# indrajeetadityaroy9/rabitq-ann-search

Hardware: AMD Instinct MI355X
Metric: qps (search_batch_device, layer-0 hot path end to end) + fastscan_dist_per_s (higher is better)
Workload: dtype u32 popcount / f32; 1 GPU; SIFT1M-class synthetic (int-valued, clustered; SURVEY 8d C2): 1000000x128 f32 (D=128), 4-bit RaBitQ FastScan + exact-L2 rerank, R=32, k=10, 10000 queries per GPU resident in HBM; n_index=1000000, dim=128, bits=4, k=10, nq_per_gpu=10000, index_builder=cphnsw_mi355x (this repo), batch_sets=2, parallelism=query-sharded x1, index replicated

## Files before the change

### include/cphnsw_mi355x.h

```cpp
#ifndef CPHNSW_MI355X_H
#define CPHNSW_MI355X_H

#include <stddef.h>
#include <stdint.h>

#ifdef __cplusplus
extern "C" {
#endif

typedef struct cph_index cph_index;

typedef enum {
    CPH_OK = 0,
    CPH_INVALID_ARGUMENT = 1,
    CPH_RUNTIME_ERROR = 2,
    CPH_OUT_OF_MEMORY = 3,
    CPH_NOT_IMPLEMENTED = 4
} cph_status;

const char* cph_last_error(void);

int cph_version(void);

int cph_create(uint64_t dim, uint64_t bits, int device, cph_index** out);
int cph_destroy(cph_index* h);

int cph_load(cph_index* h, const char* path);
int cph_save(cph_index* h, const char* path);
int cph_save_native(cph_index* h, const char* path);
int cph_load_native(cph_index* h, const char* path);
int cph_size(cph_index* h, uint64_t* n);
int cph_dim(cph_index* h, uint64_t* dim);
int cph_is_finalized(cph_index* h, int* flag);

int cph_build(cph_index* h, const float* vectors, uint64_t n);
int cph_finalize(cph_index* h);
int cph_knn_bruteforce(int device, const float* vectors, uint64_t n, uint64_t dim, const float* queries,
                       uint64_t nq, uint32_t* ids, float* dist);

int cph_encode_edges(int device, uint64_t dim, uint64_t bits, const float* parent, const float* nbrs, uint64_t cnt,
                     uint8_t* values, float* aux, uint32_t* pops);

int cph_select_hook(int device, const float* x, uint64_t n, uint64_t D, uint32_t vertex, const uint32_t* fwd,
                    const uint32_t* rev, uint64_t n_rev, uint32_t R, float alpha, float tau, float alpha_max,
                    const float* err, uint32_t* out_ids, uint32_t* out_cnt);

int cph_calib_hook(cph_index* h, const float* queries, const uint32_t* start, uint64_t ns, float* rec, uint32_t* rec_cnt,
                   float* dqp);

int cph_debug_heap_ops(int device, const uint8_t* ops, uint64_t n_ops, const float* keys, const uint32_t* ids, uint64_t n_push,
                       float* out_keys, uint32_t* out_ids, uint32_t* out_size);

int cph_search_batch(cph_index* h, const float* queries, uint64_t n, uint64_t k,
                     int64_t* ids, float* dist);

int cph_search_batch_device(cph_index* h, const float* d_queries, uint64_t n, uint64_t k,
                            int64_t* d_ids, float* d_dist, void* stream);
int cph_synchronize(cph_index* h);

typedef struct cph_filter cph_filter;
int cph_filter_create(cph_index* h, const uint32_t* words, uint64_t n_bits, cph_filter** out);
int cph_filter_destroy(cph_filter* f);
int cph_search_batch_filtered(cph_index* h, const float* queries, uint64_t n, uint64_t k, const cph_filter* f,
                              int64_t* ids, float* dist);
int cph_search_batch_device_filtered(cph_index* h, const float* d_queries, uint64_t n, uint64_t k,
                                     const cph_filter* f, int64_t* d_ids, float* d_dist, void* stream);

int cph_search(cph_index* h, const float* query, uint64_t k, int64_t* ids, float* dist,
               uint64_t* m);

int cph_get_vectors(cph_index* h, uint64_t first, uint64_t count, float* out);

int cph_set_batch_sets(cph_index* h, uint32_t n_sets);

int cph_set_search_params(cph_index* h, uint32_t slots, uint64_t beam_capacity);

int cph_last_search_stats(cph_index* h, uint64_t out[12]);
int cph_last_query_expansions(cph_index* index, uint32_t* out, uint64_t n);
int cph_order_queries(cph_index* index, const float* keys, uint64_t n, uint32_t* order);

int cph_encode_query(cph_index* h, const float* query, uint8_t* lut, float* coeffs);

int cph_entry_point(cph_index* h, const float* query, uint32_t* entry);

int cph_fastscan_block(cph_index* h, const uint8_t* lut, const float* qparams,
                       uint32_t vertex, float dist_qp_sq, float worst, int nn_full,
                       uint32_t* sums, uint32_t* msb, float* est, float* lower,
                       float* lower_stage1);

int cph_exact_l2(cph_index* h, const float* query, const uint32_t* ids, uint64_t n,
                 float* out);

typedef struct cph_stream cph_stream;
int cph_fastscan_stream_create(int device, uint32_t D, uint32_t bits, uint64_t n_blocks,
                               uint64_t seed, cph_stream** out, uint64_t* block_bytes);
int cph_fastscan_stream_run(cph_stream* s, int reps, double* avg_ms, double* checksum);
int cph_fastscan_stream_export(cph_stream* s, uint64_t first, uint64_t count,
                               uint8_t* ref_blocks, uint8_t* lut, float* qparams,
                               float* dist_qp_sq);
int cph_fastscan_stream_eval(cph_stream* s, uint64_t first, uint64_t count, float* est,
                             float* lower);
int cph_fastscan_stream_destroy(cph_stream* s);

int cph_host_rewrite_index(const char* path_in, const char* path_out);
int cph_host_repack_block(uint32_t D, uint32_t bits, const uint8_t* ref_block, uint8_t* dev_block,
                          uint64_t* dev_bytes, uint8_t* ref_roundtrip);
int cph_host_encode_query(uint64_t dim, const float* query, uint8_t* lut, float* coeffs, uint32_t* masks);

#ifdef __cplusplus
}
#endif
#endif
```

### rabitq-ann-search_amd/cphnsw_mi355x/_lib.py

```python
import ctypes as C
import importlib.util
import os
import sys

from . import build as _build

OK, INVALID_ARGUMENT, RUNTIME_ERROR, OUT_OF_MEMORY, NOT_IMPLEMENTED = range(5)

SYMBOLS = {
    "cph_last_error": (C.c_char_p, []),
    "cph_version": (C.c_int, []),
    "cph_create": (C.c_int, [C.c_uint64, C.c_uint64, C.c_int, C.POINTER(C.c_void_p)]),
    "cph_destroy": (C.c_int, [C.c_void_p]),
    "cph_load": (C.c_int, [C.c_void_p, C.c_char_p]),
    "cph_save": (C.c_int, [C.c_void_p, C.c_char_p]),
    "cph_save_native": (C.c_int, [C.c_void_p, C.c_char_p]),
    "cph_load_native": (C.c_int, [C.c_void_p, C.c_char_p]),
    "cph_size": (C.c_int, [C.c_void_p, C.POINTER(C.c_uint64)]),
    "cph_dim": (C.c_int, [C.c_void_p, C.POINTER(C.c_uint64)]),
    "cph_is_finalized": (C.c_int, [C.c_void_p, C.POINTER(C.c_int)]),
    "cph_build": (C.c_int, [C.c_void_p, C.c_void_p, C.c_uint64]),
    "cph_finalize": (C.c_int, [C.c_void_p]),
    "cph_knn_bruteforce": (C.c_int, [C.c_int, C.c_void_p, C.c_uint64, C.c_uint64, C.c_void_p, C.c_uint64,
                                     C.c_void_p, C.c_void_p]),
    "cph_debug_heap_ops": (C.c_int, [C.c_int, C.c_void_p, C.c_uint64, C.c_void_p, C.c_void_p, C.c_uint64, C.c_void_p, C.c_void_p,
                                     C.c_void_p]),
    "cph_select_hook": (C.c_int, [C.c_int, C.c_void_p, C.c_uint64, C.c_uint64, C.c_uint32, C.c_void_p, C.c_void_p, C.c_uint64,
                                  C.c_uint32, C.c_float, C.c_float, C.c_float, C.c_void_p, C.c_void_p, C.c_void_p]),
    "cph_calib_hook": (C.c_int, [C.c_void_p, C.c_void_p, C.c_void_p, C.c_uint64, C.c_void_p, C.c_void_p, C.c_void_p]),
    "cph_encode_edges": (C.c_int, [C.c_int, C.c_uint64, C.c_uint64, C.c_void_p, C.c_void_p, C.c_uint64, C.c_void_p,
                                   C.c_void_p, C.c_void_p]),
    "cph_search_batch": (C.c_int, [C.c_void_p, C.c_void_p, C.c_uint64, C.c_uint64, C.c_void_p, C.c_void_p]),
    "cph_search_batch_device": (C.c_int, [C.c_void_p, C.c_void_p, C.c_uint64, C.c_uint64, C.c_void_p,
                                          C.c_void_p, C.c_void_p]),
    "cph_filter_create": (C.c_int, [C.c_void_p, C.c_void_p, C.c_uint64, C.POINTER(C.c_void_p)]),
    "cph_filter_destroy": (C.c_int, [C.c_void_p]),
    "cph_search_batch_filtered": (C.c_int, [C.c_void_p, C.c_void_p, C.c_uint64, C.c_uint64, C.c_void_p, C.c_void_p,
                                            C.c_void_p]),
    "cph_search_batch_device_filtered": (C.c_int, [C.c_void_p, C.c_void_p, C.c_uint64, C.c_uint64, C.c_void_p,
                                                   C.c_void_p, C.c_void_p, C.c_void_p]),
    "cph_synchronize": (C.c_int, [C.c_void_p]),
    "cph_set_batch_sets": (C.c_int, [C.c_void_p, C.c_uint32]),
    "cph_search": (C.c_int, [C.c_void_p, C.c_void_p, C.c_uint64, C.c_void_p, C.c_void_p,
                             C.POINTER(C.c_uint64)]),
    "cph_get_vectors": (C.c_int, [C.c_void_p, C.c_uint64, C.c_uint64, C.c_void_p]),
    "cph_set_search_params": (C.c_int, [C.c_void_p, C.c_uint32, C.c_uint64]),
    "cph_last_search_stats": (C.c_int, [C.c_void_p, C.POINTER(C.c_uint64)]),
    "cph_last_query_expansions": (C.c_int, [C.c_void_p, C.c_void_p, C.c_uint64]),
    "cph_order_queries": (C.c_int, [C.c_void_p, C.c_void_p, C.c_uint64, C.c_void_p]),
    "cph_encode_query": (C.c_int, [C.c_void_p, C.c_void_p, C.c_void_p, C.c_void_p]),
    "cph_entry_point": (C.c_int, [C.c_void_p, C.c_void_p, C.POINTER(C.c_uint32)]),
    "cph_fastscan_block": (C.c_int, [C.c_void_p, C.c_void_p, C.c_void_p, C.c_uint32, C.c_float, C.c_float,
                                     C.c_int, C.c_void_p, C.c_void_p, C.c_void_p, C.c_void_p, C.c_void_p]),
    "cph_exact_l2": (C.c_int, [C.c_void_p, C.c_void_p, C.c_void_p, C.c_uint64, C.c_void_p]),
    "cph_host_rewrite_index": (C.c_int, [C.c_char_p, C.c_char_p]),
    "cph_host_repack_block": (C.c_int, [C.c_uint32, C.c_uint32, C.c_void_p, C.c_void_p, C.POINTER(C.c_uint64), C.c_void_p]),
    "cph_host_encode_query": (C.c_int, [C.c_uint64, C.c_void_p, C.c_void_p, C.c_void_p, C.c_void_p]),
    "cph_fastscan_stream_create": (C.c_int, [C.c_int, C.c_uint32, C.c_uint32, C.c_uint64, C.c_uint64,
                                             C.POINTER(C.c_void_p), C.POINTER(C.c_uint64)]),
    "cph_fastscan_stream_run": (C.c_int, [C.c_void_p, C.c_int, C.POINTER(C.c_double), C.POINTER(C.c_double)]),
    "cph_fastscan_stream_export": (C.c_int, [C.c_void_p, C.c_uint64, C.c_uint64, C.c_void_p, C.c_void_p,
                                             C.c_void_p, C.POINTER(C.c_float)]),
    "cph_fastscan_stream_eval": (C.c_int, [C.c_void_p, C.c_uint64, C.c_uint64, C.c_void_p, C.c_void_p]),
    "cph_fastscan_stream_destroy": (C.c_int, [C.c_void_p]),
}

_LIB = None


def _share_hip_runtime_with_torch():
    if "torch" in sys.modules:
        return
    try:
        spec = importlib.util.find_spec("torch")
    except (ImportError, ValueError):
        spec = None
    if spec is None or not spec.origin:
        return
    cand = os.path.join(os.path.dirname(spec.origin), "lib", "libamdhip64.so")
    if os.path.exists(cand):
        try:
            C.CDLL(cand, mode=C.RTLD_GLOBAL)
        except OSError:
            pass


def lib():
    global _LIB
    if _LIB is None:
        path = os.environ.get("CPH_LIB_PATH")
        if not path:
            path = _build.LIB_PATH
            if _build.needs_build():
                path = _build.build_library()
        _share_hip_runtime_with_torch()
        L = C.CDLL(path)
        diagnostic = bool(os.environ.get("CPH_LIB_PATH"))
        for name, (res, args) in SYMBOLS.items():
            try:
                fn = getattr(L, name)
            except AttributeError:
                if diagnostic:
                    continue
                raise
            fn.restype = res
            fn.argtypes = args
        _LIB = L
    return _LIB


def check(rc):
    if rc == OK:
        return
    msg = lib().cph_last_error().decode("utf-8", "replace")
    if rc == INVALID_ARGUMENT:
        raise ValueError(msg)
    if rc == OUT_OF_MEMORY:
        raise MemoryError(msg)
    if rc == NOT_IMPLEMENTED:
        raise NotImplementedError(msg)
    raise RuntimeError(msg)
```

### rabitq-ann-search_amd/cphnsw_mi355x/build.py

```python
import os
import shutil
import subprocess

PKG_DIR = os.path.dirname(os.path.abspath(__file__))
CSRC = os.path.join(os.path.dirname(PKG_DIR), "csrc")
LIB_PATH = os.path.join(PKG_DIR, "libcphnsw_mi355x.so")
SOURCES = ["cphnsw_mi355x.hip"]
HEADERS = ["cph_core.h", "builder.h", "builder_host.h", "host_parallel.h", "search_coalescer.h", "builder_pipeline.h", "device_knn.h", "device_knn_sym.h", "device_build.h", "device_buf.h", "native_file.h", "device_encode.h", "device_fastscan.h", "device_search.h", "device_stream.h", "device_heap_test.h", "host_index.h"]
FLAGS = ["-O3", "-std=c++17", "--offload-arch=gfx950", "-fPIC", "-shared", "-ffp-contract=off",
         "-Wall", "-Wno-unused-function"]


def _hipcc():
    for c in (os.environ.get("HIPCC"), shutil.which("hipcc"), "/opt/rocm/bin/hipcc"):
        if c and os.path.exists(c):
            return c
    raise RuntimeError("hipcc not found (need ROCm to build the gfx950 library)")


def needs_build():
    if not os.path.exists(LIB_PATH):
        return True
    t = os.path.getmtime(LIB_PATH)
    deps = [os.path.join(CSRC, f) for f in SOURCES + HEADERS]
    deps.append(os.path.join(os.path.dirname(os.path.dirname(PKG_DIR)), "include", "cphnsw_mi355x.h"))
    return any(os.path.getmtime(d) > t for d in deps if os.path.exists(d))


def build_library(force=False, verbose=False):
    if not force and not needs_build():
        return LIB_PATH
    cmd = [_hipcc()] + FLAGS + [os.path.join(CSRC, s) for s in SOURCES] + ["-o", LIB_PATH, "-lpthread"]
    if verbose:
        print(" ".join(cmd))
    subprocess.check_call(cmd)
    return LIB_PATH


if __name__ == "__main__":
    print(build_library(force=True, verbose=True))
```

### rabitq-ann-search_amd/csrc/builder_pipeline.h

```cpp
#pragma once
#include <exception>
#include <thread>
#include <type_traits>
#include "builder.h"

namespace cph {
namespace build {

struct BuiltDevice {
    DevBuf<uint8_t> blocks;
    DevBuf<float> raw;
    DevBuf<float> norm;
    std::vector<uint8_t> own_host;
};

inline size_t isqrt_sz(size_t n) { return (size_t)std::floor(std::sqrt((double)n)); }

template <int BW, bool G>
inline void launch_encode(const EncodeArgsB& a, uint32_t grid, size_t lds) {
    if (lds > 48 * 1024)
        HIP_CHECK(hipFuncSetAttribute(reinterpret_cast<const void*>(&encode_edges_kernel<BW, G>),
                                      hipFuncAttributeMaxDynamicSharedMemorySize, (int)lds));
    hipLaunchKernelGGL((encode_edges_kernel<BW, G>), dim3(grid), dim3(64), lds, nullptr, a);
    HIP_CHECK(hipGetLastError());
// ... 95 lines not shown
        if (Dk == D) {
            knn_self_device(d_x.p, d_norm.p, n, D, num_cus, d_knn.p, d_kd.p, verbose);
        } else {
            DevBuf<float> d_xk(n * Dk);
            HIP_CHECK(hipMemset(d_xk.p, 0, n * Dk * 4));
            HIP_CHECK(hipMemcpy2D(d_xk.p, Dk * 4, d_x.p, D * 4, D * 4, n, hipMemcpyDeviceToDevice));
            knn_self_device(d_xk.p, d_norm.p, n, Dk, num_cus, d_knn.p, d_kd.p, verbose);
        }
    }
    tm.lap("exact 32-NN (MFMA)");

    GraphStatsRecord gs{};
    {
        const size_t sample = std::max<size_t>(1, std::min(isqrt_sz(n), n));
        std::mt19937 rng(43);
        std::vector<size_t> pick(n);
        std::iota(pick.begin(), pick.end(), 0);
        std::shuffle(pick.begin(), pick.end(), rng);
        pick.resize(sample);
        auto dist = [&](uint32_t a, uint32_t b) {
            double s = 0;
            for (size_t j = 0; j < dim; ++j) { const double t = (double)vecs[(size_t)a * dim + j] - vecs[(size_t)b * dim + j]; s += t * t; }
            return (float)s;
        };
        const size_t pairs_of = std::clamp((size_t)(2.0 * std::sqrt((double)R)), (size_t)4, (size_t)R);
        std::vector<float> edge_len, first_len, between;
        std::vector<uint32_t> row(kKnnK);
        double deg = 0;
        for (size_t v : pick) {
            HIP_CHECK(hipMemcpy(row.data(), d_knn.p + v * kKnnK, kKnnK * 4, hipMemcpyDeviceToHost));
            size_t c = 0;
            while (c < (size_t)kKnnK && row[c] != kInvalidNode) ++c;
            deg += (double)c;
            for (size_t s = 0; s < c; ++s) edge_len.push_back(dist((uint32_t)v, row[s]));
            if (c) first_len.push_back(edge_len[edge_len.size() - c]);
            const size_t m = std::min(c, pairs_of);
            for (size_t i = 0; i < m; ++i)
                for (size_t j = i + 1; j < m; ++j) between.push_back(dist(row[i], row[j]));
        }
        gs.avg_degree = (float)(deg / (double)pick.size());
        if (edge_len.empty() || between.empty() || first_len.empty()) {
            gs.alpha = 1.0f; gs.tau = 0.0f; gs.alpha_max = 4.0f;
        } else {
            std::sort(edge_len.begin(), edge_len.end());
            std::sort(between.begin(), between.end());
            const float tiny = 1e-8f / (float)D;
            const float med = quantile_sorted(edge_len, 1, 2), q1 = quantile_sorted(edge_len, 1, 4), q3 = quantile_sorted(edge_len, 3, 4);
            double mu = 0, var = 0;
            for (float d : edge_len) mu += d;
            mu /= edge_len.size();
            for (float d : edge_len) var += (d - mu) * (d - mu);
            var /= edge_len.size();
            const float cv = mu > tiny ? (float)(std::sqrt(var) / mu) : 0.2f;
            const float inter = quantile_sorted(between, 1, 4);
            gs.alpha = inter < tiny ? 1.0f + cv : med / inter;
            gs.alpha_max = std::min(q1 > tiny ? q3 / q1 : 2.0f, 5.0f);
            gs.alpha = std::clamp(gs.alpha, 1.0f, gs.alpha_max);
            gs.alpha_max = std::max(gs.alpha_max, 2.0f * gs.alpha);
            gs.tau = mad_sigma(first_len, median_of(first_len));
        }
    }

    DevBuf<uint32_t> d_nbr(n * 32), d_cnt(n);
    {
        DevBuf<float> d_err(n);
        const float err_tol = 1.0f / std::sqrt((float)D);
        hipLaunchKernelGGL(centered_norm_kernel, dim3(grid_for(n, 256)), dim3(256), 0, nullptr, d_x.p, d_centroid.p, (uint64_t)n,
                           (uint32_t)D, (uint32_t)dim, err_tol, d_err.p);
        HIP_CHECK(hipGetLastError());
        LayerParams lp{R, gs.alpha, gs.tau, gs.alpha_max, d_err.p};
        select_layer(d_x.p, D, d_knn.p, n, nullptr, lp, num_cus, d_nbr.p, d_cnt.p);
    }
    d_knn.release();
    tm.lap("reverse edges + selection");

    std::vector<uint32_t> nbr(n * 32), cnt(n);
    HIP_CHECK(hipMemcpy(nbr.data(), d_nbr.p, n * 32 * 4, hipMemcpyDeviceToHost));
    HIP_CHECK(hipMemcpy(cnt.data(), d_cnt.p, n * 4, hipMemcpyDeviceToHost));
    std::vector<uint32_t> old_to_new(n, kInvalidNode), new_to_old(n);
    {
        std::vector<std::pair<double, uint32_t>> near(n);
        parallel_for(n, 4096, [&](size_t lo, size_t hi_) {
            for (size_t i = lo; i < hi_; ++i) {
                double s = 0;
                for (size_t j = 0; j < dim; ++j) { const double t = (double)vecs[i * dim + j] - centroid[j]; s += t * t; }
                near[i] = {s, (uint32_t)i};
            }
        });
        const size_t top = std::min(n, std::max<size_t>(1, isqrt_sz(n)));
        std::partial_sort(near.begin(), near.begin() + top, near.end());
        uint32_t hub = near[0].second;
        for (size_t i = 1; i < top; ++i)
            if (cnt[near[i].second] > cnt[hub]) hub = near[i].second;
        std::vector<uint8_t> seen(n, 0);
        std::vector<uint32_t> queue;
        queue.reserve(n);
        uint32_t next = 0;
        auto walk = [&](uint32_t start) {
            if (seen[start]) return;
            seen[start] = 1;
            queue.push_back(start);
            for (size_t head = queue.size() - 1; head < queue.size(); ++head) {
                const uint32_t v = queue[head];
                old_to_new[v] = next;
                new_to_old[next++] = v;
                for (uint32_t j = 0; j < cnt[v]; ++j) {
                    const uint32_t w = nbr[(size_t)v * 32 + j];
                    if (w < n && !seen[w]) { seen[w] = 1; queue.push_back(w); }
                }
            }
        };
        walk(hub);
        for (size_t i = 0; i < n; ++i) walk((uint32_t)i);
    }
    tm.lap("hub + BFS order");

    DevBuf<uint32_t> d_o2n(n), d_n2o(n);
    HIP_CHECK(hipMemcpy(d_o2n.p, old_to_new.data(), n * 4, hipMemcpyHostToDevice));
    HIP_CHECK(hipMemcpy(d_n2o.p, new_to_old.data(), n * 4, hipMemcpyHostToDevice));
    dev.raw.alloc(n * D);
    dev.norm.alloc(n);
    hipLaunchKernelGGL(gather_rows_kernel, dim3((uint32_t)std::min<uint64_t>(n, (uint64_t)num_cus * 64)), dim3(64), 0, nullptr,
                       d_x.p, d_n2o.p, (uint64_t)n, (uint32_t)D, dev.raw.p);
    HIP_CHECK(hipGetLastError());
    hipLaunchKernelGGL(gather_u32_kernel, dim3(grid_for(n, 256)), dim3(256), 0, nullptr, d_norm.p, d_n2o.p, (uint64_t)n, dev.norm.p);
    HIP_CHECK(hipGetLastError());
    DevBuf<uint32_t> d_nbr_new(n * 32);
    hipLaunchKernelGGL(permute_lists_kernel, dim3(grid_for(n * 32, 256)), dim3(256), 0, nullptr, d_nbr.p, d_n2o.p, d_o2n.p,
                       (uint64_t)n, d_nbr_new.p);
    HIP_CHECK(hipGetLastError());
    HIP_CHECK(hipDeviceSynchronize());
    d_x.release(); d_norm.release(); d_nbr.release(); d_cnt.release();

    DevBuf<float> d_signs(3 * D);
    HIP_CHECK(hipMemcpy(d_signs.p, hi.rot.signs.data(), 3 * D * 4, hipMemcpyHostToDevice));
    const float df = (float)D;
    const float norm_factor = 1.0f / (df * std::sqrt(df)), inv_sqrt_d = 1.0f / std::sqrt(df);
    dev.blocks.alloc(n * L.stride + 64);
    HIP_CHECK(hipMemset(dev.blocks.p, 0, n * L.stride + 64));
    const size_t words = (D + 63) / 64;
    const uint32_t own_meta = (uint32_t)round_up(bw * words * 8, 64);
    const uint32_t own_stride = (uint32_t)hi.RL.nb_off;
    DevBuf<uint8_t> d_own(n * own_stride);
    HIP_CHECK(hipMemset(d_own.p, 0, n * own_stride));
    {
        EncodeArgsB a{};
        a.x = dev.raw.p; a.nbr = d_nbr_new.p; a.centroid = d_centroid.p; a.n = n; a.dim = (uint32_t)dim; a.D = (uint32_t)D;
        a.signs = d_signs.p; a.norm_factor = norm_factor; a.inv_sqrt_d = inv_sqrt_d; a.L = L; a.blocks = dev.blocks.p;
        a.own = d_own.p; a.own_stride = own_stride; a.own_meta = own_meta;
        run_encode(bw, a, n, num_cus);
        a.nbr = nullptr;
        run_encode(bw, a, (n + 31) / 32, num_cus);
    }
    tm.lap("gather + edge / own codes");

    std::vector<int32_t> levels_new(n);
    for (size_t nw = 0; nw < n; ++nw) levels_new[nw] = levels[new_to_old[nw]];
    upper_job.wait();
    std::vector<std::vector<UpperEdge>> upper = ul.export_layers(old_to_new);
    const float upper_tau = ul.tau, upper_alpha = ul.alpha;
    tm.lap("upper layers (host threads, built behind the kNN): wait + export");

    hi.raw.resize(n * D);
    hi.norm_sq.resize(n);
    HIP_CHECK(hipMemcpy(hi.raw.data(), dev.raw.p, n * D * 4, hipMemcpyDeviceToHost));
    HIP_CHECK(hipMemcpy(hi.norm_sq.data(), dev.norm.p, n * 4, hipMemcpyDeviceToHost));
    hi.levels = std::move(levels_new);
    hi.search_data.clear();
    dev.own_host.resize(n * (size_t)own_stride);
    HIP_CHECK(hipMemcpy(dev.own_host.data(), d_own.p, n * (size_t)own_stride, hipMemcpyDeviceToHost));
    hi.upper = std::move(upper);
    hi.max_level = max_level;
    hi.entry = old_to_new[entry_old];
    hi.upper_tau = upper_tau;
    hi.upper_alpha = upper_alpha;
    hi.centroid = centroid;
    ProfileRecord prof;
    prof.n = n; prof.D = D; prof.R = R; prof.bits = bw;
    prof.evt_min_tail = std::max<size_t>(64, isqrt_sz(n));
    prof.min_calib_samples = std::clamp((size_t)(10.0 * std::sqrt((double)n)), (size_t)200, n);
    prof.slack_levels = std::clamp((int)std::ceil(std::log2(std::max(10.0f * std::log2((float)std::max(n, (size_t)64)), 4.0f))), 4, 32);
    prof.graph_stats = gs;
    std::memcpy(hi.profile, &prof, 72);
    std::memset(hi.calib, 0, sizeof(hi.calib));
    tm.lap("vectors, norms, own codes to the host");
}

struct DeviceIndexView {
    const uint8_t* blocks;
    const float* raw;
    const float* signs;
    DevLayout L;
    float norm_factor, inv_sqrt_d;
};

inline void calibrate(HostIndex& hi, const DeviceIndexView& dv, int num_cus, bool verbose) {
    StageTimer tm{verbose};
    const size_t n = hi.n, D = hi.D, dim = hi.dim, bw = hi.bw;
    if (n < 50) throw std::runtime_error("Calibration requires at least 50 nodes.");
    ProfileRecord prof;
    std::memcpy(&prof, hi.profile, 72);
    const size_t n_db = std::min(prof.min_calib_samples, n), n_syn = std::min(prof.min_calib_samples / 2, n);
    const size_t ns = n_db + n_syn;
    std::mt19937 rng(42 + 99999);
    std::vector<uint32_t> order(n);
    std::iota(order.begin(), order.end(), 0u);
    std::shuffle(order.begin(), order.end(), rng);
    std::vector<float> sigma(dim, 0.0f);
    {
        const size_t vs = std::max<size_t>(2, std::min(n, prof.min_calib_samples / 4));
        std::vector<double> s1(dim, 0.0), s2(dim, 0.0);
        for (size_t i = 0; i < vs; ++i) {
            const float* v = hi.vec(order[i]);
            for (size_t d = 0; d < dim; ++d) { s1[d] += v[d]; s2[d] += (double)v[d] * v[d]; }
        }
        for (size_t d = 0; d < dim; ++d) {
            const double mu = s1[d] / vs;
            sigma[d] = (float)std::sqrt(std::max(s2[d] / vs - mu * mu, (double)kEpsSmall));
        }
    }
    std::vector<float> q(ns * dim);
    std::vector<uint32_t> start(ns);
    for (size_t i = 0; i < n_db; ++i) {
        std::memcpy(&q[i * dim], hi.vec(order[i]), dim * 4);
        start[i] = order[i];
    }
    std::normal_distribution<float> gauss(0.0f, 1.0f);
    for (size_t i = 0; i < n_syn; ++i) {
        const float* base = hi.vec(order[i % n]);
        for (size_t d = 0; d < dim; ++d) q[(n_db + i) * dim + d] = base[d] + gauss(rng) * sigma[d];
        start[n_db + i] = order[(n_db + i) % n];
    }
    const uint32_t PW = dv.L.PW;
    DevBuf<float> d_q(ns * dim), d_qp(ns * D), d_rec(ns * 32 * 6), d_dqp(ns), d_ed(ns);
    DevBuf<uint4> d_masks(ns * PW);
    DevBuf<QueryHeader> d_hdr(ns);
    DevBuf<uint32_t> d_start(ns), d_rc(ns);
    HIP_CHECK(hipMemcpy(d_q.p, q.data(), ns * dim * 4, hipMemcpyHostToDevice));
    HIP_CHECK(hipMemcpy(d_start.p, start.data(), ns * 4, hipMemcpyHostToDevice));
    {
        EncodeArgs e{};
        e.queries_raw = d_q.p; e.nq = (uint32_t)ns; e.dim = (uint32_t)dim; e.D = (uint32_t)D; e.PW = PW;
        e.signs = dv.signs; e.norm_factor = dv.norm_factor; e.inv_sqrt_d = dv.inv_sqrt_d;
        e.raw = dv.raw; e.n = n; e.entry = 0; e.max_level = 0;
        e.queries_padded = d_qp.p; e.qmasks = d_masks.p; e.qhdr = d_hdr.p; e.entry_dist = d_ed.p;
        hipLaunchKernelGGL(encode_kernel, dim3((uint32_t)std::min<uint64_t>(ns, (uint64_t)num_cus * 32)), dim3(64),
                           encode_lds_bytes((uint32_t)D), nullptr, e);
        HIP_CHECK(hipGetLastError());
        CalibArgs c{};
        c.blocks = dv.blocks; c.raw = dv.raw; c.L = dv.L; c.n = n; c.queries = d_qp.p; c.qmasks = d_masks.p; c.qhdr = d_hdr.p;
        c.start = d_start.p; c.ns = (uint32_t)ns; c.rec = d_rec.p; c.rec_cnt = d_rc.p; c.dqp_out = d_dqp.p;
        const size_t lds = (size_t)PW * 16 + (size_t)D * 8;
        const dim3 grid((uint32_t)std::min<uint64_t>(ns, (uint64_t)num_cus * 16));
        if (bw == 1) hipLaunchKernelGGL(calib_kernel<1>, grid, dim3(64), lds, nullptr, c);
        else if (bw == 2) hipLaunchKernelGGL(calib_kernel<2>, grid, dim3(64), lds, nullptr, c);
        else hipLaunchKernelGGL(calib_kernel<4>, grid, dim3(64), lds, nullptr, c);
        HIP_CHECK(hipGetLastError());
    }
    std::vector<float> rec(ns * 32 * 6), dqp(ns);
    std::vector<uint32_t> rc(ns);
    HIP_CHECK(hipMemcpy(rec.data(), d_rec.p, rec.size() * 4, hipMemcpyDeviceToHost));
    HIP_CHECK(hipMemcpy(dqp.data(), d_dqp.p, ns * 4, hipMemcpyDeviceToHost));
    HIP_CHECK(hipMemcpy(rc.data(), d_rc.p, ns * 4, hipMemcpyDeviceToHost));
    tm.lap("calibration samples (GPU)");

    CalibrationRecord cal{};
    std::vector<float> ipqo, est_ratio, truth, nops;
    struct Pair { float nop, ipc, ipq, dqp, exact; };
    std::vector<Pair> pairs;
    for (size_t s = 0; s < ns; ++s)
        for (uint32_t j = 0; j < rc[s] && j < 32; ++j) {
            const float* r = &rec[(s * 32 + j) * 6];
            ipqo.push_back(r[5]);
            nops.push_back(r[0]);
            truth.push_back(r[3]);
            pairs.push_back({r[0], r[1], r[2], dqp[s], r[4]});
        }
    if (ipqo.empty()) throw std::runtime_error("Calibration failed: no ip_qo samples.");
    if (pairs.size() < 20) throw std::runtime_error("Calibration failed: too few estimator/target pairs.");
    {
        const float med = median_of(ipqo);
        cal.ip_qo_floor = std::max(med - 3.0f * mad_sigma(ipqo, med), kEpsMedium);
    }
    est_ratio.resize(pairs.size());
    for (size_t i = 0; i < pairs.size(); ++i) est_ratio[i] = pairs[i].ipc / std::max(pairs[i].ipq, cal.ip_qo_floor);
    {
        double a, b;
        robust_line(est_ratio, truth, a, b);
        const size_t np = truth.size();
        double mt = 0, me = 0;
        for (size_t i = 0; i < np; ++i) { mt += truth[i]; me += est_ratio[i]; }
        mt /= np; me /= np;
        double ssr = 0, sst = 0, sxx = 0;
        for (size_t i = 0; i < np; ++i) {
            const double res = truth[i] - (a * est_ratio[i] + b);
            ssr += res * res;
            sst += (truth[i] - mt) * (truth[i] - mt);
            sxx += (est_ratio[i] - me) * (est_ratio[i] - me);
        }
        const double r2 = sst > kEpsSmall ? 1.0 - ssr / sst : 0.0;
        double lev = 0.0;
        if (sxx > kEpsSmall)
            for (size_t i = 0; i < np; ++i) lev = std::max(lev, 1.0 / np + (est_ratio[i] - me) * (est_ratio[i] - me) / sxx);
        if (r2 < 0.1 || lev > 4.0 / (double)np) { a = 1.0; b = 0.0; }
        cal.affine_a = (float)a;
        cal.affine_b = (float)b;
// ... 49 lines not shown
```

### rabitq-ann-search_amd/csrc/cph_core.h

```cpp
#pragma once
#include <cstddef>
#include <cstdint>

namespace cph {

constexpr uint32_t kInvalidNode = 0xFFFFFFFFu;
constexpr int kR = 32;
constexpr float kEpsTiny = 1e-20f;
constexpr float kEpsSmall = 1e-12f;
constexpr float kEpsMedium = 1e-10f;
constexpr int kMaxSlack = 32;

struct DevLayout {
    uint32_t D;
    uint32_t BW;
    uint32_t PW;
    uint32_t wide;
    uint32_t NH;
    uint32_t CPL;
    uint32_t codes_bytes;
    uint32_t aux_off;
    uint32_t ids_off;
    uint32_t count_off;
    uint32_t stride;
};

#ifndef CPH_BLOCK_ALIGN
#define CPH_BLOCK_ALIGN 64u
#endif
template <int BW, int SD>
struct StaticLayout {
    static constexpr uint32_t kCodesBytes = 32u * (uint32_t)BW * (SD >= 32 ? (uint32_t)SD / 32u : 1u) * 4u;
    static constexpr uint32_t kAuxOff = kCodesBytes;
    static constexpr uint32_t kIdsOff = kAuxOff + 32u * 16u;
    static constexpr uint32_t kCountOff = kIdsOff + 32u * 4u;
    static constexpr uint32_t kStride = (kCountOff + 4u + CPH_BLOCK_ALIGN - 1u) / CPH_BLOCK_ALIGN * CPH_BLOCK_ALIGN;
};

inline DevLayout make_dev_layout(uint32_t D, uint32_t BW) {
    DevLayout L{};
    L.D = D;
    L.BW = BW;
    L.PW = D >= 32 ? D / 32 : 1;
    L.wide = D >= 128 ? 1 : 0;
    uint32_t T = BW * L.PW;
    if (L.wide) {
        L.NH = (T / 4 >= 2) ? 2 : 1;
        L.CPL = T / 4 / L.NH;
    } else {
        L.NH = 1;
        L.CPL = 0;
    }
    L.codes_bytes = 32 * T * 4;
    L.aux_off = L.codes_bytes;
    L.ids_off = L.aux_off + 32 * 16;
    L.count_off = L.ids_off + 32 * 4;
    L.stride = (L.count_off + 4 + CPH_BLOCK_ALIGN - 1) / CPH_BLOCK_ALIGN * CPH_BLOCK_ALIGN;
    return L;
}

struct RefLayout {
    size_t vertex_bytes, nb_off;
    size_t codes, nop, ip_qo, ip_cp, pop, wpop, ids, count;
    size_t plane_bytes, nb_bytes;
};

inline size_t round_up(size_t x, size_t a) { return (x + a - 1) / a * a; }

inline RefLayout make_ref_layout(size_t D, size_t bw) {
    RefLayout L{};
    size_t words = (D + 63) / 64;
    size_t code = round_up(round_up(bw * words * 8, 64) + 8, 64);
    L.plane_bytes = (((D + 3) / 4 + 1) / 2) * 32;
    size_t o = 0;
    L.codes = o; o += bw * round_up(L.plane_bytes, 64);
    L.nop = o;   o += 128;
    L.ip_qo = o; o += 128;
    L.ip_cp = o; o += 128;
    L.pop = o;   o += 64;
    if (bw > 1) { L.wpop = o; o += 64; } else { L.wpop = (size_t)-1; }
    L.ids = o;   o += 128;
    L.count = o; o += 4;
    L.nb_bytes = round_up(o, 64);
    L.nb_off = code;
    L.vertex_bytes = code + L.nb_bytes;
    return L;
}

struct QueryHeader {
    float A, B, C;
    uint32_t entry;
};

struct SearchConsts {
    float affine_a, affine_b, ip_qo_floor;
    float gamma, gamma_max, gamma_beta;
    uint64_t gamma_warmup;
    int32_t num_slack;
    float slack[kMaxSlack];
};

enum QueryStatus : uint32_t { kStatusOk = 0, kStatusOverflow = 1 };

}
```

### rabitq-ann-search_amd/csrc/cphnsw_mi355x.hip

```cpp
#include <hip/hip_runtime.h>

#include <algorithm>
#include <atomic>
#include <cfloat>
#include <chrono>
#include <condition_variable>
#include <deque>
#include <functional>
#include <memory>
#include <mutex>
#include <new>
#include <string>
#include <thread>
#include <vector>

#include "../../include/cphnsw_mi355x.h"
#include "cph_core.h"
#include "device_buf.h"
#include "device_encode.h"
#include "device_fastscan.h"
#include "device_search.h"
#include "device_stream.h"
#include "device_heap_test.h"
#include "host_index.h"
#include "host_parallel.h"
#include "search_coalescer.h"
#include "native_file.h"
#include "builder_pipeline.h"

using namespace cph;

namespace {

thread_local std::string g_err;

int fail(int code, const std::string& msg) {
    g_err = msg;
    return code;
}

struct InvalidArg : std::invalid_argument {
    using std::invalid_argument::invalid_argument;
};

template <class F>
int guarded(F&& f) {
    try {
        f();
        return CPH_OK;
    } catch (const std::invalid_argument& e) {
        return fail(CPH_INVALID_ARGUMENT, e.what());
    } catch (const std::bad_alloc&) {
        return fail(CPH_OUT_OF_MEMORY, "out of memory");
    } catch (const std::exception& e) {
        return fail(CPH_RUNTIME_ERROR, e.what());
    }
}

size_t next_pow2(size_t n) {
    size_t p = 1;
    while (p < n) p *= 2;
    return p;
}

#define CPH_LAUNCH_BITS(KERNEL, bits, SDV, grid, block, lds, st, args)                            \
    do {                                                                                          \
        if ((bits) == 1) hipLaunchKernelGGL((KERNEL<1, SDV>), grid, block, lds, st, args);        \
        else if ((bits) == 2) hipLaunchKernelGGL((KERNEL<2, SDV>), grid, block, lds, st, args);   \
        else hipLaunchKernelGGL((KERNEL<4, SDV>), grid, block, lds, st, args);                    \
    } while (0)
#define CPH_LAUNCH(KERNEL, bits, D, grid, block, lds, st, args)                                   \
    do {                                                                                          \
        if ((D) == 128) CPH_LAUNCH_BITS(KERNEL, bits, 128, grid, block, lds, st, args);           \
        else if ((D) == 1024) CPH_LAUNCH_BITS(KERNEL, bits, 1024, grid, block, lds, st, args);    \
        else CPH_LAUNCH_BITS(KERNEL, bits, 0, grid, block, lds, st, args);                        \
        HIP_CHECK(hipGetLastError());                                                             \
    } while (0)

__global__ void scan_counts_kernel(const uint8_t* blocks, uint64_t n, uint32_t stride, uint32_t count_off, uint32_t* flags) {
    const uint64_t v = (uint64_t)blockIdx.x * blockDim.x + threadIdx.x;
    if (v >= n) return;
    const uint32_t cnt = *reinterpret_cast<const uint32_t*>(blocks + v * stride + count_off);
    if (cnt & 7u) atomicOr(flags, 2u);
}

}

struct BatchSet {
    DevBuf<float> d_queries_raw, d_queries, d_entry_dist, d_dist;
    DevBuf<uint4> d_qmasks;
    DevBuf<QueryHeader> d_qhdr;
    DevBuf<int64_t> d_ids;
    DevBuf<uint32_t> d_count, d_status, d_order, d_redo;
    DevBuf<unsigned long long> d_stats;
    unsigned long long* pin_stats = nullptr;
    uint8_t* pin_io = nullptr;
    uint8_t* pin_io_dev = nullptr;
    size_t pin_io_bytes = 0;
    DevBuf<uint32_t> d_bitmaps, d_logids;
    DevBuf<uint32_t> d_beam, d_beam_tail;
    uint32_t slots = 0;
    uint64_t cap = 0;
    DevBuf<uint32_t> r_bitmaps, r_logids;
    DevBuf<uint32_t> r_beam, r_beam_tail;
    uint32_t r_slots = 0;
    hipEvent_t ev0 = nullptr, ev1 = nullptr, ev_done = nullptr;
    bool used = false;
    uint32_t nq = 0;
    uint32_t run_slots = 0;
    uint64_t run_cap = 0;
    bool stats_in_hbm = false;
};
constexpr int kStatWords = 18;
constexpr int kMaxBatchSets = 4;
constexpr uint64_t kSmallBatch = 32;

struct cph_filter {
    int device = 0;
    uint64_t n_bits = 0;
    uint64_t popcount = 0;
    DevBuf<uint32_t> words;
};

struct cph_index {
    uint64_t dim = 0;
    uint32_t bits = 0;
    uint32_t D = 0;
    int device = 0;
    bool finalized = false;
    bool needs_build = false;
    std::vector<float> pending;
    uint64_t pending_n = 0;
    HostIndex host;
    DevLayout L{};
    SearchConsts sc{};
    uint32_t flags = 0;
    int num_cus = 256;
    bool waves_from_env = false;
    uint32_t waves_per_cu = 4 * CPH_SEARCH_WAVES_PER_SIMD;
    DevBuf<uint8_t> d_blocks;
    DevBuf<float> d_raw, d_norm;
    DevBuf<float> d_signs;
    DevBuf<uint32_t> d_upper;
    DevBuf<uint32_t> d_row_of;
    UpperLayerDev layers[kMaxUpperLayers];
    int32_t dev_max_level = 0;
    float norm_factor = 0.0f, inv_sqrt_d = 0.0f;
    NativeMapping native_map;
    const uint8_t* own_view = nullptr;
    std::vector<uint8_t> own_store;
    BatchSet sets[kMaxBatchSets + kLeaderSlots];
    int n_sets = 2;
    int last_set = kMaxBatchSets - 1;
    int last_search = -1;
    hipStream_t own_stream = nullptr;
    bool order_queries = true;
    uint32_t want_slots = 0;
    uint64_t want_cap = 0;
    uint64_t auto_cap = 0;
    bool pf_off = false;
    bool pf_dense = false;
    std::mutex mu;
    SearchCoalescer coal;
    struct LeaderSlot {
        hipStream_t stream = nullptr;
        uint8_t* pin = nullptr;
        uint8_t* pin_dev = nullptr;
        size_t pin_bytes = 0;
        uint32_t seq = 0;
        uint64_t cur_n = 0, cur_k = 0;
    } leaders[kLeaderSlots];

    void use_device() const { HIP_CHECK(hipSetDevice(device)); }
};

namespace {

bool probe_first(const cph_index* h) {
    return (h->L.D == 128 || h->L.D == 1024) && !(h->flags & 2u) && !h->pf_off && !h->pf_dense;
}

void require_finalized(cph_index* h) {
    if (!h->finalized) throw std::runtime_error("Search failed: invalid entry point after finalize.");
}

void release_scratch(BatchSet& s) {
    s.d_bitmaps.release(); s.d_logids.release(); s.d_beam.release(); s.d_beam_tail.release();
    s.r_bitmaps.release(); s.r_logids.release(); s.r_beam.release(); s.r_beam_tail.release();
    s.slots = 0; s.cap = 0; s.r_slots = 0;
}

void quiesce(cph_index* h) {
    for (auto& s : h->sets)
        if (s.used && s.ev_done) HIP_CHECK(hipEventSynchronize(s.ev_done));
}

void upload_arrays(cph_index* h) {
    h->use_device();
    quiesce(h);
    const HostIndex& hi = h->host;
    h->L = make_dev_layout((uint32_t)hi.D, (uint32_t)hi.bw);
    const size_t n = hi.n;
    const size_t stride = h->L.stride;
    h->d_blocks.alloc(n * stride + 64);
    h->d_raw.alloc(n * hi.D);
    h->d_norm.alloc(n);
    const size_t chunk = std::max<size_t>(1, std::min<size_t>(n, (256u << 20) / stride));
    std::vector<uint8_t> stage(chunk * stride);
    for (size_t base = 0; base < n; base += chunk) {
        const size_t cnt = std::min(chunk, n - base);
        parallel_for(cnt, 256, [&](size_t lo, size_t hi_) {
            for (size_t v = lo; v < hi_; ++v)
                repack_ref_to_dev(hi.nb(base + v), hi.RL, h->L, &stage[v * stride]);
        });
        HIP_CHECK(hipMemcpy(h->d_blocks.p + base * stride, stage.data(), cnt * stride,
                            hipMemcpyHostToDevice));
    }
    HIP_CHECK(hipMemcpy(h->d_raw.p, hi.raw.data(), n * hi.D * 4, hipMemcpyHostToDevice));
    HIP_CHECK(hipMemcpy(h->d_norm.p, hi.norm_sq.data(), n * 4, hipMemcpyHostToDevice));
}

void upload_feeders(cph_index* h) {
    h->use_device();
    quiesce(h);
    const HostIndex& hi = h->host;
    const size_t n = hi.n;
    h->L = make_dev_layout((uint32_t)hi.D, (uint32_t)hi.bw);
    h->sc = hi.consts();
    h->flags = hi.has_dup_neighbors ? 1u : 0u;
    if (n != 0) {
        DevBuf<uint32_t> d_flag(1);
        HIP_CHECK(hipMemset(d_flag.p, 0, 4));
        hipLaunchKernelGGL(scan_counts_kernel, dim3((uint32_t)((n + 255) / 256)), dim3(256), 0, nullptr, h->d_blocks.p, (uint64_t)n,
                           h->L.stride, h->L.count_off, d_flag.p);
        HIP_CHECK(hipGetLastError());
        uint32_t f = 0;
        HIP_CHECK(hipMemcpy(&f, d_flag.p, 4, hipMemcpyDeviceToHost));
        h->flags |= f & 2u;
    }
    h->d_signs.alloc(3 * hi.D);
    HIP_CHECK(hipMemcpy(h->d_signs.p, hi.rot.signs.data(), 3 * hi.D * 4, hipMemcpyHostToDevice));
    const float d = static_cast<float>(hi.D);
    h->norm_factor = 1.0f / (d * std::sqrt(d));
    h->inv_sqrt_d = 1.0f / std::sqrt(d);
    const int nl = std::min<int>({(int)hi.upper.size(), (int)hi.max_level, kMaxUpperLayers});
    h->dev_max_level = hi.max_level > 0 ? nl : 0;
    std::vector<uint32_t> flat;
    std::vector<size_t> off_nodes(nl), off_offs(nl), off_nbrs(nl);
    for (int l = 0; l < nl; ++l) {
        const auto& layer = hi.upper[l];
        off_nodes[l] = flat.size();
        for (const auto& e : layer) flat.push_back(e.node);
        off_offs[l] = flat.size();
        uint32_t acc = 0;
        for (const auto& e : layer) { flat.push_back(acc); acc += (uint32_t)e.nbrs.size(); }
        flat.push_back(acc);
        off_nbrs[l] = flat.size();
        for (const auto& e : layer) flat.insert(flat.end(), e.nbrs.begin(), e.nbrs.end());
    }
    h->d_upper.alloc(flat.size() + 1);
    if (!flat.empty())
        HIP_CHECK(hipMemcpy(h->d_upper.p, flat.data(), flat.size() * 4, hipMemcpyHostToDevice));
    for (int l = 0; l < kMaxUpperLayers; ++l) h->layers[l] = UpperLayerDev{nullptr, nullptr, nullptr, nullptr, 0};
    int mapped = 0;
    for (int l = 0; l < nl; ++l) mapped += hi.upper[l].size() > 16 ? 1 : 0;
    h->d_row_of.alloc((size_t)mapped * n + 1);
    std::vector<uint32_t> row_of;
    for (int l = 0, m = 0; l < nl; ++l) {
        const uint32_t* dmap = nullptr;
        if (hi.upper[l].size() > 16) {
            row_of.assign(n, kInvalidNode);
            uint64_t first = 0;
            bool fits = true;
            for (size_t r = 0; r < hi.upper[l].size(); ++r) {
                const uint64_t deg = hi.upper[l][r].nbrs.size();
                if (first >= (1u << 26) || deg > 62) { fits = false; break; }
                row_of[hi.upper[l][r].node] = (uint32_t)first | ((uint32_t)deg << 26);
                first += deg;
            }
            if (!fits) { h->layers[l] = UpperLayerDev{h->d_upper.p + off_nodes[l], h->d_upper.p + off_offs[l], h->d_upper.p + off_nbrs[l], nullptr, (uint32_t)hi.upper[l].size()}; ++m; continue; }
            HIP_CHECK(hipMemcpy(h->d_row_of.p + (size_t)m * n, row_of.data(), n * 4, hipMemcpyHostToDevice));
            dmap = h->d_row_of.p + (size_t)m * n;
            ++m;
        }
        h->layers[l] = UpperLayerDev{h->d_upper.p + off_nodes[l], h->d_upper.p + off_offs[l],
                                     h->d_upper.p + off_nbrs[l], dmap, (uint32_t)hi.upper[l].size()};
    }
    for (auto& s : h->sets) release_scratch(s);
    h->auto_cap = 0;
    h->pf_off = false;
    h->pf_dense = false;
    h->last_search = -1;
}

void materialize_search_data(cph_index* h) {
    HostIndex& hi = h->host;
    if (!hi.search_data.empty() || hi.n == 0) return;
    h->use_device();
    quiesce(h);
    const size_t n = hi.n, stride = h->L.stride, own_stride = hi.RL.nb_off;
    hi.search_data.assign(n * hi.RL.vertex_bytes, 0);
    const size_t chunk = std::max<size_t>(1, std::min<size_t>(n, (512u << 20) / stride));
    std::vector<uint8_t> stage(chunk * stride);
    for (size_t base = 0; base < n; base += chunk) {
        const size_t c = std::min(chunk, n - base);
        HIP_CHECK(hipMemcpy(stage.data(), h->d_blocks.p + base * stride, c * stride, hipMemcpyDeviceToHost));
        parallel_for(c, 256, [&](size_t lo, size_t hi_) {
            for (size_t v = lo; v < hi_; ++v) {
                uint8_t* dst = &hi.search_data[(base + v) * hi.RL.vertex_bytes];
                if (h->own_view) std::memcpy(dst, h->own_view + (base + v) * own_stride, own_stride);
                repack_dev_to_ref(&stage[v * stride], h->L, hi.RL, dst + hi.RL.nb_off);
            }
        });
    }
}

void init_set(BatchSet& s) {
    if (s.ev0) return;
    HIP_CHECK(hipEventCreate(&s.ev0));
    HIP_CHECK(hipEventCreate(&s.ev1));
    HIP_CHECK(hipEventCreateWithFlags(&s.ev_done, hipEventDisableTiming));
    HIP_CHECK(hipHostMalloc(reinterpret_cast<void**>(&s.pin_stats), kStatWords * 8, hipHostMallocDefault));
    std::memset(s.pin_stats, 0, kStatWords * 8);
}

BatchSet& next_set(cph_index* h, hipStream_t st) {
    h->last_set = (h->last_set + 1) % h->n_sets;
    BatchSet& s = h->sets[h->last_set];
    init_set(s);
    for (BatchSet& o : h->sets) {
        if (!(o.used && o.ev_done && !o.stats_in_hbm && hipEventQuery(o.ev_done) == hipSuccess)) continue;
        if (o.pin_stats[5] > o.pin_stats[8] && o.cap < h->host.n + 1)
            h->auto_cap = std::max<uint64_t>(h->auto_cap, std::min<uint64_t>(h->host.n + 1, o.cap * 4));
        if (o.pin_stats[8] * 50 > o.nq) h->pf_off = true;
        if (o.pin_stats[0] >= 10000) {
            const double new_per_exp = (double)o.pin_stats[2] / (double)o.pin_stats[0];
            const double off = h->bits == 4 ? 6.0 : 2.8, on = h->bits == 4 ? 4.5 : 2.2;
            if (new_per_exp > off) h->pf_dense = true;
            else if (new_per_exp < on) h->pf_dense = false;
        }
    }
    if (s.used) HIP_CHECK(hipStreamWaitEvent(st, s.ev_done, 0));
    return s;
}

void stage_queries(cph_index* h, BatchSet& s, const float* d_raw_q, uint64_t nq, hipStream_t st) {
    const HostIndex& hi = h->host;
    const uint32_t D = (uint32_t)hi.D, PW = h->L.PW;
    if (hi.entry == kInvalidNode || hi.entry >= hi.n)
        throw std::runtime_error("Search failed: invalid entry point after finalize.");
    if (s.d_queries.n < nq * D || s.d_qmasks.n < nq * PW || s.d_qhdr.n < nq) {
        if (s.used) HIP_CHECK(hipEventSynchronize(s.ev_done));
        s.d_queries.alloc(nq * D);
        s.d_qmasks.alloc(nq * PW);
        s.d_qhdr.alloc(nq);
        s.d_entry_dist.alloc(nq);
        s.d_order.alloc(nq);
    }
    EncodeArgs a{};
    a.queries_raw = d_raw_q;
    a.nq = (uint32_t)nq;
    a.dim = (uint32_t)hi.dim;
    a.D = D;
    a.PW = PW;
    a.signs = h->d_signs.p;
    a.norm_factor = h->norm_factor;
    a.inv_sqrt_d = h->inv_sqrt_d;
    a.raw = h->d_raw.p;
    a.n = hi.n;
    a.entry = hi.entry;
    a.max_level = h->dev_max_level;
    for (int l = 0; l < kMaxUpperLayers; ++l) a.layers[l] = h->layers[l];
    a.queries_padded = s.d_queries.p;
    a.qmasks = s.d_qmasks.p;
    a.qhdr = s.d_qhdr.p;
    a.entry_dist = s.d_entry_dist.p;
    const uint32_t grid = (uint32_t)std::min<uint64_t>(nq, (uint64_t)h->num_cus * 32);
    hipLaunchKernelGGL(encode_kernel, dim3(grid), dim3(64), encode_lds_bytes(D), st, a);
    HIP_CHECK(hipGetLastError());
}

const float* upload_queries(cph_index* h, BatchSet& s, const float* queries, uint64_t nq, hipStream_t st) {
    if (s.d_queries_raw.n < nq * h->dim) {
        if (s.used) HIP_CHECK(hipEventSynchronize(s.ev_done));
        s.d_queries_raw.alloc(nq * h->dim);
    }
    HIP_CHECK(hipMemcpyAsync(s.d_queries_raw.p, queries, nq * h->dim * 4, hipMemcpyHostToDevice, st));
    return s.d_queries_raw.p;
}

void ensure_scratch(cph_index* h, BatchSet& s, uint32_t slots, uint64_t cap, hipStream_t st) {
    const uint64_t n = h->host.n;
    const uint64_t bm_words = (n + 31) / 32;
    if (!(s.slots >= slots && s.cap == cap)) {
        if (s.used) HIP_CHECK(hipEventSynchronize(s.ev_done));
        s.d_bitmaps.alloc((size_t)slots * bm_words);
        HIP_CHECK(hipMemsetAsync(s.d_bitmaps.p, 0, (size_t)slots * bm_words * 4, st));
        s.d_logids.alloc((size_t)slots * cap);
        s.d_beam.alloc((size_t)slots * kBeamPagesDwords);
        s.d_beam_tail.alloc((size_t)slots * beam_tail_dwords(cap));
        s.slots = slots;
        s.cap = cap;
    }
    if ((cap < n + 1 || probe_first(h)) && s.r_slots == 0) {
        size_t free_b = 0, total_b = 0;
        HIP_CHECK(hipMemGetInfo(&free_b, &total_b));
        const uint64_t per = (n + 1) * 4 + ((uint64_t)kBeamPagesDwords + beam_tail_dwords(n + 1)) * 4 + bm_words * 4;
        const uint64_t want = (&s - h->sets) >= kMaxBatchSets ? kLeaderGroup : kSmallBatch;
        const uint32_t rs = (uint32_t)std::max<uint64_t>(1, std::min<uint64_t>(want, (uint64_t)(free_b * 0.25) / per));
        s.r_bitmaps.alloc((size_t)rs * bm_words);
        HIP_CHECK(hipMemsetAsync(s.r_bitmaps.p, 0, (size_t)rs * bm_words * 4, st));
        s.r_logids.alloc((size_t)rs * (n + 1));
        s.r_beam.alloc((size_t)rs * kBeamPagesDwords);
        s.r_beam_tail.alloc((size_t)rs * beam_tail_dwords(n + 1));
        s.r_slots = rs;
    }
}

struct DoneFlags {
    uint32_t* flags = nullptr;
    uint32_t seq = 0;
};

template <int SD>
void launch_filtered(uint32_t bits, uint32_t grid, size_t lds, hipStream_t st, const SearchArgs& a) {
    if (bits == 1) hipLaunchKernelGGL((search_kernel<1, SD, false, true>), dim3(grid), dim3(64), lds, st, a);
    else if (bits == 2) hipLaunchKernelGGL((search_kernel<2, SD, false, true>), dim3(grid), dim3(64), lds, st, a);
    else hipLaunchKernelGGL((search_kernel<4, SD, false, true>), dim3(grid), dim3(64), lds, st, a);
    HIP_CHECK(hipGetLastError());
}

void launch_search(cph_index* h, BatchSet& s, uint32_t nq, uint32_t k, int64_t* d_ids, float* d_dist, uint32_t* d_count,
                   const uint32_t* d_todo, int mode, hipStream_t st, DoneFlags done = DoneFlags(),
                   const uint32_t* d_allow = nullptr) {
    SearchArgs a{};
    a.allow = d_allow;
    const bool pf = d_allow == nullptr && probe_first(h);
    a.done_flags = done.flags;
    a.done_seq = done.seq;
    a.blocks = h->d_blocks.p;
    a.raw = h->d_raw.p;
    a.norm_sq = h->d_norm.p;
    a.n = h->host.n;
    a.L = h->L;
    a.flags = h->flags;
    a.queries = s.d_queries.p;
    a.qmasks = s.d_qmasks.p;
    a.qhdr = s.d_qhdr.p;
    a.k = k;
    a.sc = h->sc;
    a.bm_words = (h->host.n + 31) / 32;
    a.out_ids = d_ids;
    a.out_dist = d_dist;
    a.out_count = d_count;
    a.status = s.d_status.p;
    a.stats = s.d_stats.p;
    uint32_t* words = reinterpret_cast<uint32_t*>(s.d_stats.p + 16);
    uint32_t grid;
    if (mode == 0) {
// ... 139 lines not shown

struct SmallIo {
    int64_t* h_ids; float* h_dist; uint32_t* h_count; float* h_query;
    int64_t* d_ids; float* d_dist; uint32_t* d_count; const float* d_query;
};
SmallIo small_io(cph_index* h, BatchSet& s, uint64_t n, uint64_t k) {
    const size_t o_dist = n * k * 8, o_cnt = o_dist + n * k * 4, o_q = (o_cnt + n * 4 + 15) & ~(size_t)15;
    const size_t need = o_q + n * h->dim * 4;
    if (s.pin_io_bytes < need) {
        if (s.used) HIP_CHECK(hipEventSynchronize(s.ev_done));
        if (s.pin_io) HIP_CHECK(hipHostFree(s.pin_io));
        s.pin_io = nullptr;
        s.pin_io_bytes = 0;
        const size_t bytes = std::max<size_t>(need * 2, 64 * 1024);
        HIP_CHECK(hipHostMalloc(reinterpret_cast<void**>(&s.pin_io), bytes, hipHostMallocMapped | hipHostMallocCoherent));
        HIP_CHECK(hipHostGetDevicePointer(reinterpret_cast<void**>(&s.pin_io_dev), s.pin_io, 0));
        s.pin_io_bytes = bytes;
    }
    uint8_t* hb = s.pin_io;
    uint8_t* db = s.pin_io_dev;
    return SmallIo{reinterpret_cast<int64_t*>(hb), reinterpret_cast<float*>(hb + o_dist), reinterpret_cast<uint32_t*>(hb + o_cnt),
                   reinterpret_cast<float*>(hb + o_q),
                   reinterpret_cast<int64_t*>(db), reinterpret_cast<float*>(db + o_dist), reinterpret_cast<uint32_t*>(db + o_cnt),
                   reinterpret_cast<const float*>(db + o_q)};
}

}

#ifdef CPH_SEARCH_TRACE
static std::atomic<uint64_t> g_tr[6];
static inline uint64_t now_ns() { return std::chrono::duration_cast<std::chrono::nanoseconds>(std::chrono::steady_clock::now().time_since_epoch()).count(); }
#define CPH_TR(i, v) g_tr[i] += (v)
#else
#define CPH_TR(i, v) do {} while (0)
static inline uint64_t now_ns() { return 0; }
#endif

extern "C" {

const char* cph_last_error(void) { return g_err.c_str(); }
int cph_version(void) { return 100; }

int cph_create(uint64_t dim, uint64_t bits, int device, cph_index** out) {
    return guarded([&] {
        if (!out) throw InvalidArg("out must not be null");
        *out = nullptr;
        if (bits != 1 && bits != 2 && bits != 4)
            throw InvalidArg("Unsupported bits=" + std::to_string(bits) + ". Supported: 1, 2, 4.");
        const size_t pd = next_pow2(dim);
        if (dim == 0) throw InvalidArg("dim must be > 0");
        if (pd < 16 || pd > 2048) {
            if (pd < 16) {
                throw InvalidArg("Unsupported dimension " + std::to_string(dim) + " (padded to " +
                                 std::to_string(pd) +
                                 "). Supported padded dims: 16, 32, 64, 128, 256, 512, 1024, 2048.");
            }
            throw InvalidArg("Unsupported dimension " + std::to_string(dim) + " (padded to " +
                             std::to_string(pd) +
                             "). Supported padded dims: 16, 32, 64, 128, 256, 512, 1024, 2048.");
        }
        int ndev = 0;
        if (hipGetDeviceCount(&ndev) != hipSuccess || ndev <= 0)
            throw std::runtime_error("No HIP device available: the MI355X path has no CPU fallback.");
        if (device < 0 || device >= ndev) throw InvalidArg("invalid device ordinal");
        auto* h = new cph_index();
        h->dim = dim;
        h->bits = (uint32_t)bits;
        h->D = (uint32_t)pd;
        h->device = device;
        hipDeviceProp_t prop;
        if (hipGetDeviceProperties(&prop, device) == hipSuccess) h->num_cus = prop.multiProcessorCount;
        if (const char* e = getenv("CPH_QUERY_ORDER")) h->order_queries = atoi(e) != 0;
        if (const char* e = getenv("CPH_LEADER_SLOTS")) h->coal.n_slots = std::max(1, std::min(kLeaderSlots, atoi(e)));
        if (const char* e = getenv("CPH_GATHER_US")) h->coal.gather_us = std::max(0, atoi(e));
        if (const char* e = getenv("CPH_WAVES_PER_CU")) { h->waves_per_cu = (uint32_t)std::max(1, atoi(e)); h->waves_from_env = true; }
        *out = h;
    });
}

int cph_destroy(cph_index* h) {
    return guarded([&] {
        if (!h) return;
        (void)hipSetDevice(h->device);
        for (auto& s : h->sets) {
            if (s.used && s.ev_done) (void)hipEventSynchronize(s.ev_done);
            if (s.ev0) (void)hipEventDestroy(s.ev0);
            if (s.ev1) (void)hipEventDestroy(s.ev1);
            if (s.ev_done) (void)hipEventDestroy(s.ev_done);
            if (s.pin_stats) (void)hipHostFree(s.pin_stats);
            if (s.pin_io) (void)hipHostFree(s.pin_io);
        }
#ifdef CPH_SEARCH_TRACE
        if (g_tr[0]) fprintf(stderr, "[search trace] groups=%llu callers=%llu per group: mutex wait %.1f us, enqueue %.1f us; per caller: own-query wait %.1f us\n",
                             (unsigned long long)g_tr[0], (unsigned long long)g_tr[1], g_tr[2] / 1e3 / g_tr[0], g_tr[3] / 1e3 / g_tr[0], g_tr[4] / 1e3 / g_tr[1]);
        for (auto& x : g_tr) x = 0;
#endif
        if (h->own_stream) (void)hipStreamDestroy(h->own_stream);
        for (auto& ls : h->leaders) {
            if (ls.stream) { (void)hipStreamSynchronize(ls.stream); (void)hipStreamDestroy(ls.stream); }
            if (ls.pin) (void)hipHostFree(ls.pin);
        }
        delete h;
    });
}

static void begin_device_swap(cph_index* h) {
    h->use_device();
    quiesce(h);
    h->finalized = false;
    for (auto& s : h->sets) release_scratch(s);
    h->last_search = -1;
}

int cph_load(cph_index* h, const char* path) {
    return guarded([&] {
        if (!h || !path) throw InvalidArg("null argument");
        std::lock_guard<std::mutex> lk(h->mu);
        HostIndex t;
        t.load(path, h->D, h->bits, h->dim);
        begin_device_swap(h);
        h->host = std::move(t);
        h->needs_build = false;
        std::vector<float>().swap(h->pending);
        h->pending_n = 0;
        h->native_map.reset();
        h->own_view = nullptr;
        std::vector<uint8_t>().swap(h->own_store);
        upload_arrays(h);
        upload_feeders(h);
        h->finalized = true;
    });
}

int cph_save(cph_index* h, const char* path) {
    return guarded([&] {
        if (!h || !path) throw InvalidArg("null argument");
        std::lock_guard<std::mutex> lk(h->mu);
        if (!h->finalized) throw std::runtime_error("Index must be finalized before saving.");
        materialize_search_data(h);
        h->host.save(path);
    });
}

int cph_save_native(cph_index* h, const char* path) {
    return guarded([&] {
        if (!h || !path) throw InvalidArg("null argument");
        std::lock_guard<std::mutex> lk(h->mu);
        if (!h->finalized) throw std::runtime_error("Index must be finalized before saving.");
        h->use_device();
        quiesce(h);
        const HostIndex& hi = h->host;
        const size_t n = hi.n, stride = h->L.stride, own_stride = hi.RL.nb_off;
        std::vector<uint8_t> blocks(n * stride), own;
        HIP_CHECK(hipMemcpy(blocks.data(), h->d_blocks.p, n * stride, hipMemcpyDeviceToHost));
        const uint8_t* own_p = h->own_view;
        if (!own_p) {
            own.resize(n * own_stride);
            for (size_t v = 0; v < n; ++v) std::memcpy(&own[v * own_stride], &hi.search_data[v * hi.RL.vertex_bytes], own_stride);
            own_p = own.data();
        }
        write_native(path, hi, (uint32_t)stride, own_p, (uint32_t)own_stride, blocks.data());
    });
}

int cph_load_native(cph_index* h, const char* path) {
    return guarded([&] {
        if (!h || !path) throw InvalidArg("null argument");
        std::lock_guard<std::mutex> lk(h->mu);
        HostIndex t;
        NativeMapping map;
        const NativeHeader nh = read_native(path, h->D, h->bits, h->dim, t, map);
        begin_device_swap(h);
        h->host = std::move(t);
        h->needs_build = false;
        std::vector<float>().swap(h->pending);
        h->pending_n = 0;
        h->native_map = std::move(map);
        const uint8_t* base = static_cast<const uint8_t*>(h->native_map.base);
        std::vector<uint8_t>().swap(h->own_store);
        h->own_view = base + nh.own_off;
        h->L = make_dev_layout((uint32_t)h->host.D, (uint32_t)h->host.bw);
        const size_t n = h->host.n;
        h->d_blocks.alloc(n * nh.stride + 64);
        h->d_raw.alloc(n * h->host.D);
        h->d_norm.alloc(n);
        HIP_CHECK(hipMemcpy(h->d_blocks.p, base + nh.blocks_off, n * (size_t)nh.stride, hipMemcpyHostToDevice));
        HIP_CHECK(hipMemcpy(h->d_raw.p, h->host.raw_view, n * h->host.D * 4, hipMemcpyHostToDevice));
        HIP_CHECK(hipMemcpy(h->d_norm.p, h->host.norm_sq.data(), n * 4, hipMemcpyHostToDevice));
        upload_feeders(h);
        h->finalized = true;
    });
}

int cph_size(cph_index* h, uint64_t* n) {
    return guarded([&] { *n = h->needs_build ? h->pending_n : h->host.n; });
}
int cph_dim(cph_index* h, uint64_t* dim) {
    return guarded([&] { *dim = h->dim; });
}
int cph_is_finalized(cph_index* h, int* flag) {
    return guarded([&] { *flag = h->finalized ? 1 : 0; });
}

int cph_build(cph_index* h, const float* vectors, uint64_t n) {
    return guarded([&] {
        if (!h) throw InvalidArg("null handle");
        std::lock_guard<std::mutex> lk(h->mu);
        if (n == 0) throw InvalidArg("build requires at least one vector.");
        if (!vectors) throw InvalidArg("null vectors");
        h->use_device();
        quiesce(h);
        h->host = HostIndex();
        h->native_map.reset();
        h->own_view = nullptr;
        std::vector<uint8_t>().swap(h->own_store);
        h->finalized = false;
        h->d_blocks.release(); h->d_raw.release(); h->d_norm.release();
        for (auto& s : h->sets) release_scratch(s);
        h->pending.assign(vectors, vectors + n * h->dim);
        h->pending_n = n;
        h->needs_build = true;
    });
}

int cph_finalize(cph_index* h) {
    return guarded([&] {
        if (!h) throw InvalidArg("null handle");
        std::lock_guard<std::mutex> lk(h->mu);
        const uint64_t n = h->needs_build ? h->pending_n : h->host.n;
        if (n == 0) throw std::runtime_error("Cannot finalize an empty index.");
        if (!h->needs_build) throw std::runtime_error("Finalize called without a pending build.");
        if (n < 50) throw std::runtime_error("Calibration requires at least 50 nodes.");
        if (n >= 0xFFFFFFFFull) throw InvalidArg("too many vectors");
        h->use_device();
        const bool verbose = getenv("CPH_BUILD_VERBOSE") != nullptr;
        quiesce(h);
        h->d_blocks.release(); h->d_raw.release(); h->d_norm.release();
        for (auto& s : h->sets) release_scratch(s);
        build::BuiltDevice dev;
        build::build_graph(h->host, dev, h->pending.data(), n, h->dim, h->D, h->bits, h->num_cus, verbose);
        std::vector<float>().swap(h->pending);
        h->pending_n = 0;
        h->needs_build = false;
        h->d_blocks = std::move(dev.blocks);
        h->d_raw = std::move(dev.raw);
        h->d_norm = std::move(dev.norm);
        h->native_map.reset();
        h->own_store = std::move(dev.own_host);
        h->own_view = h->own_store.data();
        upload_feeders(h);
        build::DeviceIndexView view{h->d_blocks.p, h->d_raw.p, h->d_signs.p, h->L, h->norm_factor, h->inv_sqrt_d};
        build::calibrate(h->host, view, h->num_cus, verbose);
        h->sc = h->host.consts();
        h->finalized = true;
    });
}

int cph_knn_bruteforce(int device, const float* vectors, uint64_t n, uint64_t dim, const float* queries,
                       uint64_t nq, uint32_t* ids, float* dist) {
    return guarded([&] {
        if (!vectors || !ids || !dist || n == 0 || dim == 0) throw InvalidArg("bad arguments");
        if (n >= 0xFFFFFFFFull || nq >= 0xFFFFFFFFull) throw InvalidArg("too many rows");
        HIP_CHECK(hipSetDevice(device));
        const size_t D = std::max<size_t>(16, next_pow2(dim));
        auto pad = [&](const float* src, uint64_t rows, std::vector<float>& x, std::vector<float>& nrm) {
            x.assign(rows * D, 0.0f);
            nrm.resize(rows);
            parallel_for(rows, 1024, [&](size_t lo, size_t hi) {
                for (size_t i = lo; i < hi; ++i) {
                    std::memcpy(&x[i * D], src + i * dim, dim * 4);
                    float s = 0.0f;
                    for (uint64_t j = 0; j < dim; ++j) s = std::fmaf(x[i * D + j], x[i * D + j], s);
                    nrm[i] = s;
                }
            });
        };
        std::vector<float> x, nrm, q, qn;
        pad(vectors, n, x, nrm);
        if (queries) pad(queries, nq, q, qn);
        int cus = 256;
        hipDeviceProp_t prop;
        if (hipGetDeviceProperties(&prop, device) == hipSuccess) cus = prop.multiProcessorCount;
        build::gpu_knn(queries ? q.data() : nullptr, queries ? qn.data() : nullptr, nq, x.data(), nrm.data(), n, D,
                       cus, ids, dist);
    });
}

int cph_debug_heap_ops(int device, const uint8_t* ops, uint64_t n_ops, const float* keys, const uint32_t* ids, uint64_t n_push,
                       float* out_keys, uint32_t* out_ids, uint32_t* out_size) {
    return guarded([&] {
        if (!ops || !out_keys || !out_ids || !out_size || n_ops == 0 || n_ops > 0x7FFFFFFFull) throw InvalidArg("bad arguments");
        if (n_push && (!keys || !ids)) throw InvalidArg("bad arguments");
        uint64_t pushes = 0;
        for (uint64_t i = 0; i < n_ops; ++i) pushes += ops[i] ? 1 : 0;
        if (pushes != n_push) throw InvalidArg("n_push must equal the number of push operations");
        HIP_CHECK(hipSetDevice(device));
        DevBuf<uint8_t> d_ops(n_ops);
        DevBuf<float> d_keys(std::max<uint64_t>(1, n_push)), d_ok(std::max<uint64_t>(1, n_push));
        DevBuf<uint32_t> d_ids(std::max<uint64_t>(1, n_push)), d_oi(std::max<uint64_t>(1, n_push)), d_sz(1);
        DevBuf<uint32_t> d_spill(kBeamPagesDwords), d_spill_tail(beam_tail_dwords(std::max<uint64_t>(1, n_push) + 64));
        HIP_CHECK(hipMemcpy(d_ops.p, ops, n_ops, hipMemcpyHostToDevice));
        if (n_push) {
            HIP_CHECK(hipMemcpy(d_keys.p, keys, n_push * 4, hipMemcpyHostToDevice));
            HIP_CHECK(hipMemcpy(d_ids.p, ids, n_push * 4, hipMemcpyHostToDevice));
        }
        HeapTestArgs a{d_ops.p, d_keys.p, d_ids.p, (uint32_t)n_ops, d_spill.p, d_spill_tail.p, d_ok.p, d_oi.p, d_sz.p};
        hipLaunchKernelGGL(heap_selftest_kernel, dim3(1), dim3(64), 0, nullptr, a);
        HIP_CHECK(hipGetLastError());
        HIP_CHECK(hipDeviceSynchronize());
        HIP_CHECK(hipMemcpy(out_size, d_sz.p, 4, hipMemcpyDeviceToHost));
        if (*out_size > n_push) throw std::runtime_error("heap self-test: size out of range");
        if (*out_size) {
            HIP_CHECK(hipMemcpy(out_keys, d_ok.p, (size_t)*out_size * 4, hipMemcpyDeviceToHost));
            HIP_CHECK(hipMemcpy(out_ids, d_oi.p, (size_t)*out_size * 4, hipMemcpyDeviceToHost));
        }
    });
}

int cph_encode_edges(int device, uint64_t dim, uint64_t bits, const float* parent, const float* nbrs, uint64_t cnt,
                     uint8_t* values, float* aux, uint32_t* pops) {
    return guarded([&] {
        if (!parent || !nbrs || !values || !aux || !pops || cnt == 0 || cnt > 32 || dim == 0) throw InvalidArg("bad arguments");
        if (bits != 1 && bits != 2 && bits != 4) throw InvalidArg("bits must be 1, 2 or 4");
        const size_t D = std::max<size_t>(16, next_pow2(dim));
        if (D > 2048) throw InvalidArg("unsupported dimension");
        HIP_CHECK(hipSetDevice(device));
        const size_t n = cnt + 1;
        std::vector<float> x(n * D, 0.0f);
        std::memcpy(x.data(), parent, dim * 4);
        for (uint64_t e = 0; e < cnt; ++e) std::memcpy(&x[(e + 1) * D], nbrs + e * dim, dim * 4);
        std::vector<uint32_t> nbr(n * 32, kInvalidNode);
        for (uint64_t e = 0; e < cnt; ++e) nbr[e] = (uint32_t)(e + 1);
        Rotation rot;
        rot.init(D, 42);
        const DevLayout L = make_dev_layout((uint32_t)D, (uint32_t)bits);
        DevBuf<float> d_x(n * D), d_signs(3 * D), d_aux(n * 32 * 3);
        DevBuf<uint32_t> d_nbr(n * 32), d_pops(n * 32 * 2);
        DevBuf<uint8_t> d_blocks(n * L.stride), d_vals(n * 32 * D);
        HIP_CHECK(hipMemcpy(d_x.p, x.data(), n * D * 4, hipMemcpyHostToDevice));
// ... 432 lines not shown
        r.query = query; r.k = kk; r.ids = ids; r.dist = dist; r.m = m;
        h->coal.submit(r,
                       [&](int slot, const std::vector<SearchReq*>& group) { launch_search_group(h, h->leaders[slot], group); },
                       [&](int slot, uint32_t index, SearchReq& me) { wait_search_one(h, h->leaders[slot], index, me); });
    });
    if (rc != CPH_OK) return rc;
    return r.rc == CPH_OK ? CPH_OK : fail(r.rc, r.err);
}

int cph_encode_query(cph_index* h, const float* query, uint8_t* lut, float* coeffs) {
    return guarded([&] {
        std::lock_guard<std::mutex> lk(h->mu);
        require_finalized(h);
        h->use_device();
        hipStream_t st = own_stream(h);
        BatchSet& s = next_set(h, st);
        stage_queries(h, s, upload_queries(h, s, query, 1, st), 1, st);
        HIP_CHECK(hipEventRecord(s.ev_done, st));
        s.used = true;
        HIP_CHECK(hipStreamSynchronize(st));
        const uint32_t D = h->D, PW = h->L.PW;
        std::vector<uint32_t> masks(PW * 4);
        QueryHeader hd;
        HIP_CHECK(hipMemcpy(masks.data(), s.d_qmasks.p, PW * 16, hipMemcpyDeviceToHost));
        HIP_CHECK(hipMemcpy(&hd, s.d_qhdr.p, sizeof(hd), hipMemcpyDeviceToHost));
        std::vector<uint8_t> qu(D);
        for (uint32_t d = 0; d < D; ++d) {
            uint8_t u = 0;
            for (int j = 0; j < 4; ++j) u |= (uint8_t)(((masks[(d / 32) * 4 + j] >> (d % 32)) & 1u) << j);
            qu[d] = u;
        }
        qu_to_lut(qu.data(), D, lut);
        coeffs[0] = hd.A; coeffs[1] = hd.B; coeffs[2] = hd.C;
    });
}

int cph_entry_point(cph_index* h, const float* query, uint32_t* entry) {
    return guarded([&] {
        std::lock_guard<std::mutex> lk(h->mu);
        require_finalized(h);
        h->use_device();
        hipStream_t st = own_stream(h);
        BatchSet& s = next_set(h, st);
        stage_queries(h, s, upload_queries(h, s, query, 1, st), 1, st);
        HIP_CHECK(hipEventRecord(s.ev_done, st));
        s.used = true;
        HIP_CHECK(hipStreamSynchronize(st));
        QueryHeader hd;
        HIP_CHECK(hipMemcpy(&hd, s.d_qhdr.p, sizeof(hd), hipMemcpyDeviceToHost));
        *entry = hd.entry;
    });
}

int cph_fastscan_block(cph_index* h, const uint8_t* lut, const float* qparams, uint32_t vertex,
                       float dist_qp_sq, float worst, int nn_full, uint32_t* sums, uint32_t* msb,
                       float* est, float* lower, float* lower_stage1) {
    return guarded([&] {
        std::lock_guard<std::mutex> lk(h->mu);
        require_finalized(h);
        if (vertex >= h->host.n) throw InvalidArg("vertex out of range");
        h->use_device();
        const uint32_t D = h->D, PW = h->L.PW;
        std::vector<uint8_t> qu(D);
        lut_to_qu(lut, D, qu.data());
        std::vector<uint32_t> masks(PW * 4);
        qu_to_masks(qu.data(), D, masks.data());
        DevBuf<uint4> d_mask;
        DevBuf<uint32_t> d_u;
        DevBuf<float> d_f;
        d_mask.alloc(PW);
        d_u.alloc(64);
        d_f.alloc(96);
        HIP_CHECK(hipMemcpy(d_mask.p, masks.data(), PW * 16, hipMemcpyHostToDevice));
        BlockHookArgs a{};
        a.blk = h->d_blocks.p + (size_t)vertex * h->L.stride;
        a.L = h->L;
        a.qmask = d_mask.p;
        a.qp = QP{qparams[0], qparams[1], qparams[2], qparams[3], qparams[4], qparams[5], qparams[6]};
        a.dqp = dist_qp_sq;
        a.worst = worst;
        a.nn_full = nn_full;
        a.sums = d_u.p; a.msb = d_u.p + 32;
        a.est = d_f.p; a.lower = d_f.p + 32; a.lower1 = d_f.p + 64;
        CPH_LAUNCH(block_hook_kernel, h->bits, D, dim3(1), dim3(64), (size_t)PW * 16, nullptr, a);
        HIP_CHECK(hipDeviceSynchronize());
        uint32_t hu[64];
        float hf[96];
        HIP_CHECK(hipMemcpy(hu, d_u.p, sizeof(hu), hipMemcpyDeviceToHost));
        HIP_CHECK(hipMemcpy(hf, d_f.p, sizeof(hf), hipMemcpyDeviceToHost));
        std::memcpy(sums, hu, 128); std::memcpy(msb, hu + 32, 128);
        std::memcpy(est, hf, 128); std::memcpy(lower, hf + 32, 128);
        std::memcpy(lower_stage1, hf + 64, 128);
    });
}

int cph_exact_l2(cph_index* h, const float* query, const uint32_t* ids, uint64_t n, float* out) {
    return guarded([&] {
        std::lock_guard<std::mutex> lk(h->mu);
        require_finalized(h);
        if (n == 0) return;
        for (uint64_t i = 0; i < n; ++i)
            if (ids[i] >= h->host.n) throw InvalidArg("id out of range");
        h->use_device();
        const uint32_t D = h->D;
        std::vector<float> buf(D, 0.0f);
        std::memcpy(buf.data(), query, h->dim * sizeof(float));
        DevBuf<float> d_q, d_out;
        DevBuf<uint32_t> d_i;
        d_q.alloc(D); d_out.alloc(n); d_i.alloc(n);
        HIP_CHECK(hipMemcpy(d_q.p, buf.data(), D * 4, hipMemcpyHostToDevice));
        HIP_CHECK(hipMemcpy(d_i.p, ids, n * 4, hipMemcpyHostToDevice));
        const uint32_t grid = (uint32_t)std::min<uint64_t>((n + 7) / 8, 1024);
        hipLaunchKernelGGL(exact_l2_hook_kernel, dim3(grid), dim3(64), (size_t)D * 4, nullptr, d_q.p,
                           h->d_raw.p, h->d_norm.p, d_i.p, n, D, d_out.p);
        HIP_CHECK(hipGetLastError());
        HIP_CHECK(hipMemcpy(out, d_out.p, n * 4, hipMemcpyDeviceToHost));
    });
}

}

extern "C" {

int cph_host_rewrite_index(const char* path_in, const char* path_out) {
    return guarded([&] {
        if (!path_in || !path_out) throw InvalidArg("null argument");
        FILE* f = std::fopen(path_in, "rb");
        if (!f) throw std::runtime_error(std::string("Cannot open file for reading: ") + path_in);
        uint8_t hdr[28];
        const size_t got = std::fread(hdr, 1, sizeof(hdr), f);
        std::fclose(f);
        if (got != sizeof(hdr)) throw std::runtime_error(std::string("Read error or truncated file: ") + path_in);
        uint32_t D, bw, dim;
        std::memcpy(&D, hdr + 12, 4); std::memcpy(&bw, hdr + 20, 4); std::memcpy(&dim, hdr + 24, 4);
        HostIndex hi;
        hi.load(path_in, D, bw, dim);
        hi.save(path_out);
    });
}

int cph_host_repack_block(uint32_t D, uint32_t bits, const uint8_t* ref_block, uint8_t* dev_block,
                          uint64_t* dev_bytes, uint8_t* ref_roundtrip) {
    return guarded([&] {
        if (bits != 1 && bits != 2 && bits != 4) throw InvalidArg("bits must be 1, 2 or 4");
        if (D < 16 || D > 2048 || (D & (D - 1))) throw InvalidArg("D must be a power of two in 16..2048");
        const DevLayout L = make_dev_layout(D, bits);
        const RefLayout RL = make_ref_layout(D, bits);
        repack_ref_to_dev(ref_block, RL, L, dev_block);
        if (dev_bytes) *dev_bytes = L.stride;
        if (ref_roundtrip) repack_dev_to_ref(dev_block, L, RL, ref_roundtrip);
    });
}

int cph_host_encode_query(uint64_t dim, const float* query, uint8_t* lut, float* coeffs, uint32_t* masks) {
    return guarded([&] {
        const size_t D = std::max<size_t>(16, next_pow2(dim));
        if (dim == 0 || D > 2048) throw InvalidArg("unsupported dimension");
        Rotation rot;
        rot.init(D, 42);
        std::vector<float> buf(D, 0.0f);
        std::memcpy(buf.data(), query, dim * sizeof(float));
        EncodedQuery eq;
        encode_query(rot, buf.data(), eq);
        if (lut) qu_to_lut(eq.qu.data(), D, lut);
        if (coeffs) { coeffs[0] = eq.A; coeffs[1] = eq.B; coeffs[2] = eq.C; }
        if (masks) qu_to_masks(eq.qu.data(), D, masks);
    });
}

}

struct cph_stream {
    int device = 0;
    DevLayout L{};
    RefLayout RL{};
    uint64_t n_blocks = 0;
    DevBuf<uint8_t> d_blocks;
    DevBuf<uint4> d_mask;
    DevBuf<float> d_sink;
    std::vector<uint8_t> lut;
    QP qp{};
    float dqp = 0.0f;
    int num_cus = 256;
    hipEvent_t ev0 = nullptr, ev1 = nullptr;
};

namespace {

__device__ __forceinline__ uint32_t mix32(uint64_t x) {
    x ^= x >> 33; x *= 0xff51afd7ed558ccdULL; x ^= x >> 33; x *= 0xc4ceb9fe1a85ec53ULL; x ^= x >> 33;
    return (uint32_t)x;
}

__global__ __launch_bounds__(64) void stream_fill_kernel(uint8_t* blocks, uint64_t n_blocks,
                                                         DevLayout L, uint64_t seed) {
    const int lane = threadIdx.x;
    const int i = lane & 31, h = lane >> 5;
    for (uint64_t b = blockIdx.x; b < n_blocks; b += gridDim.x) {
        uint8_t* blk = blocks + b * L.stride;
        uint32_t pc[4] = {0, 0, 0, 0};
        const uint32_t T = L.BW * L.PW;
        const uint32_t valid_bits = L.D >= 32 ? 32 : L.D;
        const uint32_t vmask = valid_bits == 32 ? 0xFFFFFFFFu : ((1u << valid_bits) - 1u);
        for (uint32_t t = h; t < T; t += 2) {
            const uint32_t plane = t / L.PW;
            uint32_t v = mix32(seed ^ (b * 0x9E3779B97F4A7C15ULL) ^ ((uint64_t)(t * 32 + i) << 20)) & vmask;
            size_t off;
            if (L.wide) {
                const uint32_t ck = t / 4, e = t % 4;
                const uint32_t hh = (L.NH == 2) ? ck / L.CPL : 0;
                const uint32_t k = (L.NH == 2) ? ck % L.CPL : ck;
                off = ((size_t)(k * L.NH * 32 + hh * 32 + i) * 16 + e * 4);
            } else {
                off = ((size_t)t * 32 + i) * 4;
            }
            *reinterpret_cast<uint32_t*>(blk + off) = v;
            const uint32_t c = __popc(v);
            if (plane == 0) pc[0] += c; else if (plane == 1) pc[1] += c;
            else if (plane == 2) pc[2] += c; else pc[3] += c;
        }
        for (int p = 0; p < 4; ++p) pc[p] += __shfl_xor(pc[p], 32);
        if (lane < 32) {
            uint32_t wp = 0;
            for (uint32_t p = 0; p < L.BW; ++p) wp += pc[p] << (L.BW - 1 - p);
            const uint32_t r0 = mix32(seed ^ (b * 1315423911ULL) ^ (0x1000 + i));
            const uint32_t r1 = mix32(seed ^ (b * 2654435761ULL) ^ (0x2000 + i));
            const uint32_t r2 = mix32(seed ^ (b * 40503ULL) ^ (0x3000 + i));
            float nop = 1.0f + 19.0f * (r0 >> 8) * (1.0f / 16777216.0f);
            float ipqo = 0.5f + 0.4f * (r1 >> 8) * (1.0f / 16777216.0f);
            float ipcp = -0.5f + (r2 >> 8) * (1.0f / 16777216.0f);
            uint4 aux = make_uint4(__float_as_uint(nop), __float_as_uint(ipqo), __float_as_uint(ipcp),
                                   (pc[0] & 0xFFFFu) | ((wp & 0xFFFFu) << 16));
            reinterpret_cast<uint4*>(blk + L.aux_off)[i] = aux;
            reinterpret_cast<uint32_t*>(blk + L.ids_off)[i] = mix32(seed ^ b ^ ((uint64_t)i << 40)) >> 1;
            if (lane == 0) *reinterpret_cast<uint32_t*>(blk + L.count_off) = 32u;
        }
    }
}

void stream_launch(cph_stream* s, float* out_est, float* out_lower, uint64_t first, uint64_t count,
                   hipStream_t st) {
    StreamArgs a{};
    a.blocks = s->d_blocks.p;
    a.n_blocks = s->n_blocks;
    a.L = s->L;
    a.qmask = s->d_mask.p;
    a.qp = s->qp;
    a.dqp = s->dqp;
    a.sink = s->d_sink.p;
    a.out_est = out_est;
    a.out_lower = out_lower;
    a.first = first;
    a.count = count;
    static const int mult = getenv("CPH_STREAM_GRID_MULT") ? atoi(getenv("CPH_STREAM_GRID_MULT")) : 32;
    const uint32_t grid = (uint32_t)s->num_cus * mult;
    static const bool pair = !(getenv("CPH_STREAM_PAIR") && atoi(getenv("CPH_STREAM_PAIR")) == 0);
    if (pair && s->L.D == 128 && s->L.BW <= 2) {
        if (s->L.BW == 1) hipLaunchKernelGGL((fastscan_stream_pair_kernel<1>), dim3(grid), dim3(256), 64, st, a);
        else hipLaunchKernelGGL((fastscan_stream_pair_kernel<2>), dim3(grid), dim3(256), 64, st, a);
        HIP_CHECK(hipGetLastError());
        return;
    }
    const uint32_t dsel = s->L.D == 128 ? 128u : 0u;
    CPH_LAUNCH(fastscan_stream_kernel, s->L.BW, dsel, dim3(grid), dim3(256), (size_t)s->L.PW * 16, st, a);
}

}

extern "C" {

int cph_fastscan_stream_create(int device, uint32_t D, uint32_t bits, uint64_t n_blocks,
                               uint64_t seed, cph_stream** out, uint64_t* block_bytes) {
    return guarded([&] {
        *out = nullptr;
        if (bits != 1 && bits != 2 && bits != 4) throw InvalidArg("bits must be 1, 2 or 4");
        if (D < 16 || D > 2048 || (D & (D - 1))) throw InvalidArg("D must be a power of two in 16..2048");
        int ndev = 0;
        if (hipGetDeviceCount(&ndev) != hipSuccess || ndev <= 0)
            throw std::runtime_error("No HIP device available: the MI355X path has no CPU fallback.");
        HIP_CHECK(hipSetDevice(device));
        auto s = std::unique_ptr<cph_stream>(new cph_stream());
        s->device = device;
        s->L = make_dev_layout(D, bits);
        s->RL = make_ref_layout(D, bits);
        s->n_blocks = n_blocks;
        hipDeviceProp_t prop;
        if (hipGetDeviceProperties(&prop, device) == hipSuccess) s->num_cus = prop.multiProcessorCount;
        s->d_blocks.alloc(n_blocks * s->L.stride + 64);
        s->d_mask.alloc(s->L.PW);
        s->d_sink.alloc((size_t)s->num_cus * 64 * 4);
        HIP_CHECK(hipMemset(s->d_sink.p, 0, s->d_sink.n * sizeof(float)));
        hipLaunchKernelGGL(stream_fill_kernel, dim3(s->num_cus * 16), dim3(64), 0, nullptr,
                           s->d_blocks.p, n_blocks, s->L, seed);
        HIP_CHECK(hipGetLastError());
        std::mt19937_64 rng(seed * 7919 + 13);
        std::normal_distribution<float> nd(0.0f, 1.0f);
        std::vector<float> q(D);
        for (auto& x : q) x = nd(rng);
        Rotation rot;
        rot.init(D, 42);
        EncodedQuery eq;
        encode_query(rot, q.data(), eq);
        s->lut.resize(D / 4 * 16);
        qu_to_lut(eq.qu.data(), D, s->lut.data());
        std::vector<uint32_t> masks(s->L.PW * 4);
        qu_to_masks(eq.qu.data(), D, masks.data());
        HIP_CHECK(hipMemcpy(s->d_mask.p, masks.data(), masks.size() * 4, hipMemcpyHostToDevice));
        s->qp = QP{eq.A, eq.B, eq.C, 1.0f, 0.0f, 0.0f, 0.05f};
        s->dqp = 140.0f;
        HIP_CHECK(hipEventCreate(&s->ev0));
        HIP_CHECK(hipEventCreate(&s->ev1));
        HIP_CHECK(hipDeviceSynchronize());
        if (block_bytes) *block_bytes = s->L.stride;
        *out = s.release();
    });
}

int cph_fastscan_stream_run(cph_stream* s, int reps, double* avg_ms, double* checksum) {
    return guarded([&] {
        HIP_CHECK(hipSetDevice(s->device));
        if (reps < 1) reps = 1;
        hipStream_t st = nullptr;
        HIP_CHECK(hipEventRecord(s->ev0, st));
        for (int r = 0; r < reps; ++r) stream_launch(s, nullptr, nullptr, 0, 0, st);
        HIP_CHECK(hipEventRecord(s->ev1, st));
        HIP_CHECK(hipEventSynchronize(s->ev1));
        float ms = 0.0f;
        HIP_CHECK(hipEventElapsedTime(&ms, s->ev0, s->ev1));
        if (avg_ms) *avg_ms = (double)ms / reps;
        if (checksum) {
            std::vector<float> sink(s->d_sink.n);
            HIP_CHECK(hipMemcpy(sink.data(), s->d_sink.p, sink.size() * 4, hipMemcpyDeviceToHost));
            double t = 0.0;
            for (float x : sink) t += x;
            *checksum = t;
        }
    });
}

int cph_fastscan_stream_export(cph_stream* s, uint64_t first, uint64_t count, uint8_t* ref_blocks,
                               uint8_t* lut, float* qparams, float* dist_qp_sq) {
    return guarded([&] {
        HIP_CHECK(hipSetDevice(s->device));
        if (first + count > s->n_blocks) throw InvalidArg("block range out of bounds");
        if (count && ref_blocks) {
            std::vector<uint8_t> dev(count * s->L.stride);
            HIP_CHECK(hipMemcpy(dev.data(), s->d_blocks.p + first * s->L.stride, dev.size(),
                                hipMemcpyDeviceToHost));
            parallel_for(count, 1024, [&](size_t lo, size_t hi) {
                for (size_t b = lo; b < hi; ++b)
                    repack_dev_to_ref(&dev[b * s->L.stride], s->L, s->RL, ref_blocks + b * s->RL.nb_bytes);
            });
        }
        if (lut) std::memcpy(lut, s->lut.data(), s->lut.size());
        if (qparams) {
            qparams[0] = s->qp.A; qparams[1] = s->qp.B; qparams[2] = s->qp.C;
            qparams[3] = s->qp.affine_a; qparams[4] = s->qp.affine_b; qparams[5] = s->qp.floor;
            qparams[6] = s->qp.slack;
        }
        if (dist_qp_sq) *dist_qp_sq = s->dqp;
    });
}

int cph_fastscan_stream_eval(cph_stream* s, uint64_t first, uint64_t count, float* est, float* lower) {
    return guarded([&] {
        HIP_CHECK(hipSetDevice(s->device));
        if (first + count > s->n_blocks) throw InvalidArg("block range out of bounds");
        if (!count) return;
        DevBuf<float> d_e, d_l;
        d_e.alloc(count * 32);
        d_l.alloc(count * 32);
        stream_launch(s, d_e.p, d_l.p, first, count, nullptr);
        HIP_CHECK(hipMemcpy(est, d_e.p, count * 128, hipMemcpyDeviceToHost));
        HIP_CHECK(hipMemcpy(lower, d_l.p, count * 128, hipMemcpyDeviceToHost));
    });
}

int cph_fastscan_stream_destroy(cph_stream* s) {
    return guarded([&] {
        if (!s) return;
        (void)hipSetDevice(s->device);
        if (s->ev0) (void)hipEventDestroy(s->ev0);
        if (s->ev1) (void)hipEventDestroy(s->ev1);
        delete s;
    });
}

}
```

### rabitq-ann-search_amd/csrc/device_build.h

```cpp
#pragma once
#include <hip/hip_runtime.h>

#include <cstdint>

#include "cph_core.h"
#include "device_encode.h"
#include "device_fastscan.h"

namespace cph {
namespace build {

__global__ __launch_bounds__(256) void row_norms_kernel(const float* __restrict__ x, uint64_t n, uint32_t D,
                                                        uint32_t dim, float* __restrict__ out) {
    const uint64_t i = (uint64_t)blockIdx.x * blockDim.x + threadIdx.x;
    if (i >= n) return;
    const float* v = x + i * D;
    float s = 0.0f;
    for (uint32_t j = 0; j < dim; ++j) s = __fmaf_rn(v[j], v[j], s);
    out[i] = s;
}

__global__ __launch_bounds__(64) void gather_rows_kernel(const float* __restrict__ src, const uint32_t* __restrict__ ids,
                                                         uint64_t rows, uint32_t D, float* __restrict__ out) {
    for (uint64_t r = blockIdx.x; r < rows; r += gridDim.x) {
// ... 448 lines not shown
    uint32_t* sel = reinterpret_cast<uint32_t*>(cd + kSelCap);
    float* selerr = reinterpret_cast<float*>(sel + 32);
    const int lane = threadIdx.x;
    const uint32_t D = a.D, R = a.R;
    const float FMAX = 3.402823466e+38f;
    for (uint64_t row = blockIdx.x; row < a.rows; row += gridDim.x) {
        const uint32_t vtx = a.row_ids ? a.row_ids[row] : (uint32_t)row;
        __syncthreads();
        for (uint32_t d = lane; d < D; d += 64) cvec[d] = a.x[(size_t)vtx * D + d];
        uint32_t id0 = kInvalidNode, id1 = kInvalidNode;
        if (lane < 32) id0 = a.fwd[row * 32 + lane];
        uint64_t rb = 0, re = 0;
        if (a.rev_off) { rb = a.rev_off[row]; re = a.rev_off[row + 1]; }
        __syncthreads();
        float d0 = FMAX, d1 = FMAX;
        auto exact_dists = [&]() {
            for (int base = 0; base < kSelCap; base += 8) {
                const int slot = base + (lane >> 3);
                const uint32_t cand = base < 64 ? (uint32_t)__shfl((int)id0, slot) : (uint32_t)__shfl((int)id1, slot - 64);
                const bool have = cand != kInvalidNode && cand != vtx;
                const float dd = group_l2sq8(cvec, a.x + (size_t)(have ? cand : vtx) * D, D, lane & 7);
                if ((lane & 7) == 0) { cd[slot] = have ? dd : FMAX; cid[slot] = have ? cand : kInvalidNode; }
            }
            __syncthreads();
            id0 = cid[lane]; d0 = cd[lane];
            id1 = cid[lane + 64]; d1 = cd[lane + 64];
        };
        auto rank_sort = [&]() {
            uint32_t r0 = 0, r1 = 0;
            bool dup0 = false, dup1 = false;
#pragma unroll 4
            for (int j = 0; j < 64; ++j) {
                const float ej0 = __uint_as_float((uint32_t)__builtin_amdgcn_readlane((int)__float_as_uint(d0), j));
                const uint32_t ij0 = (uint32_t)__builtin_amdgcn_readlane((int)id0, j);
                const float ej1 = __uint_as_float((uint32_t)__builtin_amdgcn_readlane((int)__float_as_uint(d1), j));
                const uint32_t ij1 = (uint32_t)__builtin_amdgcn_readlane((int)id1, j);
                const bool b00 = ej0 < d0 || (ej0 == d0 && (ij0 < id0 || (ij0 == id0 && j < lane)));
                const bool b01 = ej0 < d1 || (ej0 == d1 && (ij0 < id1 || ij0 == id1));
                const bool b10 = ej1 < d0 || (ej1 == d0 && ij1 < id0);
                const bool b11 = ej1 < d1 || (ej1 == d1 && (ij1 < id1 || (ij1 == id1 && j < lane)));
                r0 += (b00 ? 1u : 0u) + (b10 ? 1u : 0u);
                r1 += (b01 ? 1u : 0u) + (b11 ? 1u : 0u);
                dup0 |= (ij0 == id0 && b00) || (ij1 == id0 && b10);
                dup1 |= (ij0 == id1 && b01) || (ij1 == id1 && b11);
            }
            __syncthreads();
            cid[r0] = dup0 ? kInvalidNode : id0; cd[r0] = dup0 ? FMAX : d0;
            cid[r1] = dup1 ? kInvalidNode : id1; cd[r1] = dup1 ? FMAX : d1;
            __syncthreads();
            id0 = cid[lane]; d0 = cd[lane];
            id1 = cid[lane + 64]; d1 = cd[lane + 64];
        };
        if (re - rb <= 96) {
            const uint64_t take = re - rb;
            if (lane >= 32 && (uint64_t)(lane - 32) < take) {
                const uint32_t r = a.rev[rb + (lane - 32)];
                id0 = a.row_ids ? a.row_ids[r] : r;
            }
            if ((uint64_t)(lane + 32) < take) {
                const uint32_t r = a.rev[rb + lane + 32];
                id1 = a.row_ids ? a.row_ids[r] : r;
            }
            exact_dists();
            rank_sort();
        } else {
            while (rb < re) {
                const uint64_t take = re - rb < 64 ? re - rb : 64;
                id1 = kInvalidNode;
                if ((uint64_t)lane < take) {
                    const uint32_t r = a.rev[rb + lane];
                    id1 = a.row_ids ? a.row_ids[r] : r;
                }
                rb += take;
                exact_dists();
                rank_sort();
                rank_sort();
            }
            id1 = kInvalidNode;
            d1 = FMAX;
        }
        rank_sort();
        const uint32_t C = (uint32_t)__popcll(__ballot(id0 != kInvalidNode)) + (uint32_t)__popcll(__ballot(id1 != kInvalidNode));
        uint32_t nsel = 0;
        if (C <= R) {
            if ((uint32_t)lane < C && lane < 32) a.out[row * 32 + lane] = id0;
            if ((uint32_t)lane >= C && lane < 32) a.out[row * 32 + lane] = kInvalidNode;
            if (lane == 0) a.out_cnt[row] = C;
            continue;
        }
        float la = a.alpha * __builtin_sqrtf((float)C / (float)R);
        const float amax = a.alpha_max > 0.0f ? a.alpha_max : 2.0f * a.alpha;
        la = la < 1.0f ? 1.0f : (la > amax ? amax : la);
        unsigned long long taken_lo = 0, taken_hi = 0;
        for (uint32_t ci = 0; ci < C && nsel < R; ++ci) {
            const uint32_t c = cid[ci];
            const float dcq = cd[ci];
            const float errc = a.err ? a.err[c] : 0.0f;
            __syncthreads();
            for (uint32_t d = lane; d < D; d += 64) cvec[d] = a.x[(size_t)c * D + d];
            __syncthreads();
            bool occluded = false;
            for (uint32_t base = 0; base < nsel; base += 8) {
                const uint32_t j = base + (lane >> 3);
                const bool have = j < nsel;
                const uint32_t e = have ? sel[j] : c;
                const float dce = group_l2sq8(cvec, a.x + (size_t)e * D, D, lane & 7);
                const float thr = la * dcq + (errc + (have ? selerr[j] : 0.0f)) - (la - 1.0f) * a.tau;
                occluded |= have && dce < thr;
            }
            if (!__any(occluded)) {
                if (lane == 0) { sel[nsel] = c; selerr[nsel] = errc; }
                if (ci < 64) taken_lo |= 1ull << ci; else taken_hi |= 1ull << (ci - 64);
                ++nsel;
            }
        }
        __syncthreads();
        for (uint32_t ci = 0; ci < C && nsel < R; ++ci) {
            const bool taken = ci < 64 ? (taken_lo >> ci) & 1ull : (taken_hi >> (ci - 64)) & 1ull;
            if (taken) continue;
            if (lane == 0) sel[nsel] = cid[ci];
            ++nsel;
        }
        __syncthreads();
        if (lane < 32) a.out[row * 32 + lane] = (uint32_t)lane < nsel ? sel[lane] : kInvalidNode;
        if (lane == 0) a.out_cnt[row] = nsel;
    }
}

struct CalibArgs {
    const uint8_t* blocks;
    const float* raw;
    DevLayout L;
    uint64_t n;
    const float* queries;
    const uint4* qmasks;
    const QueryHeader* qhdr;
    const uint32_t* start;
    uint32_t ns;
    float* rec;
    uint32_t* rec_cnt;
    float* dqp_out;
};

template <int BW>
__global__ __launch_bounds__(64) void calib_kernel(CalibArgs a) {
    extern __shared__ __align__(16) unsigned char smem[];
    const uint32_t D = a.L.D, PW = a.L.PW;
    uint4* qm = reinterpret_cast<uint4*>(smem);
    float* qv = reinterpret_cast<float*>(smem + (size_t)PW * 16);
    float* pv = qv + D;
    const int lane = threadIdx.x;
    for (uint32_t s = blockIdx.x; s < a.ns; s += gridDim.x) {
        __syncthreads();
        for (uint32_t w = lane; w < PW; w += 64) qm[w] = a.qmasks[(size_t)s * PW + w];
        for (uint32_t d = lane; d < D; d += 64) qv[d] = a.queries[(size_t)s * D + d];
        __syncthreads();
        uint32_t parent = a.start[s];
        float best = group_l2sq8(qv, a.raw + (size_t)parent * D, D, lane & 7);
        best = __shfl(best, 0);
        {
            const uint8_t* blk = a.blocks + (size_t)parent * a.L.stride;
            const uint32_t nid = reinterpret_cast<const uint32_t*>(blk + a.L.ids_off)[lane & 31];
            float cand = 3.402823466e+38f;
            uint32_t cand_id = kInvalidNode, cand_pos = 64;
            for (int base = 0; base < 32; base += 8) {
                const int pos = base + (lane >> 3);
                const uint32_t nb = (uint32_t)__shfl((int)nid, pos);
                const bool have = nb != kInvalidNode;
                const float dd = group_l2sq8(qv, a.raw + (size_t)(have ? nb : parent) * D, D, lane & 7);
                if (have && dd < cand) { cand = dd; cand_id = nb; cand_pos = pos; }
            }
            for (int o = 8; o < 64; o <<= 1) {
                const float od = __shfl_xor(cand, o);
                const uint32_t oi = __shfl_xor(cand_id, o);
                const uint32_t op = __shfl_xor(cand_pos, o);
                if (od < cand || (od == cand && op < cand_pos)) { cand = od; cand_id = oi; cand_pos = op; }
            }
            cand = __shfl(cand, 0); cand_id = (uint32_t)__shfl((int)cand_id, 0);
            if (cand_id != kInvalidNode && cand < best) { best = cand; parent = cand_id; }
        }
        const uint8_t* blk = a.blocks + (size_t)parent * a.L.stride;
        for (uint32_t d = lane; d < D; d += 64) pv[d] = a.raw[(size_t)parent * D + d];
        __syncthreads();
        LaneEst v;
        load_block<BW, 0>(blk, a.L, qm, lane, v);
        const uint32_t nid = reinterpret_cast<const uint32_t*>(blk + a.L.ids_off)[lane & 31];
        const QueryHeader hd = a.qhdr[s];
        float ipa;
        if constexpr (BW == 1) {
            ipa = hd.A * (float)v.nbit + hd.B * (float)v.pop + hd.C;
        } else {
            const float invK = 1.0f / (float)((1u << BW) - 1);
            ipa = hd.A * invK * (float)v.nbit + hd.B * invK * (float)v.wpop + hd.C;
        }
        const float ipc = ipa - v.ip_cp;
        const float ipq = __builtin_fabsf(v.ip_qo) > kEpsMedium ? __builtin_fabsf(v.ip_qo) : kEpsMedium;
        const float nop = v.nop > kEpsSmall ? v.nop : kEpsSmall;
        float tip = 0.0f, dqo = 0.0f;
        for (int base = 0; base < 32; base += 8) {
            const int pos = base + (lane >> 3);
            const uint32_t nb = (uint32_t)__shfl((int)nid, pos);
            const bool have = nb != kInvalidNode;
            const float* ov = a.raw + (size_t)(have ? nb : parent) * D;
            float t = 0.0f, l2 = 0.0f;
            for (uint32_t d = lane & 7; d < D; d += 8) {
                const float o = ov[d], q = qv[d], p = pv[d];
                t = __fmaf_rn(q - p, o - p, t);
                l2 = __fmaf_rn(q - o, q - o, l2);
            }
            t = group_reduce8(t);
            l2 = group_reduce8(l2);
            const float tt = __shfl(t, (lane & 31) >= base && (lane & 31) < base + 8 ? ((lane & 31) - base) * 8 : 0);
            const float ll = __shfl(l2, (lane & 31) >= base && (lane & 31) < base + 8 ? ((lane & 31) - base) * 8 : 0);
            if ((lane & 31) >= base && (lane & 31) < base + 8) { tip = tt; dqo = ll; }
        }
        const bool valid = lane < 32 && nid != kInvalidNode;
        if (lane < 32) {
            float* r = a.rec + ((size_t)s * 32 + lane) * 6;
            r[0] = nop; r[1] = ipc; r[2] = ipq; r[3] = valid ? tip / nop : 0.0f; r[4] = dqo; r[5] = v.ip_qo;
        }
        const uint32_t nvalid = (uint32_t)__popcll(__ballot(valid));
        if (lane == 0) { a.rec_cnt[s] = nvalid; a.dqp_out[s] = best; }
    }
}

}
}
```

### rabitq-ann-search_amd/csrc/device_fastscan.h

```cpp
#pragma once
#include <hip/hip_runtime.h>

#include "cph_core.h"

namespace cph {

struct QP {
    float A, B, C, affine_a, affine_b, floor, slack;
};

struct LaneEst {
    uint32_t nbit;
    uint32_t msb;
    uint32_t msb2;
    float nop, ip_qo, ip_cp;
    uint32_t pop, wpop;
};

__device__ __forceinline__ float vmaxf(float a, float b) { return a > b ? a : b; }
__device__ __forceinline__ float vminf(float a, float b) { return a < b ? a : b; }

__device__ __forceinline__ uint32_t bcnt_acc(uint32_t x, uint32_t acc) {
    uint32_t r;
    asm("v_bcnt_u32_b32 %0, %1, %2" : "=v"(r) : "v"(x), "v"(acc));
    return r;
}

__device__ __forceinline__ void acc4(uint32_t c, uint4 q, uint32_t& a0, uint32_t& a1,
                                     uint32_t& a2, uint32_t& a3) {
    a0 = bcnt_acc(c & q.x, a0);
    a1 = bcnt_acc(c & q.y, a1);
    a2 = bcnt_acc(c & q.z, a2);
    a3 = bcnt_acc(c & q.w, a3);
}

__device__ __forceinline__ void half_pair(uint32_t x, uint32_t& lo, uint32_t& hi) {
    auto r = __builtin_amdgcn_permlane32_swap(x, x, false, false);
    lo = r[0];
    hi = r[1];
}

template <int BW, int SD>
__device__ __forceinline__ void block_sums(const uint8_t* __restrict__ blk, const DevLayout& L,
                                           const uint4* qm, int lane, uint32_t& nbit,
                                           uint32_t& msb, uint32_t& msb2) {
    const int h = lane >> 5;
    const uint32_t PW = SD ? (SD >= 32 ? SD / 32 : 1) : L.PW;
    const bool wide = SD ? (SD >= 128) : (L.wide != 0);
    if (wide) {
        const uint4* cp = reinterpret_cast<const uint4*>(blk) + lane;
        if constexpr (BW >= 2) {
            constexpr int PPH = BW / 2;
            const uint32_t G = PW >> 2;
            uint32_t S[PPH];
#pragma unroll
            for (int pl = 0; pl < PPH; ++pl) {
                uint32_t a0 = 0, a1 = 0, a2 = 0, a3 = 0;
#pragma unroll 2
                for (uint32_t g = 0; g < G; ++g) {
                    uint4 c = cp[(pl * G + g) * 64];
                    acc4(c.x, qm[4 * g + 0], a0, a1, a2, a3);
                    acc4(c.y, qm[4 * g + 1], a0, a1, a2, a3);
                    acc4(c.z, qm[4 * g + 2], a0, a1, a2, a3);
                    acc4(c.w, qm[4 * g + 3], a0, a1, a2, a3);
                }
                S[pl] = a0 + 2 * a1 + 4 * a2 + 8 * a3;
            }
            uint32_t part = 0;
#pragma unroll
            for (int pl = 0; pl < PPH; ++pl) part += S[pl] << (BW - 1 - (h * PPH + pl));
            uint32_t plo, phi, s0, s0hi;
            half_pair(part, plo, phi);
            nbit = plo + phi;
            half_pair(S[0], s0, s0hi);
            if constexpr (BW == 2) {
                msb = s0;
                msb2 = 2 * s0 + s0hi;
            } else {
                uint32_t s1, s1hi;
                half_pair(S[1], s1, s1hi);
                msb = s0;
                msb2 = 2 * s0 + s1;
            }
        } else {
            const uint32_t NH = SD ? ((SD / 32) / 4 >= 2 ? 2 : 1) : L.NH;
            const uint32_t CPL = SD ? ((SD / 32) / 4 / NH) : L.CPL;
            uint32_t a0 = 0, a1 = 0, a2 = 0, a3 = 0;
            if ((uint32_t)h < NH) {
                const uint4* cq = reinterpret_cast<const uint4*>(blk) + (lane & (NH * 32 - 1));
#pragma unroll 2
                for (uint32_t k = 0; k < CPL; ++k) {
                    uint4 c = cq[k * NH * 32];
                    uint32_t w0 = (h * CPL + k) * 4;
                    acc4(c.x, qm[w0 + 0], a0, a1, a2, a3);
                    acc4(c.y, qm[w0 + 1], a0, a1, a2, a3);
                    acc4(c.z, qm[w0 + 2], a0, a1, a2, a3);
                    acc4(c.w, qm[w0 + 3], a0, a1, a2, a3);
                }
            }
            uint32_t s = a0 + 2 * a1 + 4 * a2 + 8 * a3, slo, shi;
            half_pair(s, slo, shi);
            s = (NH == 2) ? slo + shi : slo;
            nbit = msb = msb2 = s;
        }
    } else {
        const uint32_t* cw = reinterpret_cast<const uint32_t*>(blk) + (lane & 31);
        uint32_t S[BW];
#pragma unroll
        for (int b = 0; b < BW; ++b) {
            uint32_t a0 = 0, a1 = 0, a2 = 0, a3 = 0;
            for (uint32_t w = 0; w < PW; ++w) acc4(cw[(b * PW + w) * 32], qm[w], a0, a1, a2, a3);
            S[b] = a0 + 2 * a1 + 4 * a2 + 8 * a3;
        }
        uint32_t t = 0;
#pragma unroll
        for (int b = 0; b < BW; ++b) t += S[b] << (BW - 1 - b);
        nbit = t;
        msb = S[0];
        if constexpr (BW >= 2) msb2 = 2 * S[0] + S[1]; else msb2 = S[0];
    }
}

template <int BW, int SD>
struct BlockLoads {
    static constexpr bool kStatic = (SD >= 128);
    static constexpr int kT = kStatic ? BW * (SD / 32) : 4;
    static constexpr int kNH = (kT / 4 >= 2) ? 2 : 1;
    static constexpr int kCPL = kStatic ? kT / 4 / kNH : 1;
    uint4 c[kCPL];
    uint4 aux;

    __device__ __forceinline__ void issue_static(const uint8_t* __restrict__ blk, int lane) {
        static_assert(kStatic, "static D only");
        const uint4* cp = reinterpret_cast<const uint4*>(blk) + (lane & (kNH * 32 - 1));
#pragma unroll
        for (int k = 0; k < kCPL; ++k) c[k] = cp[k * kNH * 32];
        aux = reinterpret_cast<const uint4*>(blk + StaticLayout<BW, SD>::kAuxOff)[lane & 31];
    }

    __device__ __forceinline__ void issue(const uint8_t* __restrict__ blk, const DevLayout& L, int lane) {
        if constexpr (kStatic) {
            const uint4* cp = reinterpret_cast<const uint4*>(blk) + (lane & (kNH * 32 - 1));
#pragma unroll
            for (int k = 0; k < kCPL; ++k) c[k] = cp[k * kNH * 32];
        }
        aux = reinterpret_cast<const uint4*>(blk + L.aux_off)[lane & 31];
    }

    __device__ __forceinline__ void retire() {
        if constexpr (kStatic) {
#pragma unroll
            for (int k = 0; k < kCPL; ++k)
                asm volatile("" : "+v"(c[k].x), "+v"(c[k].y), "+v"(c[k].z), "+v"(c[k].w));
        }
        asm volatile("" : "+v"(aux.x), "+v"(aux.y), "+v"(aux.z), "+v"(aux.w));
    }

    __device__ __forceinline__ void reduce(const uint8_t* __restrict__ blk, const DevLayout& L,
                                           const uint4* qm, int lane, LaneEst& o) {
        if constexpr (kStatic) {
            const int h = lane >> 5;
            constexpr int PW = SD / 32;
            if constexpr (BW >= 2) {
                constexpr int PPH = BW / 2;
                constexpr int G = PW / 4;
                uint32_t S[PPH];
#pragma unroll
                for (int pl = 0; pl < PPH; ++pl) {
                    uint32_t a0 = 0, a1 = 0, a2 = 0, a3 = 0;
#pragma unroll
                    for (int g = 0; g < G; ++g) {
                        const uint4 cc = c[pl * G + g];
                        acc4(cc.x, qm[4 * g + 0], a0, a1, a2, a3);
                        acc4(cc.y, qm[4 * g + 1], a0, a1, a2, a3);
                        acc4(cc.z, qm[4 * g + 2], a0, a1, a2, a3);
                        acc4(cc.w, qm[4 * g + 3], a0, a1, a2, a3);
                    }
                    S[pl] = a0 + 2 * a1 + 4 * a2 + 8 * a3;
                }
                uint32_t part = 0;
#pragma unroll
                for (int pl = 0; pl < PPH; ++pl) part += S[pl] << (BW - 1 - (h * PPH + pl));
                uint32_t plo, phi, s0, s0hi;
                half_pair(part, plo, phi);
                o.nbit = plo + phi;
                half_pair(S[0], s0, s0hi);
                if constexpr (BW == 2) {
                    o.msb = s0;
                    o.msb2 = 2 * s0 + s0hi;
                } else {
                    uint32_t s1, s1hi;
                    half_pair(S[1], s1, s1hi);
                    o.msb = s0;
                    o.msb2 = 2 * s0 + s1;
                }
            } else {
                uint32_t a0 = 0, a1 = 0, a2 = 0, a3 = 0;
                if (h < kNH) {
#pragma unroll
                    for (int k = 0; k < kCPL; ++k) {
                        const uint4 cc = c[k];
                        const uint32_t w0 = (h * kCPL + k) * 4;
                        acc4(cc.x, qm[w0 + 0], a0, a1, a2, a3);
                        acc4(cc.y, qm[w0 + 1], a0, a1, a2, a3);
                        acc4(cc.z, qm[w0 + 2], a0, a1, a2, a3);
                        acc4(cc.w, qm[w0 + 3], a0, a1, a2, a3);
                    }
                }
                uint32_t sv = a0 + 2 * a1 + 4 * a2 + 8 * a3, slo, shi;
                half_pair(sv, slo, shi);
                sv = (kNH == 2) ? slo + shi : slo;
                o.nbit = o.msb = o.msb2 = sv;
            }
        } else {
            block_sums<BW, SD>(blk, L, qm, lane, o.nbit, o.msb, o.msb2);
        }
        o.nop = __uint_as_float(aux.x);
        o.ip_qo = __uint_as_float(aux.y);
        o.ip_cp = __uint_as_float(aux.z);
        o.pop = aux.w & 0xFFFFu;
        o.wpop = aux.w >> 16;
    }
};

template <int BW, int SD>
__device__ __forceinline__ void load_block(const uint8_t* __restrict__ blk, const DevLayout& L,
                                           const uint4* qm, int lane, LaneEst& o) {
    BlockLoads<BW, SD> b;
    b.issue(blk, L, lane);
    b.reduce(blk, L, qm, lane, o);
}

struct TailLanes {
    bool any;
    bool mine;
};
__device__ __forceinline__ TailLanes tail_lanes(bool valid, int lane) {
    const uint32_t count = (uint32_t)__popc((uint32_t)(__ballot(valid) & 0xFFFFFFFFull));
    TailLanes t;
    t.any = (count & 7u) != 0u;
    t.mine = (uint32_t)(lane & 31) >= (count & ~7u);
    return t;
}
__device__ __forceinline__ TailLanes no_tail() { return TailLanes{false, false}; }
__device__ __forceinline__ float ip_approx_est(float A, float s, float B, float pc, float C, const TailLanes& t) {
    float r = __fmaf_rn(A, s, __fmaf_rn(B, pc, C));
    if (__builtin_expect(t.any, 0)) {
        const float u = __fmaf_rn(B, pc, A * s) + C;
        r = t.mine ? u : r;
    }
    return r;
}
__device__ __forceinline__ float ip_approx_msb(float A, float s, float B, float pc, float C, const TailLanes& t) {
    float r = __fmaf_rn(A, s, __fmaf_rn(B, pc, C));
    if (__builtin_expect(t.any, 0)) {
        const float u = __fmaf_rn(A, s, B * pc) + C;
        r = t.mine ? u : r;
    }
    return r;
}

__device__ __forceinline__ void est_and_lower(const QP& q, float ip_est_approx, float ip_lb_approx,
                                              float nop, float ip_qo, float ip_cp, float dqp,
                                              float sqrt_dqp, float& est, float& lower) {
    float ipq = vmaxf(ip_qo, q.floor);
    bool good = ipq > kEpsMedium;
    float e = good ? (ip_est_approx - ip_cp) / ipq : 0.0f;
    e = __fmaf_rn(q.affine_a, e, q.affine_b);
    float dist = __fmaf_rn(nop, nop, dqp);
    dist = __fmaf_rn(-(2.0f * nop), e, dist);
    est = vmaxf(dist, 0.0f);
    float m = good ? (ip_lb_approx - ip_cp) / ipq : 0.0f;
    m = __fmaf_rn(q.affine_a, m, q.affine_b);
    float cosu = (m + q.slack) / vmaxf(sqrt_dqp, kEpsMedium);
    cosu = vminf(vmaxf(cosu, -1.0f), 1.0f);
    float lo = __fmaf_rn(nop, nop, dqp);
    lo = __fmaf_rn(-((2.0f * nop) * sqrt_dqp), cosu, lo);
    lo = vmaxf(lo, 0.0f);
    lower = good ? lo : 0.0f;
}

template <int BW>
__device__ __forceinline__ float stage1_lower(const QP& q, const LaneEst& v, float dqp,
                                              float sqrt_dqp) {
    if (dqp < kEpsSmall) return 0.0f;
    const float invk = (BW >= 2) ? (1.0f / 3.0f) : 1.0f;
    float A = q.A * invk, B = q.B * invk;
    float ipq = (v.ip_qo < q.floor) ? q.floor : v.ip_qo;
    if (ipq <= kEpsMedium) return 0.0f;
    float ipa = __fmaf_rn(B, (float)v.pop, A * (float)v.msb2) + q.C;
    float e = (ipa - v.ip_cp) / ipq;
    e = __fmaf_rn(e, q.affine_a, q.affine_b);
    float c = (e + q.slack) / sqrt_dqp;
    c = (c < -1.0f) ? -1.0f : ((1.0f < c) ? 1.0f : c);
    float lo = __fmaf_rn(-c, (v.nop + v.nop) * sqrt_dqp, __fmaf_rn(v.nop, v.nop, dqp));
    return (lo < 0.0f) ? 0.0f : lo;
}

template <int BW>
__device__ __forceinline__ void stage2_est(const QP& q, const LaneEst& v, float dqp,
                                           float sqrt_dqp, float& est, float& lower,
                                           const TailLanes& tl) {
    if (dqp < kEpsSmall) {
        est = __fmaf_rn(v.nop, v.nop, dqp);
        lower = 0.0f;
        return;
    }
    if constexpr (BW == 1) {
        float ipa = ip_approx_est(q.A, (float)v.nbit, q.B, (float)v.pop, q.C, tl);
        est_and_lower(q, ipa, ipa, v.nop, v.ip_qo, v.ip_cp, dqp, sqrt_dqp, est, lower);
    } else {
        constexpr float K = (float)((1u << BW) - 1);
        constexpr float invK = 1.0f / K;
        float An = q.A * invK, Bn = q.B * invK;
        float ipn = ip_approx_est(An, (float)v.nbit, Bn, (float)v.wpop, q.C, tl);
        float ipm = ip_approx_msb(q.A, (float)v.msb, q.B, (float)v.pop, q.C, tl);
        est_and_lower(q, ipn, ipm, v.nop, v.ip_qo, v.ip_cp, dqp, sqrt_dqp, est, lower);
    }
}

template <int BW>
__device__ __forceinline__ void lower_bounds_split(const QP& q, const LaneEst& v, float dqp, float sqrt_dqp,
                                                   int lane, float& lo_stage1, float& lo_stage2, const TailLanes& tl) {
    static_assert(BW >= 2, "N-bit path");
    const float invk = 1.0f / 3.0f;
    const float n1 = __fmaf_rn(q.B * invk, (float)v.pop, (q.A * invk) * (float)v.msb2) + q.C;
    const float n2 = ip_approx_msb(q.A, (float)v.msb, q.B, (float)v.pop, q.C, tl);
    const float num = lane >= 32 ? n2 : n1;
    const float ipq = (v.ip_qo < q.floor) ? q.floor : v.ip_qo;
    float e = (num - v.ip_cp) / ipq;
    e = __fmaf_rn(e, q.affine_a, q.affine_b);
    float c = (e + q.slack) / sqrt_dqp;
    c = (c < -1.0f) ? -1.0f : ((1.0f < c) ? 1.0f : c);
    float lo = __fmaf_rn(-c, (v.nop + v.nop) * sqrt_dqp, __fmaf_rn(v.nop, v.nop, dqp));
    lo = (lo < 0.0f) ? 0.0f : lo;
    lo = (ipq > kEpsMedium) ? lo : 0.0f;
    uint32_t a, b;
    half_pair(__float_as_uint(lo), a, b);
    lo_stage1 = __uint_as_float(a);
    lo_stage2 = __uint_as_float(b);
}

template <int BW>
__device__ __forceinline__ float stage2_est_only(const QP& q, const LaneEst& v, float dqp, const TailLanes& tl, bool tiny) {
    static_assert(BW >= 2, "N-bit path");
    if (tiny) return __fmaf_rn(v.nop, v.nop, dqp);
    constexpr float K = (float)((1u << BW) - 1);
    constexpr float invK = 1.0f / K;
// ... 119 lines not shown
```

### rabitq-ann-search_amd/csrc/device_search.h

```cpp
#pragma once
#include <cstddef>
#include <hip/hip_runtime.h>

#include "cph_core.h"
#include "device_fastscan.h"

namespace cph {

struct Result {
    uint32_t id;
    float dist;
};

struct SearchArgs {
    const uint8_t* blocks;
    const float* raw;
    const float* norm_sq;
    uint64_t n;
    DevLayout L;
    uint32_t flags;
    const float* queries;
    const uint4* qmasks;
    const QueryHeader* qhdr;
    const uint32_t* todo;
// ... 371 lines not shown
    const int lane = opaque_lane(lane_in);
    const uint32_t hp = hole + 1;
    const uint32_t depth = 31u - (uint32_t)__builtin_clz(hp);
    const uint32_t t = (uint32_t)lane + 1;
    const bool on = t <= depth;
    uint4 e = v;
    bool down = false;
    if (hp <= kBeamPaged) {
        const uint32_t lvl = depth - 7u;
        const uint32_t pbase = ((hp >> lvl) - 128u) * kPageDwords;
        const uint32_t rl = (hp & ((1u << lvl) - 1u)) | (1u << lvl);
        if (on) {
            if (t < lvl) e = h.pload(pbase + 3u * (rl >> t)); else e = h.lds((hp >> t) - 1);
            down = Beam::before(Beam::key_of(e), Beam::key_of(v));
        }
        const unsigned long long stop = ~__ballot(down);
        const uint32_t m = (uint32_t)__builtin_ctzll(stop);
        auto put_anc = [&](uint32_t s, uint4 val) {
            if (s < lvl) h.pstore(pbase + 3u * (rl >> s), val); else h.lds_put((hp >> s) - 1, val);
        };
        if (t <= m) put_anc(t - 1, e);
        if ((uint32_t)lane == m) put_anc(m, v);
        return;
    }
    const uint32_t pt = on ? (hp >> t) - 1 : 0u;
    if (on) {
        e = h.raw(pt);
        down = Beam::before(Beam::key_of(e), Beam::key_of(v));
    }
    const unsigned long long stop = ~__ballot(down);
    const uint32_t m = (uint32_t)__builtin_ctzll(stop);
    if (t <= m) h.put((hp >> (t - 1)) - 1, e);
    if ((uint32_t)lane == m) h.put((hp >> m) - 1, v);
}

__device__ __forceinline__ void nn_push_wave(const NnLds& w, Result* h, uint32_t& size, uint32_t k, uint32_t id, float dist,
                                             float top, int lane_in) {
#ifndef CPH_NO_LAUNDER_NN
    const int lane = opaque_lane(lane_in);
#else
    const int lane = lane_in;
#endif
    const uint2 r = make_uint2(id, __float_as_uint(dist));
    if (size < k) {
        if (size < kWaveHeapMax) {
            heap_push_wave(w, size, r, lane);
        } else {
            if (lane == 0) nn_sift_up(h, size, 0, Result{id, dist});
            __builtin_amdgcn_wave_barrier();
        }
        ++size;
    } else if (dist < top) {
        if (size <= kWaveHeapMax) {
            if (size > 1) heap_pop_wave(w, size, lane);
            heap_push_wave(w, size - 1, r, lane);
        } else {
            if (lane == 0) {
                nn_adjust(h, 0, size - 1, h[size - 1]);
                nn_sift_up(h, size - 1, 0, Result{id, dist});
            }
            __builtin_amdgcn_wave_barrier();
        }
    }
}

__device__ __forceinline__ uint32_t bcast_u32(uint32_t v) {
    return (uint32_t)__builtin_amdgcn_readfirstlane((int)v);
}
__device__ __forceinline__ float bcast_f32(float v) {
    return __uint_as_float((uint32_t)__builtin_amdgcn_readfirstlane((int)__float_as_uint(v)));
}

constexpr uint32_t kLdsTail = 128 + 64 + 128 + 16 + 80;
__host__ __device__ inline uint32_t search_vec_bytes(uint32_t D, bool static_d) { return static_d ? D * 4 : 512; }
__host__ __device__ inline bool search_static_d(uint32_t D) { return D == 128 || D == 1024; }
__host__ __device__ inline size_t search_lds_bytes(uint32_t D, uint32_t PW, uint32_t k) {
    return (size_t)PW * 16 + (size_t)D * 4 + search_vec_bytes(D, search_static_d(D)) + kLdsTail +
           (((size_t)k * 8 + 15) & ~(size_t)15) + 16 * (kBeamLds + 1);
}

typedef __attribute__((address_space(3))) void lds_void;
__device__ __forceinline__ uint32_t lds_offset(const void* p) {
    return (uint32_t)__builtin_amdgcn_readfirstlane((int)(uint32_t)(uintptr_t)(lds_void*)p);
}
__device__ __forceinline__ void lds_dma16(const void* g, uint32_t lds_off) {
    asm volatile("s_mov_b32 m0, %1\n\ts_nop 0\n\tglobal_load_lds_dwordx4 %0, off" ::"v"(g), "s"(lds_off) : "memory");
}

#ifndef CPH_SEARCH_WAVES_PER_SIMD
#define CPH_SEARCH_WAVES_PER_SIMD 5
#endif
#ifndef CPH_SEARCH_WAVES_PER_SIMD_128
#define CPH_SEARCH_WAVES_PER_SIMD_128 6
#endif
#ifndef CPH_SEARCH_WAVES_PER_SIMD_1024
#define CPH_SEARCH_WAVES_PER_SIMD_1024 2
#endif
#ifndef CPH_SEARCH_WAVES_PER_SIMD_128_NARROW
#define CPH_SEARCH_WAVES_PER_SIMD_128_NARROW CPH_SEARCH_WAVES_PER_SIMD_128
#endif
__host__ __device__ constexpr int search_waves_per_simd(int sd, int bw) {
    return sd == 128 ? (bw <= 2 ? CPH_SEARCH_WAVES_PER_SIMD_128_NARROW : CPH_SEARCH_WAVES_PER_SIMD_128)
                     : (sd == 1024 ? CPH_SEARCH_WAVES_PER_SIMD_1024 : CPH_SEARCH_WAVES_PER_SIMD);
}
template <int BW, int SD, bool PF = true, bool FILT = false>
__global__ __launch_bounds__(64, search_waves_per_simd(SD, BW)) void search_kernel(SearchArgs a) {
    extern __shared__ __align__(16) unsigned char smem[];
    const int lane = threadIdx.x;
    const int li = lane & 31;
    const uint32_t D = SD ? SD : a.L.D;
    const uint32_t PW = SD ? (SD >= 32 ? SD / 32 : 1) : a.L.PW;
    const uint32_t k = a.k;
    uint4* qm = reinterpret_cast<uint4*>(smem);
    float* qv = reinterpret_cast<float*>(smem + (size_t)PW * 16);
    unsigned char* fixed = smem + (size_t)PW * 16 + (size_t)D * 4;
    float* s_vec = reinterpret_cast<float*>(fixed);
    constexpr uint32_t vsz = SD >= 128 ? (uint32_t)SD * 4u : 512u;
    float* s_exact = reinterpret_cast<float*>(fixed + vsz);
    uint8_t* s_list = fixed + vsz + 128;
    float* s_slack = reinterpret_cast<float*>(fixed + vsz + 192);
    double* s_ratio = reinterpret_cast<double*>(fixed + vsz + 320);
    unsigned long long* s_tot = reinterpret_cast<unsigned long long*>(fixed + vsz + 336);
    if (lane < 10) s_tot[lane] = 0ull;
    Result* nn = reinterpret_cast<Result*>(fixed + vsz + kLdsTail);
    NnLds nnw;
    nnw.l = (lds_u32x2*)(fixed + vsz + kLdsTail);
    const uint32_t beam_off = PW * 16 + D * 4 + vsz + kLdsTail + ((k * 8 + 15) & ~15u);
    lds_u32x4* s_beam = (lds_u32x4*)(smem + beam_off);

    const uint32_t vec_off = __builtin_amdgcn_groupstaticsize() + PW * 16 + D * 4;
    const uint32_t slot = blockIdx.x;
    uint32_t* bm = CPH_COLD(bitmaps) + (size_t)slot * CPH_COLD(bm_words);
    uint32_t* logi = CPH_COLD(log_ids) + (size_t)slot * a.cap;
    Beam heap;
    heap.l = s_beam;
    heap.gp = CPH_COLD(beam_pages) + (size_t)slot * kBeamPagesDwords;
    heap.gt = CPH_COLD(beam_tail) + (size_t)slot * beam_tail_dwords(a.cap);
    const float FMAX = 3.402823466e+38f;
    if (lane < kMaxSlack) s_slack[lane] = a.sc.slack[lane];

    const uint32_t* nq_dev = CPH_COLD(nq_dev);
    const uint32_t nq = nq_dev ? *nq_dev : CPH_COLD(nq);
    for (;;) {
        uint32_t t = 0;
        if (lane == 0) t = atomicAdd(CPH_COLD(counter), 1u);
        t = bcast_u32(t);
        if (t >= nq) break;
        const uint32_t* todo = CPH_COLD(todo);
        const uint32_t qi = todo ? todo[t] : t;

        {
            const uint4* qmasks = CPH_COLD(qmasks);
            const float* queries = CPH_COLD(queries);
            for (uint32_t w = lane; w < PW; w += 64) qm[w] = qmasks[(size_t)qi * PW + w];
            for (uint32_t d = lane; d < D; d += 64) qv[d] = queries[(size_t)qi * D + d];
        }
        const QueryHeader hd = CPH_COLD(qhdr)[qi];
        __syncthreads();

        QP qp;
        qp.A = hd.A; qp.B = hd.B; qp.C = hd.C;
        {
            float af_a = a.sc.affine_a, af_b = a.sc.affine_b, fl = a.sc.ip_qo_floor;
            asm volatile("" : "+s"(af_a), "+s"(af_b), "+s"(fl));
            qp.affine_a = af_a; qp.affine_b = af_b; qp.floor = fl;
        }
        qp.slack = s_slack[0];
        const float gamma = a.sc.gamma;

        float qnorm;
        {
            float c = 0.0f;
            for (uint32_t i = lane & 7; i < D; i += 8) c = __fmaf_rn(qv[i], qv[i], c);
            qnorm = bcast_f32(group_reduce8_lo(c));
        }

        uint32_t beam_size = 0, nn_size = 0;
        float gamma_q = gamma;
        if (lane == 0) { s_ratio[0] = 0.0; s_ratio[1] = 0.0; nn[0].dist = FMAX; }
        uint32_t ratio_count = 0;
        uint32_t log_count = 0;
        int slack_batch = 0;
        bool overflow = false, wipe = false, stage2_redo = false;
        uint32_t st_exp = 0, st_exact = 0, st_new = 0, st_push = 0, st_skip = 0, st_allseen = 0;
        uint32_t st_undecided = 0;
#ifdef CPH_TRAFFIC_STATS
        unsigned long long trf[8] = {0, 0, 0, 0, 0, 0, 0, 0};
#endif
#ifdef CPH_PHASE_TIMERS
        unsigned long long tph[8] = {0, 0, 0, 0, 0, 0, 0, 0};
        unsigned long long tlast = clock64();
#define CPH_TICK_(i) do { unsigned long long tn_ = clock64(); tph[i] += tn_ - tlast; tlast = tn_; } while (0)
#if CPH_PHASE_TIMERS + 0 == 2
#define CPH_TICK(i) do {} while (0)
#define CPH_TICKF(i) CPH_TICK_(i)
#else
#define CPH_TICK(i) CPH_TICK_(i)
#define CPH_TICKF(i) do {} while (0)
#endif
#else
#define CPH_TICK(i) do {} while (0)
#define CPH_TICKF(i) do {} while (0)
#endif

        {
            const uint32_t ep = hd.entry;
            const float enorm = a.norm_sq[ep];
            float dot = group_dot8_lo(qv, a.raw + (size_t)ep * D, D, lane & 7);
            float ex = exact_from_dot(qnorm, enorm, dot);
            st_exact++;
            if (lane == 0) {
                logi[0] = ep;
                heap.put(0, beam_pack(BeamEntry{ex, 0.0f, ep}));
                atomicOr(&bm[ep >> 5], 1u << (ep & 31));
            }
            beam_size = 1;
            log_count = 1;
        }
        __syncthreads();

        for (;;) {
            CPH_TICK(7);
            if (beam_size == 0) break;
            uint32_t cur_id;
            float worst_pop;
            auto pop_beam = [&](uint32_t size) {
#ifdef CPH_TRAFFIC_STATS
                trf[5] += size;
                if (size > trf[6]) trf[6] = size;
                if (size > kBeamLds) { trf[0]++; uint32_t lv = 31u - (uint32_t)__builtin_clz(size); trf[1] += (lv - 7 + 4) / 5; }
                if (size > 8191) trf[7]++;
#endif
                if (size > 1) {
                    if (size <= kBeamLds) heap_pop_wave(heap, size, lane);
                    else beam_pop_hybrid(heap, size, lane);
                }
            };
            {
                const uint4 topv = heap.lds(0);
                const float worst = nn[0].dist;
                cur_id = bcast_u32(topv.z);
                const float cur_est = __uint_as_float(topv.x);
                const float cur_lower = __uint_as_float(topv.y);
                uint32_t verdict = 2;
                if (nn_size >= k && cur_est >= gamma_q * worst) verdict = 0;
                else if (nn_size >= k && cur_lower > worst) verdict = 1;
                verdict = bcast_u32(verdict);
                if (verdict == 0) break;
                if (verdict == 1) {
                    pop_beam(beam_size);
                    --beam_size;
                    continue;
                }
                worst_pop = bcast_f32(worst);
            }
            CPH_TICK(0);

            constexpr bool kStaticLayout = SD >= 128 && PF;
            const uint32_t blk_stride = kStaticLayout ? StaticLayout<BW, SD>::kStride : a.L.stride;
            const uint32_t blk_ids_off = kStaticLayout ? StaticLayout<BW, SD>::kIdsOff : a.L.ids_off;
            const uint8_t* blk = a.blocks + (size_t)cur_id * blk_stride;
            const float* vrow = a.raw + (size_t)cur_id * D;
#ifndef CPH_NO_LOOPHEAD_WAIT
            __builtin_amdgcn_s_waitcnt(0x0F70);
#endif
            if constexpr (SD == 128) {
                if (lane < 32) lds_dma16(vrow + 4 * lane, vec_off);
                __builtin_amdgcn_sched_barrier(0);
            } else if constexpr (SD > 128) {
#pragma unroll
                for (int c = 0; c < SD / 256; ++c) lds_dma16(vrow + 4 * lane + 256 * c, vec_off + 1024 * c);
                __builtin_amdgcn_sched_barrier(0);
            }
            const float norm_ld = a.norm_sq[cur_id];
            const uint32_t nid_ld = reinterpret_cast<const uint32_t*>(blk + blk_ids_off)[li];
            uint32_t allow_cur = 0;
            if constexpr (FILT) allow_cur = CPH_COLD(allow)[cur_id >> 5];
            BlockLoads<BW, SD> bl;
#ifdef CPH_NO_PROBE_FIRST
            constexpr bool kProbeFirst = false;
#else
            constexpr bool kProbeFirst = PF && SD >= 128;
#endif
            if constexpr (kProbeFirst) {
#pragma unroll
                for (int kk = 0; kk < BlockLoads<BW, SD>::kCPL; ++kk) bl.c[kk] = make_uint4(0u, 0u, 0u, 0u);
                bl.aux = make_uint4(0u, 0u, 0u, 0u);
            } else {
                bl.issue(blk, a.L, lane);
            }
            __builtin_amdgcn_sched_barrier(0);
            CPH_TICKF(0);
            uint32_t touch = 0;
            if (beam_size > kBeamLds) {
                const uint32_t depth = 31u - (uint32_t)__builtin_clz(beam_size);
                const uint32_t j = (uint32_t)lane + 1u;
                const bool on = j <= 5u && 7u + j < depth;
                const uint32_t sh = on ? depth - 7u - j : 0u;
                const uint32_t rj = ((beam_size >> sh) & ((1u << (j & 7u)) - 1u)) | (1u << (j & 7u));
                const uint32_t pb = ((beam_size >> (depth - 7u)) - 128u) * kPageDwords;
                touch = heap.gp[on ? pb + 3u * rj : 0u];
            }
            pop_beam(beam_size);
            --beam_size;
            __builtin_amdgcn_sched_barrier(0);
            CPH_TICKF(1);
            uint32_t nid = nid_ld;
// ... 338 lines not shown
```

### rabitq-ann-search_amd/csrc/device_stream.h

```cpp
#pragma once
#include <hip/hip_runtime.h>

#include "cph_core.h"
#include "device_fastscan.h"

namespace cph {

struct StreamArgs {
    const uint8_t* blocks;
    uint64_t n_blocks;
    DevLayout L;
    const uint4* qmask;
    QP qp;
    float dqp;
    float* sink;
    float* out_est;
    float* out_lower;
    uint64_t first, count;
};

template <int BW, int SD>
__global__ __launch_bounds__(256) void fastscan_stream_kernel(StreamArgs a) {
    extern __shared__ __align__(16) unsigned char smem[];
    uint4* qm = reinterpret_cast<uint4*>(smem);
    const uint32_t PW = SD ? (SD >= 32 ? SD / 32 : 1) : a.L.PW;
    for (uint32_t w = threadIdx.x; w < PW; w += blockDim.x) qm[w] = a.qmask[w];
    __syncthreads();
    const int lane = threadIdx.x & 63;
    const uint64_t wave = (uint64_t)blockIdx.x * (blockDim.x >> 6) + (threadIdx.x >> 6);
    const uint64_t nwaves = (uint64_t)gridDim.x * (blockDim.x >> 6);
    const float sq = __builtin_sqrtf(a.dqp);
    float acc = 0.0f;
    const uint64_t lo = a.out_est ? a.first : 0;
    const uint64_t hi = a.out_est ? a.first + a.count : a.n_blocks;
    BlockLoads<BW, SD> cur, nxt;
    uint32_t cur_id = 0, nxt_id = 0;
    uint64_t b = lo + wave;
    if (b < hi) {
        const uint8_t* blk = a.blocks + b * a.L.stride;
        cur.issue(blk, a.L, lane);
        cur_id = reinterpret_cast<const uint32_t*>(blk + a.L.ids_off)[lane & 31];
    }
    for (; b < hi; b += nwaves) {
        const uint64_t bn = b + nwaves;
        if (bn < hi) {
            const uint8_t* nblk = a.blocks + bn * a.L.stride;
            nxt.issue(nblk, a.L, lane);
            nxt_id = reinterpret_cast<const uint32_t*>(nblk + a.L.ids_off)[lane & 31];
        }
        const uint8_t* blk = a.blocks + b * a.L.stride;
        LaneEst v;
        cur.reduce(blk, a.L, qm, lane, v);
        float est, lower;
        const TailLanes tl = tail_lanes(cur_id != kInvalidNode, lane);
        if constexpr (BW == 1) {
            stage2_est<1>(a.qp, v, a.dqp, sq, est, lower, tl);
            acc += est + lower;
        } else {
            float lo1 = stage1_lower<BW>(a.qp, v, a.dqp, sq);
            stage2_est<BW>(a.qp, v, a.dqp, sq, est, lower, tl);
            acc += est + lower + lo1;
        }
        if (cur_id == kInvalidNode) acc = 0.0f;
        if (a.out_est && lane < 32) {
            a.out_est[(b - a.first) * 32 + lane] = est;
            a.out_lower[(b - a.first) * 32 + lane] = lower;
        }
        cur = nxt;
        cur_id = nxt_id;
    }
    for (int o = 1; o < 64; o <<= 1) acc += __shfl_xor(acc, o);
    if (lane == 0 && !a.out_est) a.sink[wave] = acc;
}

template <int BW>
__global__ __launch_bounds__(256) void fastscan_stream_pair_kernel(StreamArgs a) {
    static_assert(BW == 1 || BW == 2, "pair kernel: narrow codes only");
    extern __shared__ __align__(16) unsigned char smem[];
    uint4* qm = reinterpret_cast<uint4*>(smem);
    for (uint32_t w = threadIdx.x; w < 4; w += blockDim.x) qm[w] = a.qmask[w];
    __syncthreads();
    const int lane = threadIdx.x & 63;
    const int h = lane >> 5, i = lane & 31;
    const uint64_t wave = (uint64_t)blockIdx.x * (blockDim.x >> 6) + (threadIdx.x >> 6);
    const uint64_t nwaves = (uint64_t)gridDim.x * (blockDim.x >> 6);
    const float sq = __builtin_sqrtf(a.dqp);
    float acc = 0.0f;
    const uint64_t lo = a.out_est ? a.first : 0;
    const uint64_t hi = a.out_est ? a.first + a.count : a.n_blocks;
    struct Loads { uint4 c[BW]; uint4 aux; uint32_t id; };
    auto issue = [&](uint64_t b, Loads& L) {
        const uint8_t* blk = a.blocks + b * a.L.stride;
        const uint4* cp = reinterpret_cast<const uint4*>(blk) + i;
#pragma unroll
        for (int k = 0; k < BW; ++k) L.c[k] = cp[k * 32];
        L.aux = reinterpret_cast<const uint4*>(blk + a.L.aux_off)[i];
        L.id = reinterpret_cast<const uint32_t*>(blk + a.L.ids_off)[i];
    };
    Loads cur{}, nxt{};
    uint64_t b = lo + 2 * wave + h;
    if (b < hi) issue(b, cur);
    for (; b - h < hi; b += 2 * nwaves) {
        const uint64_t bn = b + 2 * nwaves;
        if (bn < hi) issue(bn, nxt);
        const bool live = b < hi;
        LaneEst v;
        uint32_t S[BW];
#pragma unroll
        for (int k = 0; k < BW; ++k) {
            uint32_t a0 = 0, a1 = 0, a2 = 0, a3 = 0;
            acc4(cur.c[k].x, qm[0], a0, a1, a2, a3);
            acc4(cur.c[k].y, qm[1], a0, a1, a2, a3);
            acc4(cur.c[k].z, qm[2], a0, a1, a2, a3);
            acc4(cur.c[k].w, qm[3], a0, a1, a2, a3);
            S[k] = a0 + 2 * a1 + 4 * a2 + 8 * a3;
        }
        if constexpr (BW == 1) { v.nbit = v.msb = v.msb2 = S[0]; }
        else { v.nbit = 2 * S[0] + S[1]; v.msb = S[0]; v.msb2 = 2 * S[0] + S[1]; }
        v.nop = __uint_as_float(cur.aux.x);
        v.ip_qo = __uint_as_float(cur.aux.y);
        v.ip_cp = __uint_as_float(cur.aux.z);
        v.pop = cur.aux.w & 0xFFFFu;
        v.wpop = cur.aux.w >> 16;
        float est, lower;
        TailLanes tl;
        {
            const unsigned long long vm = __ballot(live && cur.id != kInvalidNode);
            const uint32_t count = (uint32_t)__popc((uint32_t)(h ? vm >> 32 : vm & 0xFFFFFFFFull));
            tl.any = __any((count & 7u) != 0u);
            tl.mine = (uint32_t)i >= (count & ~7u);
        }
        if constexpr (BW == 1) {
            stage2_est<1>(a.qp, v, a.dqp, sq, est, lower, tl);
            if (live) acc += est + lower;
        } else {
            const float lo1 = stage1_lower<BW>(a.qp, v, a.dqp, sq);
            stage2_est<BW>(a.qp, v, a.dqp, sq, est, lower, tl);
            if (live) acc += est + lower + lo1;
        }
        if (live && cur.id == kInvalidNode) acc = 0.0f;
        if (a.out_est && live) {
            a.out_est[(b - a.first) * 32 + i] = est;
            a.out_lower[(b - a.first) * 32 + i] = lower;
        }
        cur = nxt;
    }
    for (int o = 1; o < 64; o <<= 1) acc += __shfl_xor(acc, o);
    if (lane == 0 && !a.out_est) a.sink[wave] = acc;
}

struct BlockHookArgs {
    const uint8_t* blk;
    DevLayout L;
    const uint4* qmask;
    QP qp;
    float dqp, worst;
    int nn_full;
    uint32_t* sums;
    uint32_t* msb;
    float* est;
    float* lower;
    float* lower1;
};

template <int BW, int SD>
__global__ __launch_bounds__(64) void block_hook_kernel(BlockHookArgs a) {
    extern __shared__ __align__(16) unsigned char smem[];
    uint4* qm = reinterpret_cast<uint4*>(smem);
    const uint32_t PW = SD ? (SD >= 32 ? SD / 32 : 1) : a.L.PW;
    const int lane = threadIdx.x;
    for (uint32_t w = lane; w < PW; w += 64) qm[w] = a.qmask[w];
    __syncthreads();
    LaneEst v;
    load_block<BW, SD>(a.blk, a.L, qm, lane, v);
    const bool valid = reinterpret_cast<const uint32_t*>(a.blk + a.L.ids_off)[lane & 31] != kInvalidNode;
    const float sq = __builtin_sqrtf(a.dqp);
    float est, lower, lo1;
    const TailLanes tl = tail_lanes(valid, lane);
    if constexpr (BW == 1) {
        stage2_est<1>(a.qp, v, a.dqp, sq, est, lower, tl);
        lo1 = lower;
    } else {
        lo1 = stage1_lower<BW>(a.qp, v, a.dqp, sq);
        bool surv = (!a.nn_full) || (valid && lo1 < a.worst);
        if (__any(surv)) {
            stage2_est<BW>(a.qp, v, a.dqp, sq, est, lower, tl);
        } else {
            est = 3.402823466e+38f;
            lower = lo1;
        }
    }
    const int i = lane & 31;
    const bool writer = (i < 16) ? (lane < 32) : (lane >= 32);
    if (writer) {
        a.sums[i] = v.nbit;
        a.msb[i] = v.msb;
        a.est[i] = est;
        a.lower[i] = lower;
        a.lower1[i] = lo1;
    }
}

__global__ __launch_bounds__(64) void exact_l2_hook_kernel(const float* __restrict__ q,
                                                           const float* __restrict__ raw,
                                                           const float* __restrict__ norm_sq,
                                                           const uint32_t* __restrict__ ids,
                                                           uint64_t n, uint32_t D, float* out) {
    extern __shared__ __align__(16) unsigned char smem[];
    float* qv = reinterpret_cast<float*>(smem);
    const int lane = threadIdx.x;
    for (uint32_t d = lane; d < D; d += 64) qv[d] = q[d];
    __syncthreads();
    float c = 0.0f;
    for (uint32_t i = lane & 7; i < D; i += 8) c = __fmaf_rn(qv[i], qv[i], c);
    const float qnorm = group_reduce8(c);
    const int g = lane >> 3;
    for (uint64_t base = (uint64_t)blockIdx.x * 8; base < n; base += (uint64_t)gridDim.x * 8) {
        const bool have = base + g < n;
        const uint32_t id = have ? ids[base + g] : ids[0];
        float dot = group_dot8(qv, raw + (size_t)id * D, D, lane & 7);
        float ex = exact_from_dot(qnorm, norm_sq[id], dot);
        if (have && (lane & 7) == 0) out[base + g] = ex;
    }
}

}
```

### rabitq-ann-search_amd/csrc/host_index.h

```cpp
#pragma once
#include <fcntl.h>
#include <unistd.h>

#include <algorithm>
#include <cmath>
#include <cstdint>
#include <cstdio>
#include <cstring>
#include <random>
#include <stdexcept>
#include <string>
#include <vector>

#include "cph_core.h"

namespace cph {

struct UpperEdge {
    uint32_t node;
    std::vector<uint32_t> nbrs;
};

struct Rotation {
    size_t D = 0;
// ... 133 lines not shown
        return v;
    }

    SearchConsts consts() const {
        SearchConsts s{};
        s.affine_a = rd<float>(calib + 0);
        s.affine_b = rd<float>(calib + 4);
        s.ip_qo_floor = rd<float>(calib + 8);
        s.gamma_max = rd<float>(calib + 84);
        s.gamma_beta = rd<float>(calib + 88);
        s.gamma_warmup = rd<uint64_t>(calib + 96);
        std::memcpy(s.slack, calib + 108, 128);
        s.num_slack = rd<int32_t>(calib + 236);
        if (s.num_slack > kMaxSlack) s.num_slack = kMaxSlack;
        s.gamma = rd<float>(calib + 240);
        return s;
    }

    void load(const std::string& path, size_t expect_D, size_t expect_bw, size_t expect_dim) {
        FILE* f = std::fopen(path.c_str(), "rb");
        if (!f) throw std::runtime_error("Cannot open file for reading: " + path);
        struct Closer { FILE* f; ~Closer() { std::fclose(f); } } closer{f};
        auto rdn = [&](void* p, size_t b) {
            if (b && std::fread(p, 1, b, f) != b)
                throw std::runtime_error("Read error or truncated file: " + path);
        };
        uint8_t hdr[68];
        rdn(hdr, 12);
        if (rd<uint64_t>(hdr) != 0x57534E48504300ULL)
            throw std::runtime_error("Invalid magic bytes (not a CP-HNSW index file).");
        if (rd<uint32_t>(hdr + 8) != 2)
            throw std::runtime_error("Unsupported index file version: " +
                                     std::to_string(rd<uint32_t>(hdr + 8)));
        rdn(hdr + 12, 56);
        const uint32_t fD = rd<uint32_t>(hdr + 12), fR = rd<uint32_t>(hdr + 16),
                       fBW = rd<uint32_t>(hdr + 20), fdim = rd<uint32_t>(hdr + 24);
        if (fD != expect_D || fR != 32 || fBW != expect_bw)
            throw std::runtime_error(
                "Index file template parameters mismatch: file D=" + std::to_string(fD) +
                " R=" + std::to_string(fR) + " BW=" + std::to_string(fBW) + ", expected D=" +
                std::to_string(expect_D) + " R=32 BW=" + std::to_string(expect_bw));
        if (fdim != expect_dim)
            throw std::runtime_error("Index file dim=" + std::to_string(fdim) +
                                     " mismatches Index dim=" + std::to_string(expect_dim));
        if (rd<uint64_t>(hdr + 60) != 42) throw std::runtime_error("Index file rotation seed mismatch.");

        HostIndex t;
        t.D = fD; t.bw = fBW; t.dim = fdim;
        t.n = rd<uint64_t>(hdr + 28);
        t.max_level = rd<int32_t>(hdr + 36);
        t.entry = rd<uint32_t>(hdr + 40);
        t.upper_tau = rd<float>(hdr + 44);
        t.upper_alpha = rd<float>(hdr + 48);
        t.mL = rd<double>(hdr + 52);
        t.seed = rd<uint64_t>(hdr + 60);
        t.RL = make_ref_layout(t.D, t.bw);
        rdn(t.calib, 248);
        rdn(t.profile, 72);
        const size_t n = t.n;
        {
            const long here = std::ftell(f);
            std::fseek(f, 0, SEEK_END);
            const long total = std::ftell(f);
            std::fseek(f, here, SEEK_SET);
            const unsigned __int128 need = (unsigned __int128)n * (8 + t.D * 4 + t.RL.vertex_bytes) + t.dim * 4 + 4;
            if (here < 0 || total < here || need > (unsigned __int128)(total - here))
                throw std::runtime_error("Read error or truncated file: " + path);
        }
        t.centroid.resize(t.dim);  rdn(t.centroid.data(), t.dim * 4);
        t.levels.resize(n);        rdn(t.levels.data(), n * 4);
        t.norm_sq.resize(n);       rdn(t.norm_sq.data(), n * 4);
        t.raw.resize(n * t.D);     rdn(t.raw.data(), n * t.D * 4);
        t.search_data.resize(n * t.RL.vertex_bytes);
        rdn(t.search_data.data(), t.search_data.size());
        uint32_t nl = 0;
        rdn(&nl, 4);
        if (nl > 64) throw std::runtime_error("Corrupt index: too many upper layers");
        t.upper.resize(nl);
        for (uint32_t l = 0; l < nl; ++l) {
            uint32_t sz = 0;
            rdn(&sz, 4);
            if (sz > n) throw std::runtime_error("Corrupt index: upper layer larger than the index");
            t.upper[l].resize(sz);
            for (uint32_t e = 0; e < sz; ++e) {
                uint32_t cnt = 0;
                rdn(&t.upper[l][e].node, 4);
                rdn(&cnt, 4);
                if (cnt > n) throw std::runtime_error("Corrupt index: upper-layer degree out of range");
                t.upper[l][e].nbrs.resize(cnt);
                rdn(t.upper[l][e].nbrs.data(), (size_t)cnt * 4);
            }
        }
        t.validate();
        t.rot.init(t.D, t.seed);
        *this = std::move(t);
    }

    void validate() {
        has_dup_neighbors = false;
        if (n != 0 && entry != kInvalidNode && entry >= n) throw std::runtime_error("Corrupt index: entry point out of range");
        for (size_t v = 0; v < n; ++v) {
            const uint8_t* nb = &search_data[v * RL.vertex_bytes + RL.nb_off];
            uint32_t cnt = rd<uint32_t>(nb + RL.count);
            if (cnt > 32) throw std::runtime_error("Corrupt index: neighbour count > 32");
            const uint32_t* ids = reinterpret_cast<const uint32_t*>(nb + RL.ids);
            for (uint32_t i = 0; i < cnt; ++i) {
                if (ids[i] >= n) throw std::runtime_error("Corrupt index: neighbour id out of range");
                for (uint32_t j = 0; j < i; ++j)
                    if (ids[j] == ids[i]) has_dup_neighbors = true;
            }
        }
        for (auto& layer : upper)
            for (auto& e : layer) {
                if (e.node >= n) throw std::runtime_error("Corrupt index: upper-layer node out of range");
                for (uint32_t x : e.nbrs)
                    if (x >= n) throw std::runtime_error("Corrupt index: upper-layer neighbour out of range");
            }
    }

    void save(const std::string& path) const {
        AtomicFile out(path);
        auto wr = [&](const void* p, size_t b) { out.write(p, b); };
        const uint64_t magic = 0x57534E48504300ULL;
        const uint32_t version = 2, hD = (uint32_t)D, hR = 32, hBW = (uint32_t)bw, hdim = (uint32_t)dim;
        const uint64_t hn = n;
        wr(&magic, 8); wr(&version, 4); wr(&hD, 4); wr(&hR, 4); wr(&hBW, 4); wr(&hdim, 4);
        wr(&hn, 8); wr(&max_level, 4); wr(&entry, 4); wr(&upper_tau, 4); wr(&upper_alpha, 4);
        wr(&mL, 8); wr(&seed, 8);
        wr(calib, 248); wr(profile, 72);
        wr(centroid.data(), dim * 4);
        wr(levels.data(), n * 4);
        wr(norm_sq.data(), n * 4);
        wr(vec(0), n * D * 4);
        wr(search_data.data(), search_data.size());
        const uint32_t nl = (uint32_t)upper.size();
        wr(&nl, 4);
        for (const auto& layer : upper) {
            const uint32_t sz = (uint32_t)layer.size();
            wr(&sz, 4);
            for (const auto& e : layer) {
                const uint32_t cnt = (uint32_t)e.nbrs.size();
                wr(&e.node, 4); wr(&cnt, 4);
                wr(e.nbrs.data(), (size_t)cnt * 4);
            }
        }
        out.commit();
    }

    const uint8_t* nb(size_t v) const { return &search_data[v * RL.vertex_bytes + RL.nb_off]; }
    const float* vec(size_t v) const { return (raw_view ? raw_view : raw.data()) + v * D; }
};

inline size_t dev_dword_offset(const DevLayout& L, uint32_t plane, uint32_t w, uint32_t i) {
    const uint32_t t = plane * L.PW + w;
    if (L.wide) {
        const uint32_t ck = t / 4, e = t % 4;
        const uint32_t h = (L.NH == 2) ? ck / L.CPL : 0;
        const uint32_t k = (L.NH == 2) ? ck % L.CPL : ck;
        return ((size_t)(k * L.NH * 32 + h * 32 + i) * 16 + e * 4);
    }
    return ((size_t)t * 32 + i) * 4;
}

inline void repack_ref_to_dev(const uint8_t* ref_nb, const RefLayout& RL, const DevLayout& L,
                              uint8_t* dev) {
    std::memset(dev, 0, L.stride);
    const size_t bytes_per_plane_nb = (L.D + 7) / 8;
    const size_t plane_stride = round_up(RL.plane_bytes, 64);
    for (uint32_t b = 0; b < L.BW; ++b) {
        const uint8_t* plane = ref_nb + RL.codes + b * plane_stride;
        for (uint32_t w = 0; w < L.PW; ++w)
            for (uint32_t i = 0; i < 32; ++i) {
                uint32_t v = 0;
                for (uint32_t s = 0; s < 4; ++s) {
                    size_t sp = (size_t)4 * w + s;
                    if (sp < bytes_per_plane_nb) v |= (uint32_t)plane[sp * 32 + i] << (8 * s);
                }
                std::memcpy(dev + dev_dword_offset(L, b, w, i), &v, 4);
            }
    }
    const float* nop = reinterpret_cast<const float*>(ref_nb + RL.nop);
    const float* ipqo = reinterpret_cast<const float*>(ref_nb + RL.ip_qo);
    const float* ipcp = reinterpret_cast<const float*>(ref_nb + RL.ip_cp);
    const uint16_t* pop = reinterpret_cast<const uint16_t*>(ref_nb + RL.pop);
    const uint16_t* wpop = L.BW > 1 ? reinterpret_cast<const uint16_t*>(ref_nb + RL.wpop) : nullptr;
    for (uint32_t i = 0; i < 32; ++i) {
        uint32_t a[4];
        std::memcpy(&a[0], &nop[i], 4);
        std::memcpy(&a[1], &ipqo[i], 4);
        std::memcpy(&a[2], &ipcp[i], 4);
        a[3] = (uint32_t)pop[i] | ((uint32_t)(wpop ? wpop[i] : 0) << 16);
        std::memcpy(dev + L.aux_off + i * 16, a, 16);
    }
    uint32_t cnt;
    std::memcpy(&cnt, ref_nb + RL.count, 4);
    if (cnt > 32) cnt = 32;
    uint32_t ids[32];
    std::memcpy(ids, ref_nb + RL.ids, 128);
    for (uint32_t i = cnt; i < 32; ++i) ids[i] = kInvalidNode;
    std::memcpy(dev + L.ids_off, ids, 128);
    std::memcpy(dev + L.count_off, &cnt, 4);
}

inline void repack_dev_to_ref(const uint8_t* dev, const DevLayout& L, const RefLayout& RL,
                              uint8_t* ref_nb) {
    std::memset(ref_nb, 0, RL.nb_bytes);
    const size_t bytes_per_plane_nb = (L.D + 7) / 8;
    const size_t plane_stride = round_up(RL.plane_bytes, 64);
    for (uint32_t b = 0; b < L.BW; ++b) {
        uint8_t* plane = ref_nb + RL.codes + b * plane_stride;
        for (uint32_t w = 0; w < L.PW; ++w)
            for (uint32_t i = 0; i < 32; ++i) {
                uint32_t v;
                std::memcpy(&v, dev + dev_dword_offset(L, b, w, i), 4);
                for (uint32_t s = 0; s < 4; ++s) {
                    size_t sp = (size_t)4 * w + s;
                    if (sp < bytes_per_plane_nb) plane[sp * 32 + i] = (uint8_t)(v >> (8 * s));
                }
            }
    }
    for (uint32_t i = 0; i < 32; ++i) {
        uint32_t a[4];
        std::memcpy(a, dev + L.aux_off + i * 16, 16);
        std::memcpy(ref_nb + RL.nop + 4 * i, &a[0], 4);
        std::memcpy(ref_nb + RL.ip_qo + 4 * i, &a[1], 4);
        std::memcpy(ref_nb + RL.ip_cp + 4 * i, &a[2], 4);
        uint16_t p = (uint16_t)(a[3] & 0xFFFF), wp = (uint16_t)(a[3] >> 16);
        std::memcpy(ref_nb + RL.pop + 2 * i, &p, 2);
        if (L.BW > 1) std::memcpy(ref_nb + RL.wpop + 2 * i, &wp, 2);
    }
    std::memcpy(ref_nb + RL.ids, dev + L.ids_off, 128);
    std::memcpy(ref_nb + RL.count, dev + L.count_off, 4);
}

}
```

Measured before the change: 5.870 million queries/s.

## Store 4-bit codes as nibble-packed words and score with udot8

For 4-bit wide layouts, the resident code blocks are converted from bit-plane order to per-vector nibble-packed words with a relayout kernel after upload, build, load and stream fill. Query masks are spread into matching nibble words in LDS, and the FastScan reduce uses three udot8 accumulations (full, top bit, top two bits) instead of per-plane popcount work. Downloads convert back to plane order so the host formats stay unchanged. This aims to cut ALU work per block in the hot scan, at the cost of an extra relayout pass at load time, different per-lane load addressing, and more code paths to keep correct.

```diff
diff --git a/include/cphnsw_mi355x.h b/include/cphnsw_mi355x.h
--- a/include/cphnsw_mi355x.h
+++ b/include/cphnsw_mi355x.h
@@ -105,6 +105,9 @@
 int cph_host_rewrite_index(const char* path_in, const char* path_out);
 int cph_host_repack_block(uint32_t D, uint32_t bits, const uint8_t* ref_block, uint8_t* dev_block,
                           uint64_t* dev_bytes, uint8_t* ref_roundtrip);
+int cph_host_relayout_block(uint32_t D, uint32_t bits, const uint8_t* dev_block, uint8_t* resident_block,
+                            uint8_t* dev_roundtrip);
+int cph_export_blocks(cph_index* h, uint64_t first, uint64_t count, int resident, uint8_t* out);
 int cph_host_encode_query(uint64_t dim, const float* query, uint8_t* lut, float* coeffs, uint32_t* masks);
 
 #ifdef __cplusplus
diff --git a/rabitq-ann-search_amd/cphnsw_mi355x/_lib.py b/rabitq-ann-search_amd/cphnsw_mi355x/_lib.py
--- a/rabitq-ann-search_amd/cphnsw_mi355x/_lib.py
+++ b/rabitq-ann-search_amd/cphnsw_mi355x/_lib.py
@@ -55,6 +55,8 @@
     "cph_exact_l2": (C.c_int, [C.c_void_p, C.c_void_p, C.c_void_p, C.c_uint64, C.c_void_p]),
     "cph_host_rewrite_index": (C.c_int, [C.c_char_p, C.c_char_p]),
     "cph_host_repack_block": (C.c_int, [C.c_uint32, C.c_uint32, C.c_void_p, C.c_void_p, C.POINTER(C.c_uint64), C.c_void_p]),
+    "cph_host_relayout_block": (C.c_int, [C.c_uint32, C.c_uint32, C.c_void_p, C.c_void_p, C.c_void_p]),
+    "cph_export_blocks": (C.c_int, [C.c_void_p, C.c_uint64, C.c_uint64, C.c_int, C.c_void_p]),
     "cph_host_encode_query": (C.c_int, [C.c_uint64, C.c_void_p, C.c_void_p, C.c_void_p, C.c_void_p]),
     "cph_fastscan_stream_create": (C.c_int, [C.c_int, C.c_uint32, C.c_uint32, C.c_uint64, C.c_uint64,
                                              C.POINTER(C.c_void_p), C.POINTER(C.c_uint64)]),
diff --git a/rabitq-ann-search_amd/cphnsw_mi355x/build.py b/rabitq-ann-search_amd/cphnsw_mi355x/build.py
--- a/rabitq-ann-search_amd/cphnsw_mi355x/build.py
+++ b/rabitq-ann-search_amd/cphnsw_mi355x/build.py
@@ -6,7 +6,7 @@
 CSRC = os.path.join(os.path.dirname(PKG_DIR), "csrc")
 LIB_PATH = os.path.join(PKG_DIR, "libcphnsw_mi355x.so")
 SOURCES = ["cphnsw_mi355x.hip"]
-HEADERS = ["cph_core.h", "builder.h", "builder_host.h", "host_parallel.h", "search_coalescer.h", "builder_pipeline.h", "device_knn.h", "device_knn_sym.h", "device_build.h", "device_buf.h", "native_file.h", "device_encode.h", "device_fastscan.h", "device_search.h", "device_stream.h", "device_heap_test.h", "host_index.h"]
+HEADERS = ["cph_core.h", "builder.h", "builder_host.h", "host_parallel.h", "search_coalescer.h", "builder_pipeline.h", "device_knn.h", "device_knn_sym.h", "device_build.h", "device_buf.h", "native_file.h", "device_encode.h", "device_fastscan.h", "device_search.h", "device_stream.h", "device_heap_test.h", "device_relayout.h", "host_index.h"]
 FLAGS = ["-O3", "-std=c++17", "--offload-arch=gfx950", "-fPIC", "-shared", "-ffp-contract=off",
          "-Wall", "-Wno-unused-function"]
 
diff --git a/rabitq-ann-search_amd/csrc/builder_pipeline.h b/rabitq-ann-search_amd/csrc/builder_pipeline.h
--- a/rabitq-ann-search_amd/csrc/builder_pipeline.h
+++ b/rabitq-ann-search_amd/csrc/builder_pipeline.h
@@ -271,6 +271,7 @@
         a.nbr = nullptr;
         run_encode(bw, a, (n + 31) / 32, num_cus);
     }
+    relayout_blocks(dev.blocks.p, n, L, true);
     tm.lap("gather + edge / own codes");
 
     std::vector<int32_t> levels_new(n);
diff --git a/rabitq-ann-search_amd/csrc/cph_core.h b/rabitq-ann-search_amd/csrc/cph_core.h
--- a/rabitq-ann-search_amd/csrc/cph_core.h
+++ b/rabitq-ann-search_amd/csrc/cph_core.h
@@ -1,6 +1,12 @@
 #pragma once
 #include <cstddef>
 #include <cstdint>
+
+#if defined(__HIPCC__)
+#define CPH_HD __host__ __device__
+#else
+#define CPH_HD
+#endif
 
 namespace cph {
 
@@ -23,6 +29,7 @@
     uint32_t ids_off;
     uint32_t count_off;
     uint32_t stride;
+    uint32_t nib;
 };
 
 #ifndef CPH_BLOCK_ALIGN
@@ -56,7 +63,46 @@
     L.ids_off = L.aux_off + 32 * 16;
     L.count_off = L.ids_off + 32 * 4;
     L.stride = (L.count_off + 4 + CPH_BLOCK_ALIGN - 1) / CPH_BLOCK_ALIGN * CPH_BLOCK_ALIGN;
+    L.nib = (BW == 4 && L.wide) ? 1 : 0;
     return L;
+}
+
+CPH_HD inline uint32_t plane_dword_offset(const DevLayout& L, uint32_t plane, uint32_t w, uint32_t i) {
+    const uint32_t t = plane * L.PW + w;
+    if (L.wide) {
+        const uint32_t ck = t / 4, e = t % 4;
+        const uint32_t h = (L.NH == 2) ? ck / L.CPL : 0;
+        const uint32_t k = (L.NH == 2) ? ck % L.CPL : ck;
+        return (k * L.NH * 32 + h * 32 + i) * 16 + e * 4;
+    }
+    return (t * 32 + i) * 4;
+}
+
+CPH_HD inline uint32_t nib_spread8(uint32_t x) {
+    x &= 0xFFu;
+    x = (x | (x << 12)) & 0x000F000Fu;
+    x = (x | (x << 6)) & 0x03030303u;
+    return (x | (x << 3)) & 0x11111111u;
+}
+CPH_HD inline uint32_t nib_compact8(uint32_t x) {
+    x &= 0x11111111u;
+    x = (x | (x >> 3)) & 0x03030303u;
+    x = (x | (x >> 6)) & 0x000F000Fu;
+    return (x | (x >> 12)) & 0xFFu;
+}
+CPH_HD inline uint32_t nib_word_from_planes(uint32_t p0, uint32_t p1, uint32_t p2, uint32_t p3, uint32_t w) {
+    const uint32_t sh = 8u * (w & 3u);
+    return (nib_spread8(p0 >> sh) << 3) | (nib_spread8(p1 >> sh) << 2) | (nib_spread8(p2 >> sh) << 1) |
+           nib_spread8(p3 >> sh);
+}
+CPH_HD inline uint32_t plane_dword_from_nibs(uint32_t n0, uint32_t n1, uint32_t n2, uint32_t n3, uint32_t b) {
+    const uint32_t sh = 3u - b;
+    return nib_compact8(n0 >> sh) | (nib_compact8(n1 >> sh) << 8) | (nib_compact8(n2 >> sh) << 16) |
+           (nib_compact8(n3 >> sh) << 24);
+}
+CPH_HD inline uint32_t qmask_nib_word(uint32_t q0, uint32_t q1, uint32_t q2, uint32_t q3, uint32_t s) {
+    const uint32_t sh = 8u * s;
+    return nib_spread8(q0 >> sh) | (nib_spread8(q1 >> sh) << 1) | (nib_spread8(q2 >> sh) << 2) | (nib_spread8(q3 >> sh) << 3);
 }
 
 struct RefLayout {
diff --git a/rabitq-ann-search_amd/csrc/cphnsw_mi355x.hip b/rabitq-ann-search_amd/csrc/cphnsw_mi355x.hip
--- a/rabitq-ann-search_amd/csrc/cphnsw_mi355x.hip
+++ b/rabitq-ann-search_amd/csrc/cphnsw_mi355x.hip
@@ -22,6 +22,7 @@
 #include "device_search.h"
 #include "device_stream.h"
 #include "device_heap_test.h"
+#include "device_relayout.h"
 #include "host_index.h"
 #include "host_parallel.h"
 #include "search_coalescer.h"
@@ -216,6 +217,7 @@
         HIP_CHECK(hipMemcpy(h->d_blocks.p + base * stride, stage.data(), cnt * stride,
                             hipMemcpyHostToDevice));
     }
+    relayout_blocks(h->d_blocks.p, n, h->L, true);
     HIP_CHECK(hipMemcpy(h->d_raw.p, hi.raw.data(), n * hi.D * 4, hipMemcpyHostToDevice));
     HIP_CHECK(hipMemcpy(h->d_norm.p, hi.norm_sq.data(), n * 4, hipMemcpyHostToDevice));
 }
@@ -304,7 +306,7 @@
     std::vector<uint8_t> stage(chunk * stride);
     for (size_t base = 0; base < n; base += chunk) {
         const size_t c = std::min(chunk, n - base);
-        HIP_CHECK(hipMemcpy(stage.data(), h->d_blocks.p + base * stride, c * stride, hipMemcpyDeviceToHost));
+        download_blocks(h->d_blocks.p + base * stride, c, h->L, stage.data());
         parallel_for(c, 256, [&](size_t lo, size_t hi_) {
             for (size_t v = lo; v < hi_; ++v) {
                 uint8_t* dst = &hi.search_data[(base + v) * hi.RL.vertex_bytes];
@@ -750,7 +752,7 @@
         const HostIndex& hi = h->host;
         const size_t n = hi.n, stride = h->L.stride, own_stride = hi.RL.nb_off;
         std::vector<uint8_t> blocks(n * stride), own;
-        HIP_CHECK(hipMemcpy(blocks.data(), h->d_blocks.p, n * stride, hipMemcpyDeviceToHost));
+        download_blocks(h->d_blocks.p, n, h->L, blocks.data());
         const uint8_t* own_p = h->own_view;
         if (!own_p) {
             own.resize(n * own_stride);
@@ -783,6 +785,7 @@
         h->d_raw.alloc(n * h->host.D);
         h->d_norm.alloc(n);
         HIP_CHECK(hipMemcpy(h->d_blocks.p, base + nh.blocks_off, n * (size_t)nh.stride, hipMemcpyHostToDevice));
+        relayout_blocks(h->d_blocks.p, n, h->L, true);
         HIP_CHECK(hipMemcpy(h->d_raw.p, h->host.raw_view, n * h->host.D * 4, hipMemcpyHostToDevice));
         HIP_CHECK(hipMemcpy(h->d_norm.p, h->host.norm_sq.data(), n * 4, hipMemcpyHostToDevice));
         upload_feeders(h);
@@ -1521,6 +1524,32 @@
     });
 }
 
+int cph_host_relayout_block(uint32_t D, uint32_t bits, const uint8_t* dev_block, uint8_t* resident_block,
+                            uint8_t* dev_roundtrip) {
+    return guarded([&] {
+        if (bits != 1 && bits != 2 && bits != 4) throw InvalidArg("bits must be 1, 2 or 4");
+        if (D < 16 || D > 2048 || (D & (D - 1))) throw InvalidArg("D must be a power of two in 16..2048");
+        if (!dev_block || !resident_block) throw InvalidArg("null block");
+        const DevLayout L = make_dev_layout(D, bits);
+        block_plane_to_nib(dev_block, L, resident_block);
+        if (dev_roundtrip) block_nib_to_plane(resident_block, L, dev_roundtrip);
+    });
+}
+
+int cph_export_blocks(cph_index* h, uint64_t first, uint64_t count, int resident, uint8_t* out) {
+    return guarded([&] {
+        if (!h || !out) throw InvalidArg("null argument");
+        std::lock_guard<std::mutex> lk(h->mu);
+        if (!h->finalized) throw std::runtime_error("Index must be finalized.");
+        if (first > h->host.n || count > h->host.n - first) throw InvalidArg("block range out of bounds");
+        h->use_device();
+        quiesce(h);
+        const uint8_t* src = h->d_blocks.p + first * h->L.stride;
+        if (resident) HIP_CHECK(hipMemcpy(out, src, count * h->L.stride, hipMemcpyDeviceToHost));
+        else download_blocks(src, count, h->L, out);
+    });
+}
+
 int cph_host_encode_query(uint64_t dim, const float* query, uint8_t* lut, float* coeffs, uint32_t* masks) {
     return guarded([&] {
         const size_t D = std::max<size_t>(16, next_pow2(dim));
@@ -1662,6 +1691,7 @@
         hipLaunchKernelGGL(stream_fill_kernel, dim3(s->num_cus * 16), dim3(64), 0, nullptr,
                            s->d_blocks.p, n_blocks, s->L, seed);
         HIP_CHECK(hipGetLastError());
+        relayout_blocks(s->d_blocks.p, n_blocks, s->L, true);
         std::mt19937_64 rng(seed * 7919 + 13);
         std::normal_distribution<float> nd(0.0f, 1.0f);
         std::vector<float> q(D);
@@ -1714,8 +1744,7 @@
         if (first + count > s->n_blocks) throw InvalidArg("block range out of bounds");
         if (count && ref_blocks) {
             std::vector<uint8_t> dev(count * s->L.stride);
-            HIP_CHECK(hipMemcpy(dev.data(), s->d_blocks.p + first * s->L.stride, dev.size(),
-                                hipMemcpyDeviceToHost));
+            download_blocks(s->d_blocks.p + first * s->L.stride, count, s->L, dev.data());
             parallel_for(count, 1024, [&](size_t lo, size_t hi) {
                 for (size_t b = lo; b < hi; ++b)
                     repack_dev_to_ref(&dev[b * s->L.stride], s->L, s->RL, ref_blocks + b * s->RL.nb_bytes);
diff --git a/rabitq-ann-search_amd/csrc/device_build.h b/rabitq-ann-search_amd/csrc/device_build.h
--- a/rabitq-ann-search_amd/csrc/device_build.h
+++ b/rabitq-ann-search_amd/csrc/device_build.h
@@ -624,7 +624,7 @@
     const int lane = threadIdx.x;
     for (uint32_t s = blockIdx.x; s < a.ns; s += gridDim.x) {
         __syncthreads();
-        for (uint32_t w = lane; w < PW; w += 64) qm[w] = a.qmasks[(size_t)s * PW + w];
+        for (uint32_t w = lane; w < PW; w += 64) qm[w] = qm_lds_word(a.qmasks[(size_t)s * PW + w], nib_codes<BW, 0>(a.L));
         for (uint32_t d = lane; d < D; d += 64) qv[d] = a.queries[(size_t)s * D + d];
         __syncthreads();
         uint32_t parent = a.start[s];
diff --git a/rabitq-ann-search_amd/csrc/device_fastscan.h b/rabitq-ann-search_amd/csrc/device_fastscan.h
--- a/rabitq-ann-search_amd/csrc/device_fastscan.h
+++ b/rabitq-ann-search_amd/csrc/device_fastscan.h
@@ -38,6 +38,49 @@
     auto r = __builtin_amdgcn_permlane32_swap(x, x, false, false);
     lo = r[0];
     hi = r[1];
+}
+
+template <int BW, int SD>
+__device__ __forceinline__ bool nib_codes(const DevLayout& L) {
+    if constexpr (BW != 4) return false;
+    else if constexpr (SD != 0) return SD >= 128;
+    else return L.nib != 0u;
+}
+
+__device__ __forceinline__ uint4 qm_lds_word(uint4 m, bool nib) {
+    if (!nib) return m;
+    return make_uint4(qmask_nib_word(m.x, m.y, m.z, m.w, 0), qmask_nib_word(m.x, m.y, m.z, m.w, 1),
+                      qmask_nib_word(m.x, m.y, m.z, m.w, 2), qmask_nib_word(m.x, m.y, m.z, m.w, 3));
+}
+
+__device__ __forceinline__ void dot3(uint32_t c, uint32_t q, uint32_t& s, uint32_t& s8, uint32_t& s12) {
+    s = __builtin_amdgcn_udot8(c, q, s, false);
+    s8 = __builtin_amdgcn_udot8(c & 0x88888888u, q, s8, false);
+    s12 = __builtin_amdgcn_udot8(c & 0xCCCCCCCCu, q, s12, false);
+}
+__device__ __forceinline__ void dot3(uint4 c, uint4 q, uint32_t& s, uint32_t& s8, uint32_t& s12) {
+    dot3(c.x, q.x, s, s8, s12);
+    dot3(c.y, q.y, s, s8, s12);
+    dot3(c.z, q.z, s, s8, s12);
+    dot3(c.w, q.w, s, s8, s12);
+}
+template <int SD>
+__device__ __forceinline__ void nib_merge(uint32_t s, uint32_t s8, uint32_t s12, uint32_t& nbit, uint32_t& msb,
+                                          uint32_t& msb2) {
+    uint32_t lo, hi;
+    if constexpr (SD != 0 && SD <= 256) {
+        half_pair(s | (s8 << 16), lo, hi);
+        const uint32_t t = lo + hi;
+        nbit = t & 0xFFFFu;
+        msb = t >> 19;
+    } else {
+        half_pair(s, lo, hi);
+        nbit = lo + hi;
+        half_pair(s8, lo, hi);
+        msb = (lo + hi) >> 3;
+    }
+    half_pair(s12, lo, hi);
+    msb2 = (lo + hi) >> 2;
 }
 
 template <int BW, int SD>
@@ -49,7 +92,14 @@
     const bool wide = SD ? (SD >= 128) : (L.wide != 0);
     if (wide) {
         const uint4* cp = reinterpret_cast<const uint4*>(blk) + lane;
-        if constexpr (BW >= 2) {
+        if constexpr (BW == 4) {
+            const uint4* cn = reinterpret_cast<const uint4*>(blk) + (uint32_t)(lane & 31) * PW + h;
+            const uint4* qn = qm + h;
+            uint32_t s = 0, s8 = 0, s12 = 0;
+#pragma unroll 2
+            for (uint32_t g = 0; g < PW / 2; ++g) dot3(cn[2 * g], qn[2 * g], s, s8, s12);
+            nib_merge<SD>(s, s8, s12, nbit, msb, msb2);
+        } else if constexpr (BW == 2) {
             constexpr int PPH = BW / 2;
             const uint32_t G = PW >> 2;
             uint32_t S[PPH];
@@ -73,15 +123,8 @@
             half_pair(part, plo, phi);
             nbit = plo + phi;
             half_pair(S[0], s0, s0hi);
-            if constexpr (BW == 2) {
-                msb = s0;
-                msb2 = 2 * s0 + s0hi;
-            } else {
-                uint32_t s1, s1hi;
-                half_pair(S[1], s1, s1hi);
-                msb = s0;
-                msb2 = 2 * s0 + s1;
-            }
+            msb = s0;
+            msb2 = 2 * s0 + s0hi;
         } else {
             const uint32_t NH = SD ? ((SD / 32) / 4 >= 2 ? 2 : 1) : L.NH;
             const uint32_t CPL = SD ? ((SD / 32) / 4 / NH) : L.CPL;
@@ -127,23 +170,30 @@
     static constexpr int kT = kStatic ? BW * (SD / 32) : 4;
     static constexpr int kNH = (kT / 4 >= 2) ? 2 : 1;
     static constexpr int kCPL = kStatic ? kT / 4 / kNH : 1;
+    static constexpr bool kNib = kStatic && BW == 4;
     uint4 c[kCPL];
     uint4 aux;
 
+    __device__ __forceinline__ void issue_codes(const uint8_t* __restrict__ blk, int lane) {
+        if constexpr (kNib) {
+            const uint4* cp = reinterpret_cast<const uint4*>(blk) + (lane & 31) * (SD / 32) + (lane >> 5);
+#pragma unroll
+            for (int k = 0; k < kCPL; ++k) c[k] = cp[k * kNH];
+        } else {
+            const uint4* cp = reinterpret_cast<const uint4*>(blk) + (lane & (kNH * 32 - 1));
+#pragma unroll
+            for (int k = 0; k < kCPL; ++k) c[k] = cp[k * kNH * 32];
+        }
+    }
+
     __device__ __forceinline__ void issue_static(const uint8_t* __restrict__ blk, int lane) {
         static_assert(kStatic, "static D only");
-        const uint4* cp = reinterpret_cast<const uint4*>(blk) + (lane & (kNH * 32 - 1));
-#pragma unroll
-        for (int k = 0; k < kCPL; ++k) c[k] = cp[k * kNH * 32];
+        issue_codes(blk, lane);
         aux = reinterpret_cast<const uint4*>(blk + StaticLayout<BW, SD>::kAuxOff)[lane & 31];
     }
 
     __device__ __forceinline__ void issue(const uint8_t* __restrict__ blk, const DevLayout& L, int lane) {
-        if constexpr (kStatic) {
-            const uint4* cp = reinterpret_cast<const uint4*>(blk) + (lane & (kNH * 32 - 1));
-#pragma unroll
-            for (int k = 0; k < kCPL; ++k) c[k] = cp[k * kNH * 32];
-        }
+        if constexpr (kStatic) issue_codes(blk, lane);
         aux = reinterpret_cast<const uint4*>(blk + L.aux_off)[lane & 31];
     }
 
@@ -158,7 +208,13 @@
 
     __device__ __forceinline__ void reduce(const uint8_t* __restrict__ blk, const DevLayout& L,
                                            const uint4* qm, int lane, LaneEst& o) {
-        if constexpr (kStatic) {
+        if constexpr (kNib) {
+            const uint4* qn = qm + (lane >> 5);
+            uint32_t s = 0, s8 = 0, s12 = 0;
+#pragma unroll
+            for (int k = 0; k < kCPL; ++k) dot3(c[k], qn[k * kNH], s, s8, s12);
+            nib_merge<SD>(s, s8, s12, o.nbit, o.msb, o.msb2);
+        } else if constexpr (kStatic) {
             const int h = lane >> 5;
             constexpr int PW = SD / 32;
             if constexpr (BW >= 2) {
@@ -185,15 +241,8 @@
                 half_pair(part, plo, phi);
                 o.nbit = plo + phi;
                 half_pair(S[0], s0, s0hi);
-                if constexpr (BW == 2) {
-                    o.msb = s0;
-                    o.msb2 = 2 * s0 + s0hi;
-                } else {
-                    uint32_t s1, s1hi;
-                    half_pair(S[1], s1, s1hi);
-                    o.msb = s0;
-                    o.msb2 = 2 * s0 + s1;
-                }
+                o.msb = s0;
+                o.msb2 = 2 * s0 + s0hi;
             } else {
                 uint32_t a0 = 0, a1 = 0, a2 = 0, a3 = 0;
                 if (h < kNH) {
diff --git a/rabitq-ann-search_amd/csrc/device_relayout.h b/rabitq-ann-search_amd/csrc/device_relayout.h
--- /dev/null
+++ b/rabitq-ann-search_amd/csrc/device_relayout.h
@@ -0,0 +1,66 @@
+#pragma once
+#include <hip/hip_runtime.h>
+
+#include <algorithm>
+
+#include "cph_core.h"
+#include "device_buf.h"
+
+namespace cph {
+
+template <bool TO_NIB>
+__global__ __launch_bounds__(64) void relayout_kernel(uint8_t* blocks, uint64_t n_blocks, DevLayout L) {
+    extern __shared__ __align__(16) unsigned char smem[];
+    uint4* s4 = reinterpret_cast<uint4*>(smem);
+    const uint8_t* sb = smem;
+    const int lane = threadIdx.x;
+    const uint32_t chunks = L.codes_bytes / 16, dwords = L.codes_bytes / 4;
+    const uint32_t NW = L.D / 8;
+    for (uint64_t b = blockIdx.x; b < n_blocks; b += gridDim.x) {
+        const uint4* in = reinterpret_cast<const uint4*>(blocks + b * L.stride);
+        uint32_t* out = reinterpret_cast<uint32_t*>(blocks + b * L.stride);
+        for (uint32_t j = lane; j < chunks; j += 64) s4[j] = in[j];
+        __syncthreads();
+        for (uint32_t o = lane; o < dwords; o += 64) {
+            if constexpr (TO_NIB) {
+                const uint32_t i = o / NW, w = o % NW;
+                uint32_t p[4];
+#pragma unroll
+                for (uint32_t pl = 0; pl < 4; ++pl)
+                    p[pl] = *reinterpret_cast<const uint32_t*>(sb + plane_dword_offset(L, pl, w / 4, i));
+                out[o] = nib_word_from_planes(p[0], p[1], p[2], p[3], w);
+            } else {
+                const uint32_t i = o % 32, t = o / 32, pl = t / L.PW, pw = t % L.PW;
+                const uint4 nw = *reinterpret_cast<const uint4*>(sb + ((size_t)i * NW + 4 * pw) * 4);
+                out[plane_dword_offset(L, pl, pw, i) / 4] = plane_dword_from_nibs(nw.x, nw.y, nw.z, nw.w, pl);
+            }
+        }
+        __syncthreads();
+    }
+}
+
+inline void relayout_blocks(uint8_t* blocks, uint64_t n, const DevLayout& L, bool to_nib) {
+    if (!L.nib || n == 0) return;
+    const uint32_t grid = (uint32_t)std::min<uint64_t>(n, 1u << 16);
+    if (to_nib) hipLaunchKernelGGL(relayout_kernel<true>, dim3(grid), dim3(64), L.codes_bytes, nullptr, blocks, n, L);
+    else hipLaunchKernelGGL(relayout_kernel<false>, dim3(grid), dim3(64), L.codes_bytes, nullptr, blocks, n, L);
+    HIP_CHECK(hipGetLastError());
+    HIP_CHECK(hipDeviceSynchronize());
+}
+
+inline void download_blocks(const uint8_t* blocks, uint64_t n, const DevLayout& L, uint8_t* host) {
+    if (!L.nib) {
+        HIP_CHECK(hipMemcpy(host, blocks, n * L.stride, hipMemcpyDeviceToHost));
+        return;
+    }
+    const uint64_t chunk = std::max<uint64_t>(1, std::min<uint64_t>(n, (64u << 20) / L.stride));
+    DevBuf<uint8_t> stage(chunk * L.stride);
+    for (uint64_t base = 0; base < n; base += chunk) {
+        const uint64_t c = std::min(chunk, n - base);
+        HIP_CHECK(hipMemcpy(stage.p, blocks + base * L.stride, c * L.stride, hipMemcpyDeviceToDevice));
+        relayout_blocks(stage.p, c, L, false);
+        HIP_CHECK(hipMemcpy(host + base * L.stride, stage.p, c * L.stride, hipMemcpyDeviceToHost));
+    }
+}
+
+}
diff --git a/rabitq-ann-search_amd/csrc/device_search.h b/rabitq-ann-search_amd/csrc/device_search.h
--- a/rabitq-ann-search_amd/csrc/device_search.h
+++ b/rabitq-ann-search_amd/csrc/device_search.h
@@ -547,7 +547,7 @@
         {
             const uint4* qmasks = CPH_COLD(qmasks);
             const float* queries = CPH_COLD(queries);
-            for (uint32_t w = lane; w < PW; w += 64) qm[w] = qmasks[(size_t)qi * PW + w];
+            for (uint32_t w = lane; w < PW; w += 64) qm[w] = qm_lds_word(qmasks[(size_t)qi * PW + w], nib_codes<BW, SD>(a.L));
             for (uint32_t d = lane; d < D; d += 64) qv[d] = queries[(size_t)qi * D + d];
         }
         const QueryHeader hd = CPH_COLD(qhdr)[qi];
diff --git a/rabitq-ann-search_amd/csrc/device_stream.h b/rabitq-ann-search_amd/csrc/device_stream.h
--- a/rabitq-ann-search_amd/csrc/device_stream.h
+++ b/rabitq-ann-search_amd/csrc/device_stream.h
@@ -24,7 +24,7 @@
     extern __shared__ __align__(16) unsigned char smem[];
     uint4* qm = reinterpret_cast<uint4*>(smem);
     const uint32_t PW = SD ? (SD >= 32 ? SD / 32 : 1) : a.L.PW;
-    for (uint32_t w = threadIdx.x; w < PW; w += blockDim.x) qm[w] = a.qmask[w];
+    for (uint32_t w = threadIdx.x; w < PW; w += blockDim.x) qm[w] = qm_lds_word(a.qmask[w], nib_codes<BW, SD>(a.L));
     __syncthreads();
     const int lane = threadIdx.x & 63;
     const uint64_t wave = (uint64_t)blockIdx.x * (blockDim.x >> 6) + (threadIdx.x >> 6);
@@ -169,7 +169,7 @@
     uint4* qm = reinterpret_cast<uint4*>(smem);
     const uint32_t PW = SD ? (SD >= 32 ? SD / 32 : 1) : a.L.PW;
     const int lane = threadIdx.x;
-    for (uint32_t w = lane; w < PW; w += 64) qm[w] = a.qmask[w];
+    for (uint32_t w = lane; w < PW; w += 64) qm[w] = qm_lds_word(a.qmask[w], nib_codes<BW, SD>(a.L));
     __syncthreads();
     LaneEst v;
     load_block<BW, SD>(a.blk, a.L, qm, lane, v);
diff --git a/rabitq-ann-search_amd/csrc/host_index.h b/rabitq-ann-search_amd/csrc/host_index.h
--- a/rabitq-ann-search_amd/csrc/host_index.h
+++ b/rabitq-ann-search_amd/csrc/host_index.h
@@ -309,14 +309,38 @@
 };
 
 inline size_t dev_dword_offset(const DevLayout& L, uint32_t plane, uint32_t w, uint32_t i) {
-    const uint32_t t = plane * L.PW + w;
-    if (L.wide) {
-        const uint32_t ck = t / 4, e = t % 4;
-        const uint32_t h = (L.NH == 2) ? ck / L.CPL : 0;
-        const uint32_t k = (L.NH == 2) ? ck % L.CPL : ck;
-        return ((size_t)(k * L.NH * 32 + h * 32 + i) * 16 + e * 4);
-    }
-    return ((size_t)t * 32 + i) * 4;
+    return plane_dword_offset(L, plane, w, i);
+}
+
+inline void block_plane_to_nib(const uint8_t* src, const DevLayout& L, uint8_t* dst) {
+    std::vector<uint8_t> out(src, src + L.stride);
+    if (L.nib) {
+        const uint32_t NW = L.D / 8;
+        for (uint32_t i = 0; i < 32; ++i)
+            for (uint32_t w = 0; w < NW; ++w) {
+                uint32_t p[4];
+                for (uint32_t b = 0; b < 4; ++b) std::memcpy(&p[b], src + plane_dword_offset(L, b, w / 4, i), 4);
+                const uint32_t v = nib_word_from_planes(p[0], p[1], p[2], p[3], w);
+                std::memcpy(&out[((size_t)i * NW + w) * 4], &v, 4);
+            }
+    }
+    std::memcpy(dst, out.data(), L.stride);
+}
+inline void block_nib_to_plane(const uint8_t* src, const DevLayout& L, uint8_t* dst) {
+    std::vector<uint8_t> out(src, src + L.stride);
+    if (L.nib) {
+        const uint32_t NW = L.D / 8;
+        for (uint32_t i = 0; i < 32; ++i)
+            for (uint32_t pw = 0; pw < L.PW; ++pw) {
+                uint32_t n[4];
+                std::memcpy(n, src + ((size_t)i * NW + 4 * pw) * 4, 16);
+                for (uint32_t b = 0; b < 4; ++b) {
+                    const uint32_t v = plane_dword_from_nibs(n[0], n[1], n[2], n[3], b);
+                    std::memcpy(&out[plane_dword_offset(L, b, pw, i)], &v, 4);
+                }
+            }
+    }
+    std::memcpy(dst, out.data(), L.stride);
 }
 
 inline void repack_ref_to_dev(const uint8_t* ref_nb, const RefLayout& RL, const DevLayout& L,
```

New measurement: 6.133 million queries/s, median of 6. 4.5% higher.
